# junfeng-chen/position_induced_transformer

Measured on AMD Instinct MI355X. Metric: PiT fwd+bwd samples/sec on Darcy2D, higher is better.
Workload: dtype f32; 1 GPU; darcy2d 43x43 grid->16x16 latent, pit_fixed hid64 H2 blocks4 loc0.02, RelL2 (train_darcy.py:64-111), fwd+loss+bwd, per-GPU batch 8; per_gpu_batch=8, global_batch=8, parallelism=single, launch=hipgraph, head_scale_route=host

## Files before the change

### include/pit_hip.h

```cpp
#ifndef PIT_HIP_H
#define PIT_HIP_H

#ifdef __cplusplus
extern "C" {
#endif

#define PIT_ABI_VERSION 23
#define PIT_DSCALE_SLOTS 1024

#define PIT_METRIC_EUCLID     0
#define PIT_METRIC_PERIODIC1D 1
#define PIT_METRIC_PERIODIC2D 2

#define PIT_ERR_NULL     -1
#define PIT_ERR_SIZE     -2
#define PIT_ERR_METRIC   -3
#define PIT_ERR_UNSUPPORTED -4

int pit_version(void);
const char* pit_error_string(int code);

#define PIT_MATH_FP32 0
#define PIT_MATH_BF16 1
#define PIT_IO_X_BF16    0x100
#define PIT_IO_SAVE_BF16 0x200
#define PIT_IO_DX_BF16   0x400
#define PIT_IO_OUT_BF16  0x800
#define PIT_IO_DOUT_BF16 0x1000
#define PIT_ATT_UNION    0x2000
int pit_mlp_bf16_io_supported(int rows, int n0, int n1, int n2, int out_gelu);

int pit_head_scale(const float* lmda, int n_head, float* scale_out, void* stream);

int pit_select_fwd(const float* mesh_out, const float* mesh_in, int mesh_batch, int n_out, int n_in,
                   int space_dim, int metric, float period, int rank_k, int need_kth,
                   float* stats, void* stream);

int pit_lists_transpose(const int* nbr_idx, const int* nbr_cnt, int mesh_batch, int n_out, int n_in, int cap,
                        int* rev_ptr, int* rev_row, int* workspace, void* stream);

#define PIT_PLAN_WAVE_PER_ROW 1
#define PIT_PLAN_TWO_PASSES   2
int pit_plan_fwd(const float* mesh_out, const float* mesh_in, int mesh_batch, int n_out, int n_in,
                 int space_dim, int metric, float period, int rank_k, float* stats, int cap,
                 int* nbr_idx, int* nbr_cnt, int* rev_ptr, int* rev_row, int* workspace, int flags, void* stream);

int pit_neighbors_fwd(const float* mesh_out, const float* mesh_in, int mesh_batch, int n_out, int n_in,
                      int space_dim, int metric, float period, const float* stats, int cap,
                      int* nbr_idx, int* nbr_cnt, int* rev_ptr, int* rev_row, int* workspace, void* stream);

int pit_posatt_fwd(const float* mesh_out, const float* mesh_in, int mesh_batch, int n_out, int n_in,
                   int space_dim, int metric, float period,
                   const float* values, int batch, int dim, long ld_values, long values_bstride,
                   const float* head, int n_head, int head_is_scale,
                   const float* stats, float rank_w, int masked, int self_attn,
                   float* out, long ld_out, long out_bstride, int out_col0, int copy_inputs,
                   float* rowstat, float* scale_out,
                   const int* nbr_idx, const int* nbr_cnt, int nbr_cap, int coord_dims, int math_mode, void* stream);

struct pit_mlp_params_job;

struct pit_block_weights_job {
    const float* mesh; int n_pts, space_dim, metric; float period;
    int n_layers; const float* const* heads; int head_is_scale, n_head;
    float *e, *q, *inv, *rowstat, *scale_out;
};
int pit_posatt_fwd_job(const float* mesh_out, const float* mesh_in, int mesh_batch, int n_out, int n_in,
                       int space_dim, int metric, float period,
                       const float* values, int batch, int dim, long ld_values, long values_bstride,
                       const float* head, int n_head, int head_is_scale,
                       const float* stats, float rank_w, int masked, int self_attn,
                       float* out, long ld_out, long out_bstride, int out_col0, int copy_inputs,
                       float* rowstat, float* scale_out,
                       const int* nbr_idx, const int* nbr_cnt, int nbr_cap, int coord_dims, int math_mode, void* stream,
                       const struct pit_block_weights_job* job);

typedef struct pit_mlp_params_job {
    const float* x; long ldx; int rows, n0, n1, n2; const float* h; int out_gelu;
    const float* d_y; long ld_dy;
    float *d_w1, *d_b1, *d_w2, *d_b2; int accumulate; const float* scratch; int math_mode;
} pit_mlp_params_job;
#define PIT_HEAD_ACCUMULATE 1
#define PIT_HEAD_DEFER      2
#define PIT_HEAD_IS_SCALE   4
int pit_posatt_bwd(const float* mesh_out, const float* mesh_in, int mesh_batch, int n_out, int n_in,
                   int space_dim, int metric, float period,
                   const float* values, int batch, int dim, long ld_values, long values_bstride,
                   const float* head, int n_head, int head_is_scale, const float* scale,
                   const float* rowstat, int masked,
                   const float* d_out, long ld_dout, long dout_bstride, int out_col0,
                   float* d_values, long ld_dvalues, long dvalues_bstride, int add_residual,
                   float* d_head, int accumulate_head, double* workspace,
                   const int* nbr_idx, const int* nbr_cnt, int nbr_cap, int nbr_complete,
                   const int* rev_ptr, const int* rev_row, const pit_mlp_params_job* rider,
                   int coord_dims, int math_mode, void* stream);

int pit_posatt_dhead_finish(int n_layers, double* const* workspaces, float* const* d_heads,
                            const float* const* heads, const float* const* scales, const int* n_heads,
                            const int* flags, const pit_mlp_params_job* rider, void* stream);

int pit_block_supported(int n_pts, int n_head, int dim, int batch);

int pit_block_weights(const float* mesh, int n_pts, int space_dim, int metric, float period, int n_layers,
                      const float* const* heads, int head_is_scale, int n_head, float* e, float* q,
                      float* inv, float* rowstat, float* scale_out, void* stream);

int pit_block_fwd(const float* e, const float* inv, int n_pts, int n_head, int dim, int batch, float* xcat,
                  const float* w1, const float* b1, const float* w2, const float* b2, int out_gelu,
                  float* z1, float* h, float* z2, float* y, long ldy, int math_mode, void* stream);

int pit_block_bwd(const float* e, const float* inv, const float* qw, int n_pts, int n_head, int dim, int batch,
                  const float* d_xcat, const float* xcat, double* dscale,
                  const float* w1, const float* w2, const float* z1, const float* z2, int out_gelu, int n0_prev,
                  float* d_xprev, long ld_dxprev, float* scratch_prev,
                  float* d_values, long ld_dvalues,
                  const struct pit_mlp_params_job* rider, const struct pit_mlp_params_job* rider2,
                  int math_mode, void* stream);

#define PIT_SLAB_UNION_MAX 64
typedef struct pit_slab_plan {
    int n_out, n_in, cap, n_slabs, umax;
    const float* stats; float rank_w;
    const int* idx; const int* cnt;
    const float* m; const unsigned short* slot; const int* keys; const int* nkeys;
    int rows;
} pit_slab_plan;
int pit_slab_plan_build(const float* mesh_out, const float* mesh_in, int n_out, int n_in, int space_dim, int metric, float period,
                        const int* nbr_idx, const int* nbr_cnt, int cap, int rows_per_slab, float* m, unsigned short* slot,
                        int* keys, int* nkeys, int* report, void* stream);
int pit_edge_supported(int n_head, int dim, int batch, int rows_per_sample);
int pit_decoder_weights(const pit_slab_plan* plan, const float* head, int head_is_scale, int n_head, int max_union, int max_count,
                        float* pw, float* qw, float* scale_out, const float* w1, float* w1f, int dim, void* stream);
typedef struct pit_decoder_weights_job {
    const pit_slab_plan* plan; const float* head; int head_is_scale, n_head, max_union, max_count;
    float *pw, *qw, *scale_out;
    const float* w1; float* w1f; int dim;
} pit_decoder_weights_job;
int pit_decoder_fwd(const pit_slab_plan* plan, const float* values, long ld_values, long values_bstride, int batch,
                    int n_head, int dim, const float* pw,
                    const float* w1, const float* w1f, const float* b1, const float* w2, const float* b2, int n2,
                    float* x, float* z1, float* h, float* y, float* zero_buf, long zero_n,
                    const float* loss_true, const float* loss_scale, const float* loss_shift, int loss_p, double* loss_part,
                    int max_union, void* stream);
int pit_decoder_bwd(const pit_slab_plan* plan, const float* values, long ld_values, long values_bstride, int batch,
                    int n_head, int dim, const float* pw, const float* qw,
                    const float* w1, const float* w2, int n2, const float* z1,
                    const float* d_y, long ld_dy, float* dz1, float* d_values, long dvalues_bstride, double* dscale,
                    const float* loss_pred, const float* loss_true, const float* loss_scale, const float* loss_shift,
                    const float* loss_seed, int loss_p, const double* loss_part, float* d_pred, float* loss_out,
                    float* norms_out, int max_union, void* stream);
int pit_union_att_supported(int n_head, int dim, int batch, int rows_per_sample);
int pit_union_att_fwd(const pit_slab_plan* plan, const float* values, long ld_values, long values_bstride, int batch,
                      int n_head, int dim, const float* pw, void* out, long ld_out, long out_bstride, int out_bf16,
                      int max_union, void* stream);
int pit_union_att_bwd(const pit_slab_plan* plan, const float* values, long ld_values, long values_bstride, int batch,
                      int n_head, int dim, const float* pw, const float* qw,
                      const void* d_out, long ld_dout, long dout_bstride, int dout_bf16,
                      float* d_values, long ld_dvalues, long dvalues_bstride, double* dscale, int max_union, void* stream);
int pit_fold_supported(int n_head, int dim, int batch, int rows_per_sample, int n_in);
int pit_fold_weights(const pit_slab_plan* plan, const float* head, int head_is_scale, int n_head, int max_union, int max_count,
                     float* pw, float* qw, float* scale_out, unsigned short* pw16, unsigned short* qw16, void* stream);
int pit_fold_att_fwd(const pit_slab_plan* plan, const float* vw, long ld_vw, long vw_bstride, int batch, int n_head, int dim,
                     const void* pw, void* z, long ld_z, long z_bstride, int max_union, int math_mode, void* stream);
int pit_fold_att_bwd(const pit_slab_plan* plan, const float* vw, long ld_vw, long vw_bstride, int batch, int n_head, int dim,
                     const void* pw, const void* qw, const void* dz, long ld_dz, long dz_bstride,
                     float* d_vw, long ld_dvw, long dvw_bstride, double* dscale,
                     float* tiles, const int* rev_ptr, const int* rev_ent, int max_union, int math_mode, void* stream);
int pit_thin_tail_scratch_floats(void);
int pit_thin_tail_fwd(const void* z, long ldz, int rows, int n1, int n2, const float* b1, const float* w2, const float* b2,
                      float* y, long ldy, int math_mode, void* stream);
int pit_thin_tail_bwd(const void* z, long ldz, int rows, int n1, int n2, const float* b1, const float* w2,
                      const float* d_y, long ld_dy, void* dz, long ld_dz, float* d_b1, float* d_w2, float* d_b2,
                      float* scratch, int math_mode, void* stream);
int pit_linear_fwd(const float* x, long ldx, int rows, int n_in, int n_out, const float* w, const float* zero_bias,
                   float* y, long ldy, int math_mode, void* stream);
int pit_linear_bwd(const float* x, long ldx, int rows, int n_in, int n_out, const float* w, const float* d_y, long ld_dy,
                   float* d_x, long ld_dx, float* d_w, int accumulate, int math_mode, void* stream);

struct pit_block_weights_job;
int pit_encoder_fwd(const pit_slab_plan* plan, const float* mesh_in, int space_dim, int coord_dims,
                    const float* values, long ld_values, long values_bstride, int value_dim, int batch,
                    int n_head, int dim, const float* head, int head_is_scale,
                    const float* w1, const float* b1, const float* w2, const float* b2,
                    float* x, float* z1, float* h, float* z2, float* y, long ldy, float* rowstat, float* scale_out,
                    float* clear_buf, long clear_n, const struct pit_block_weights_job* weights,
                    const pit_decoder_weights_job* dec_weights, void* stream);
int pit_encoder_bwd(const pit_slab_plan* plan, const float* mesh_in, int space_dim, int coord_dims,
                    const float* values, long ld_values, long values_bstride, int value_dim, int batch,
                    int n_head, int dim, const float* scale, const float* rowstat,
                    const float* w1, const float* w2, const float* z1, const float* z2,
                    const float* d_y, long ld_dy, float* scratch, double* dscale, void* stream);

int pit_posatt_pre_supported(int n_pts, int n_head, int dim, int batch);
int pit_posatt_pre_fwd(const float* e, const float* rowstat, int n_pts, int n_head, int dim, int batch,
                       const float* values, long ld_values, long values_bstride,
                       float* out, long ld_out, long out_bstride, int out_col0, int copy_inputs, int math_mode, void* stream);
int pit_posatt_pre_bwd(const float* e, const float* q, const float* rowstat, int n_pts, int n_head, int dim, int batch,
                       const float* values, long ld_values, long values_bstride,
                       const float* d_out, long ld_dout, long dout_bstride, int out_col0,
                       float* d_values, long ld_dvalues, long dvalues_bstride, int add_residual,
                       double* workspace, int math_mode, void* stream);

int pit_satt_supported(int n_pts, int n_head, int dim, int batch, int mesh_batch);
int pit_satt_fwd(const float* mesh, int mesh_batch, int n_pts, int space_dim, int metric, float period,
                 const float* values, long ld_values, long values_bstride, int batch, int dim,
                 const float* head, int n_head, int head_is_scale, unsigned short* x16,
                 float* out, long ld_out, long out_bstride, int out_col0, int copy_inputs,
                 float* rowstat, float* scale_out, unsigned short* e_tiles, int x16_ready, void* stream);
int pit_satt_bwd(const float* mesh, int mesh_batch, int n_pts, int space_dim, int metric, float period,
                 int batch, int dim, const float* scale, int n_head, const float* rowstat,
                 const unsigned short* x16, unsigned short* g16,
                 const float* d_out, long ld_dout, long dout_bstride, int out_col0,
                 float* d_values, long ld_dvalues, long dvalues_bstride, int add_residual, double* dscale,
                 const unsigned short* e_tiles, int g16_ready, const pit_mlp_params_job* rider, void* stream);
long pit_satt_tiles_elems(int n_pts);

int pit_mlp_fwd(const float* x, long ldx, int rows, int n0, int n1, int n2,
                const float* w1, const float* b1, const float* w2, const float* b2, int out_gelu,
                float* z1, float* h, float* z2, float* y, long ldy, int math_mode, void* stream);

int pit_mlp_chain_supported(int rows, int n0, int n1, int n2);
int pit_mlp_chain_fwd(const float* x, long ldx, int rows, int n0, int n1, const unsigned short* w1_bf16, const float* b1,
                      const unsigned short* w2_bf16, const float* b2, float* z1, float* h, float* z2, float* y, long ldy,
                      unsigned short* y16 , void* stream);
int pit_mlp_chain_bwd(int rows, int n0, int n1, const unsigned short* w1_bf16, const unsigned short* w2_bf16,
                      const float* z1, const float* z2, const float* d_y, long ld_dy, float* d_x, long ld_dx, float* scratch,
                      unsigned short* g16 ,
                      const float* rowstat , int pts, int mesh_batch, void* stream);
int pit_cast_bf16_multi(int n, const float* const* src, unsigned short* const* dst, const long* count, void* stream);

int pit_mlp_bwd(const float* x, long ldx, int rows, int n0, int n1, int n2,
                const float* w1, const float* w2, const float* z1, const float* h, const float* z2,
                int out_gelu, const float* d_y, long ld_dy,
                float* d_x, long ld_dx, float* d_w1, float* d_b1, float* d_w2, float* d_b2,
                int accumulate, float* scratch, int math_mode, void* stream);

int pit_mlp_bwd_data(int rows, int n0, int n1, int n2, const float* w1, const float* w2,
                     const float* z1, const float* z2, int out_gelu, const float* d_y, long ld_dy,
                     float* d_x, long ld_dx, float* scratch, int math_mode, void* stream);
int pit_mlp_bwd_params(const float* x, long ldx, int rows, int n0, int n1, int n2, const float* h,
                       int out_gelu, const float* d_y, long ld_dy,
                       float* d_w1, float* d_b1, float* d_w2, float* d_b2,
                       int accumulate, const float* scratch, int math_mode, void* stream);
int pit_mlp_bwd_params_deferrable(int rows, int n0, int n1, int n2, int out_gelu, long ld_dy);

#define PIT_REL_LP_WS_FLOATS(batch, nch) (4 + 5 * (batch) * (nch))
int pit_rel_lp_loss_fwd(const float* tru, const float* pred, const float* pred_scale,
                        const float* pred_shift, int batch, int npts, int nch, int p,
                        float* norms, float* loss, float* workspace, void* stream);
int pit_rel_lp_loss_bwd(const float* tru, const float* pred, const float* pred_scale,
                        const float* pred_shift, int batch, int npts, int nch, int p,
                        const float* norms, const float* grad_loss, float* d_pred, float* d_true, void* stream);

int pit_rel_lp_loss_fwd_grad(const float* tru, const float* pred, const float* pred_scale,
                             const float* pred_shift, int batch, int npts, int nch, int p,
                             float* norms, float* loss, float* workspace, float* d_pred_unit,
                             float* d_true_unit, float* clear_buf, long clear_n, void* stream);

int pit_rel_max_norm(const float* tru, const float* pred, int batch, int npts, int nch, float* out,
                     double* workspace, void* stream);

int pit_instance_norm_fwd(const float* x, long ldx, long x_bstride, int batch, int npts, int nch, float eps,
                          float* y, float* rstd, void* stream);
int pit_instance_norm_bwd(const float* d_y, const float* y, const float* rstd, int batch, int npts, int nch,
                          float* d_x, void* stream);

int pit_adam_step(float* params, float* grads, float* exp_avg, float* exp_avg_sq, long n,
                  long long* step, float lr0, float eta_min, int cosine_t_max, float beta1, float beta2,
                  float eps, float weight_decay, int zero_grads, float* scalars, void* stream);

int pit_debug_mfma_tile(const float* a, const float* b, float* d, void* stream);

#ifdef __cplusplus
}
#endif
#endif
```

### position_induced_transformer_amd/_lib.py

```python
from __future__ import annotations

import ctypes
import os

import torch

_HERE = os.path.dirname(os.path.abspath(__file__))
LIB_PATH = os.environ.get("PIT_LIB_PATH") or os.path.join(_HERE, "csrc", "libpit_hip.so")

_P = ctypes.c_void_p
_I = ctypes.c_int
_L = ctypes.c_long
_F = ctypes.c_float

class MlpParamsJob(ctypes.Structure):
    _fields_ = [("x", _P), ("ldx", _L), ("rows", _I), ("n0", _I), ("n1", _I), ("n2", _I), ("h", _P), ("out_gelu", _I),
                ("d_y", _P), ("ld_dy", _L), ("d_w1", _P), ("d_b1", _P), ("d_w2", _P), ("d_b2", _P),
                ("accumulate", _I), ("scratch", _P), ("math_mode", _I)]


class BlockWeightsJob(ctypes.Structure):
    _fields_ = [("mesh", _P), ("n_pts", _I), ("space_dim", _I), ("metric", _I), ("period", _F),
                ("n_layers", _I), ("heads", _P), ("head_is_scale", _I), ("n_head", _I),
                ("e", _P), ("q", _P), ("inv", _P), ("rowstat", _P), ("scale_out", _P)]


class SlabPlan(ctypes.Structure):
    _fields_ = [("n_out", _I), ("n_in", _I), ("cap", _I), ("n_slabs", _I), ("umax", _I), ("stats", _P), ("rank_w", _F),
                ("idx", _P), ("cnt", _P), ("m", _P), ("slot", _P), ("keys", _P), ("nkeys", _P), ("rows", _I)]


class DecoderWeightsJob(ctypes.Structure):
    _fields_ = [("plan", _P), ("head", _P), ("head_is_scale", _I), ("n_head", _I), ("max_union", _I), ("max_count", _I),
                ("pw", _P), ("qw", _P), ("scale_out", _P), ("w1", _P), ("w1f", _P), ("dim", _I)]


SIGNATURES = {
    "pit_version": [],
    "pit_error_string": [_I],
    "pit_head_scale": [_P, _I, _P, _P],
    "pit_select_fwd": [_P, _P, _I, _I, _I, _I, _I, _F, _I, _I, _P, _P],
    "pit_plan_fwd": [_P, _P, _I, _I, _I, _I, _I, _F, _I, _P, _I, _P, _P, _P, _P, _P, _I, _P],
    "pit_lists_transpose": [_P, _P, _I, _I, _I, _I, _P, _P, _P, _P],
    "pit_neighbors_fwd": [_P, _P, _I, _I, _I, _I, _I, _F, _P, _I, _P, _P, _P, _P, _P, _P],
    "pit_posatt_fwd": [_P, _P, _I, _I, _I, _I, _I, _F,
                       _P, _I, _I, _L, _L,
                       _P, _I, _I,
                       _P, _F, _I, _I,
                       _P, _L, _L, _I, _I,
                       _P, _P, _P, _P, _I, _I, _I, _P],
    "pit_posatt_fwd_job": [_P, _P, _I, _I, _I, _I, _I, _F,
                           _P, _I, _I, _L, _L,
                           _P, _I, _I,
                           _P, _F, _I, _I,
                           _P, _L, _L, _I, _I,
                           _P, _P, _P, _P, _I, _I, _I, _P, _P],
    "pit_posatt_bwd": [_P, _P, _I, _I, _I, _I, _I, _F,
                       _P, _I, _I, _L, _L,
                       _P, _I, _I, _P,
                       _P, _I,
                       _P, _L, _L, _I,
                       _P, _L, _L, _I,
                       _P, _I, _P, _P, _P, _I, _I, _P, _P, _P, _I, _I, _P],
    "pit_posatt_dhead_finish": [_I, _P, _P, _P, _P, _P, _P, _P, _P],
    "pit_block_supported": [_I, _I, _I, _I],
    "pit_block_weights": [_P, _I, _I, _I, _F, _I, _P, _I, _I, _P, _P, _P, _P, _P, _P],
    "pit_block_fwd": [_P, _P, _I, _I, _I, _I, _P, _P, _P, _P, _P, _I, _P, _P, _P, _P, _L, _I, _P],
    "pit_slab_plan_build": [_P, _P, _I, _I, _I, _I, _F, _P, _P, _I, _I, _P, _P, _P, _P, _P, _P],
    "pit_fold_supported": [_I, _I, _I, _I, _I],
    "pit_fold_weights": [_P, _P, _I, _I, _I, _I, _P, _P, _P, _P, _P, _P],
    "pit_fold_att_fwd": [_P, _P, _L, _L, _I, _I, _I, _P, _P, _L, _L, _I, _I, _P],
    "pit_fold_att_bwd": [_P, _P, _L, _L, _I, _I, _I, _P, _P, _P, _L, _L, _P, _L, _L, _P, _P, _P, _P, _I, _I, _P],
    "pit_thin_tail_scratch_floats": [],
    "pit_thin_tail_fwd": [_P, _L, _I, _I, _I, _P, _P, _P, _P, _L, _I, _P],
    "pit_thin_tail_bwd": [_P, _L, _I, _I, _I, _P, _P, _P, _L, _P, _L, _P, _P, _P, _P, _I, _P],
    "pit_satt_supported": [_I, _I, _I, _I, _I],
    "pit_satt_fwd": [_P, _I, _I, _I, _I, _F, _P, _L, _L, _I, _I, _P, _I, _I, _P, _P, _L, _L, _I, _I, _P, _P, _P, _I, _P],
    "pit_satt_bwd": [_P, _I, _I, _I, _I, _F, _I, _I, _P, _I, _P, _P, _P, _P, _L, _L, _I, _P, _L, _L, _I, _P, _P, _I, _P, _P],
    "pit_satt_tiles_elems": [_I],
    "pit_mlp_chain_supported": [_I, _I, _I, _I],
    "pit_mlp_chain_fwd": [_P, _L, _I, _I, _I, _P, _P, _P, _P, _P, _P, _P, _P, _L, _P, _P],
    "pit_mlp_chain_bwd": [_I, _I, _I, _P, _P, _P, _P, _P, _L, _P, _L, _P, _P, _P, _I, _I, _P],
    "pit_cast_bf16_multi": [_I, _P, _P, _P, _P],
    "pit_linear_fwd": [_P, _L, _I, _I, _I, _P, _P, _P, _L, _I, _P],
    "pit_linear_bwd": [_P, _L, _I, _I, _I, _P, _P, _L, _P, _L, _P, _I, _I, _P],
    "pit_edge_supported": [_I, _I, _I, _I],
    "pit_decoder_weights": [_P, _P, _I, _I, _I, _I, _P, _P, _P, _P, _P, _I, _P],
    "pit_decoder_fwd": [_P, _P, _L, _L, _I, _I, _I, _P, _P, _P, _P, _P, _P, _I, _P, _P, _P, _P, _P, _L,
                        _P, _P, _P, _I, _P, _I, _P],
    "pit_decoder_bwd": [_P, _P, _L, _L, _I, _I, _I, _P, _P, _P, _P, _I, _P, _P, _L, _P, _P, _L, _P,
                        _P, _P, _P, _P, _P, _I, _P, _P, _P, _P, _I, _P],
    "pit_union_att_supported": [_I, _I, _I, _I],
    "pit_union_att_fwd": [_P, _P, _L, _L, _I, _I, _I, _P, _P, _L, _L, _I, _I, _P],
    "pit_union_att_bwd": [_P, _P, _L, _L, _I, _I, _I, _P, _P, _P, _L, _L, _I, _P, _L, _L, _P, _I, _P],
    "pit_encoder_fwd": [_P, _P, _I, _I, _P, _L, _L, _I, _I, _I, _I, _P, _I, _P, _P, _P, _P,
                        _P, _P, _P, _P, _P, _L, _P, _P, _P, _L, _P, _P, _P],
    "pit_encoder_bwd": [_P, _P, _I, _I, _P, _L, _L, _I, _I, _I, _I, _P, _P, _P, _P, _P, _P, _P, _L, _P, _P, _P],
    "pit_posatt_pre_supported": [_I, _I, _I, _I],
    "pit_posatt_pre_fwd": [_P, _P, _I, _I, _I, _I, _P, _L, _L, _P, _L, _L, _I, _I, _I, _P],
    "pit_posatt_pre_bwd": [_P, _P, _P, _I, _I, _I, _I, _P, _L, _L, _P, _L, _L, _I, _P, _L, _L, _I, _P, _I, _P],
    "pit_block_bwd": [_P, _P, _P, _I, _I, _I, _I, _P, _P, _P, _P, _P, _P, _P, _I, _I, _P, _L, _P, _P, _L, _P, _P, _I, _P],
    "pit_mlp_bf16_io_supported": [_I, _I, _I, _I, _I],
    "pit_mlp_fwd": [_P, _L, _I, _I, _I, _I, _P, _P, _P, _P, _I, _P, _P, _P, _P, _L, _I, _P],
    "pit_mlp_bwd": [_P, _L, _I, _I, _I, _I, _P, _P, _P, _P, _P, _I, _P, _L,
                    _P, _L, _P, _P, _P, _P, _I, _P, _I, _P],
    "pit_mlp_bwd_data": [_I, _I, _I, _I, _P, _P, _P, _P, _I, _P, _L, _P, _L, _P, _I, _P],
    "pit_mlp_bwd_params": [_P, _L, _I, _I, _I, _I, _P, _I, _P, _L, _P, _P, _P, _P, _I, _P, _I, _P],
    "pit_mlp_bwd_params_deferrable": [_I, _I, _I, _I, _I, _L],
    "pit_rel_lp_loss_fwd": [_P, _P, _P, _P, _I, _I, _I, _I, _P, _P, _P, _P],
    "pit_rel_lp_loss_fwd_grad": [_P, _P, _P, _P, _I, _I, _I, _I, _P, _P, _P, _P, _P, _P, _L, _P],
    "pit_rel_lp_loss_bwd": [_P, _P, _P, _P, _I, _I, _I, _I, _P, _P, _P, _P, _P],
    "pit_rel_max_norm": [_P, _P, _I, _I, _I, _P, _P, _P],
    "pit_instance_norm_fwd": [_P, _L, _L, _I, _I, _I, _F, _P, _P, _P],
    "pit_instance_norm_bwd": [_P, _P, _P, _I, _I, _I, _P, _P],
    "pit_adam_step": [_P, _P, _P, _P, _L, _P, _F, _F, _I, _F, _F, _F, _F, _I, _P, _P],
    "pit_debug_mfma_tile": [_P, _P, _P, _P],
}

LONG_RETURN = {"pit_satt_tiles_elems"}
ABI_VERSION = 23

_lib = None


def lib() -> ctypes.CDLL:
    global _lib
    if _lib is None:
        if not os.path.exists(LIB_PATH):
            raise RuntimeError(
                f"{LIB_PATH} not found: build it with `python -m position_induced_transformer_amd.build` "
                "(hipcc --offload-arch=gfx950). There is no CPU or PyTorch fallback for the PiT hot path.")
        handle = ctypes.CDLL(LIB_PATH)
        for name, argtypes in SIGNATURES.items():
            fn = getattr(handle, name)
            fn.argtypes = argtypes
            fn.restype = ctypes.c_char_p if name == "pit_error_string" else (_L if name in LONG_RETURN else _I)
        got = handle.pit_version()
        if got != ABI_VERSION:
            raise RuntimeError(f"{LIB_PATH} implements PIT_ABI_VERSION {got}, this package binds version {ABI_VERSION}: "
                               "rebuild it (python -m position_induced_transformer_amd.build)")
        _lib = handle
    return _lib


def check(code: int, what: str) -> None:
    if code != 0:
        msg = lib().pit_error_string(code)
        raise RuntimeError(f"{what} failed ({code}): {msg.decode() if msg else '?'}")


def stream_ptr() -> int:
    return torch.cuda.current_stream().cuda_stream


def ptr(t) -> int:
    return 0 if t is None else t.data_ptr()
```

### position_induced_transformer_amd/csrc/pit_block.hip

```cpp
#include "pit_common.h"
#include "pit_gemm_rd.h"
#include "pit_block_dev.h"
#include <cstdlib>

namespace {

#ifdef PIT_STAMPS
__device__ unsigned long long pit_block_stamps[32];
#define BSTAMP(i_) do { if (blockIdx.x == 5 && threadIdx.x == 0) pit_block_stamps[i_] = __builtin_amdgcn_s_memtime(); } while (0)
#else
#define BSTAMP(i_) do { } while (0)
#endif

#ifdef PIT_WGREC
__device__ unsigned long long pit_block_wgrec[1024 * 4];
#define BREC(slot_) do { if (threadIdx.x == 0 && blockIdx.x < 1024) {                                                       \
        pit_block_wgrec[blockIdx.x * 4 + (slot_)] = __builtin_amdgcn_s_memrealtime();                                       \
        if ((slot_) == 0) { pit_block_wgrec[blockIdx.x * 4 + 2] = __builtin_amdgcn_s_getreg((4 << 0) | (0 << 6) | (31 << 11));   \
                            pit_block_wgrec[blockIdx.x * 4 + 3] = __builtin_amdgcn_s_getreg((20 << 0) | (0 << 6) | (31 << 11)); } } } while (0)
#else
#define BREC(slot_) do { } while (0)
#endif
#ifdef PIT_STAMPS_DBG
__device__ int pit_block_dbg = 0;
#define PIT_BLOCK_DBG pit_block_dbg
#else
#define PIT_BLOCK_DBG 0
#endif
#ifndef PIT_BLOCK_EXP
#define PIT_BLOCK_EXP 0
#endif

__global__ __launch_bounds__(256) void block_weights_kernel(WeightsArgs a) { block_weights_body(a, blockIdx.x); }

template <int NH, bool SHARED>
__device__ __forceinline__ void slab_contract(const float* __restrict__ w, long wstride, int L, const float* __restrict__ v,
                                              long ldv, int vhead, const float* __restrict__ sc, int jb, int je, int l15, int kq,
                                              f32x4_t (&acc)[SHARED ? NH : 1][4]) {
    constexpr int NS = SHARED ? 2 : 1;
    const float* wp = w + (long)l15 * L + 4 * kq;
    const float* vp = v + 4 * l15;
    for (int j0 = jb; j0 < je; j0 += 16 * NS) {
        float4 av[NH][NS], sv[NH][NS], bv[SHARED ? 1 : NH][NS][4];
        const int dbg = PIT_BLOCK_DBG;
#pragma unroll
        for (int h = 0; h < NH; ++h)
#pragma unroll
            for (int s = 0; s < NS; ++s) {
                av[h][s] = (dbg & 4) ? make_float4(1.f, 2.f, 3.f, 4.f) : *reinterpret_cast<const float4*>(wp + h * wstride + j0 + 16 * s);
                if (!SHARED) sv[h][s] = *reinterpret_cast<const float4*>(sc + (long)h * L + j0 + 16 * s + 4 * kq);
            }
#pragma unroll
        for (int h = 0; h < (SHARED ? 1 : NH); ++h)
#pragma unroll
            for (int s = 0; s < NS; ++s)
#pragma unroll
                for (int m = 0; m < 4; ++m)
                    bv[h][s][m] = (dbg & 2) ? make_float4(1.f, 2.f, 3.f, 4.f)
                                            : *reinterpret_cast<const float4*>(vp + h * vhead + (long)(j0 + 16 * s + 4 * kq + m) * ldv);
        __builtin_amdgcn_sched_barrier(0);
#pragma unroll
        for (int s = 0; s < NS; ++s)
#pragma unroll
            for (int m = 0; m < 4; ++m)
#pragma unroll
                for (int h = 0; h < NH; ++h) {
                    if ((PIT_BLOCK_EXP & (SHARED ? 1 : 4)) && (SHARED ? s == 1 : h == 1)) {
                        asm volatile("" :: "v"(av[h][s].x), "v"(av[h][s].y), "v"(av[h][s].z), "v"(av[h][s].w));
                        asm volatile("" :: "v"(bv[SHARED ? 0 : h][s][m].x), "v"(bv[SHARED ? 0 : h][s][m].y), "v"(bv[SHARED ? 0 : h][s][m].z), "v"(bv[SHARED ? 0 : h][s][m].w));
                        if (!SHARED) asm volatile("" :: "v"(sv[h][s].x), "v"(sv[h][s].y), "v"(sv[h][s].z), "v"(sv[h][s].w));
                        continue;
                    }
                    const float* ap = &av[h][s].x;
                    const float* sp = &sv[h][s].x;
                    const float aw = SHARED ? ap[m] : ap[m] * sp[m];
                    const float4 bb = bv[SHARED ? 0 : h][s][m];
                    f32x4_t (&ac)[4] = acc[SHARED ? h : 0];
                    ac[0] = mfma_16x16x4(aw, bb.x, ac[0]);
                    ac[1] = mfma_16x16x4(aw, bb.y, ac[1]);
                    ac[2] = mfma_16x16x4(aw, bb.z, ac[2]);
                    ac[3] = mfma_16x16x4(aw, bb.w, ac[3]);
                }
    }
}

__device__ __forceinline__ bool slab_of(int id, int batch, int slabs, int& sample, int& slab) {
    if (PIT_BLOCK_DBG & 1) return slab_of_linear(id, batch, slabs, sample, slab);
    return slab_of_xcd(id, batch, slabs, sample, slab);
}

struct BlockFwdArgs {
    const float *e, *inv;
    int L, batch;
    float* xcat;
    const float *w1, *b1, *w2, *b2;
    int out_gelu;
    float *z1, *h, *z2, *y; long ldy;
};

template <int H, bool WLDS>
__global__ __launch_bounds__(512, WLDS ? 1 : 2) void block_fwd_kernel(BlockFwdArgs g) {
    constexpr int W = (1 + H) * BD;
    constexpr int XP = W + 4, HP = BD + 4;
    constexpr int KS = W / 16;
    constexpr int NW1 = BD * W / 4 / 512, NW2 = BD * BD / 4 / 512;
    extern __shared__ __attribute__((aligned(16))) float smem[];
    float* pk = smem;
    float* xs = smem + H * PARK_FLOATS;
    float* hs = xs + 16 * XP;
    float* w1s = hs + 16 * HP;
    float* w2s = w1s + BD * XP;
    const int tid = threadIdx.x, lane = tid & 63, wave = tid >> 6;
    const int l15 = lane & 15, kq = lane >> 4;
    const int slabs = g.L / 16;
    int b, slab;
    if (!slab_of(blockIdx.x, g.batch, slabs, b, slab)) return;
    const int n0 = slab * 16;
    const long m0 = ((long)b * slabs + slab) * 16;
    const int klen = g.L / BW;

    float4 xown = make_float4(0.f, 0.f, 0.f, 0.f);
    if (tid < 256) xown = *reinterpret_cast<const float4*>(g.xcat + (m0 + (tid >> 4)) * W + 4 * (tid & 15));
    const float rinv0 = g.inv[(long)((tid >> 8) % H) * g.L + n0 + 4 * ((tid & 63) >> 4) + ((tid >> 6) & 3)];

    BSTAMP(0);
    const bool mlp_wave = wave < 4;
    const int c1 = (wave & 3) * 16 + l15;
    float4 bv[KS], w2v[4];
    float bias = 0.0f, bias2 = 0.0f;
    auto load_weights = [&]() {
        if (!mlp_wave) return;
        if (!WLDS) {
#pragma unroll
            for (int s = 0; s < KS; ++s) bv[s] = *reinterpret_cast<const float4*>(g.w1 + (long)c1 * W + 16 * s + 4 * kq);
#pragma unroll
            for (int s = 0; s < 4; ++s) w2v[s] = *reinterpret_cast<const float4*>(g.w2 + (long)c1 * BD + 16 * s + 4 * kq);
        }
        bias = g.b1[c1];
        bias2 = g.b2[c1];
    };
    f32x4_t wq1[WLDS ? NW1 : 1], wq2[WLDS ? NW2 : 1];
    if (WLDS) {
#pragma unroll
        for (int p = 0; p < NW1; ++p) wq1[p] = reinterpret_cast<const f32x4_t*>(g.w1)[p * 512 + tid];
#pragma unroll
        for (int p = 0; p < NW2; ++p) wq2[p] = reinterpret_cast<const f32x4_t*>(g.w2)[p * 512 + tid];
        load_weights();
    }
    f32x4_t acc[H][4];
#pragma unroll
    for (int hh = 0; hh < H; ++hh)
#pragma unroll
        for (int t = 0; t < 4; ++t) acc[hh][t] = f32x4_t{0.f, 0.f, 0.f, 0.f};
    constexpr int EP = 256 + 4;
    const bool elds = WLDS && g.L == 256 && !(PIT_BLOCK_EXP & 64);
    if (elds) {
        float* es = w1s;
        const float* vp = g.xcat + (long)b * g.L * W + 4 * l15;
        const int j0 = wave * 32;
        f32x4_t eq[H * 2];
#pragma unroll
        for (int p = 0; p < H * 2; ++p) {
            const int q = p * 512 + tid;
            eq[p] = *reinterpret_cast<const f32x4_t*>(g.e + (long)(q >> 10) * g.L * g.L + (long)(n0 + ((q >> 6) & 15)) * g.L + 4 * (q & 63));
        }
        f32x4_t bvv[2][4];
#pragma unroll
        for (int s = 0; s < 2; ++s)
#pragma unroll
            for (int m = 0; m < 4; ++m) bvv[s][m] = *reinterpret_cast<const f32x4_t*>(vp + (long)(j0 + 16 * s + 4 * kq + m) * W);
        __builtin_amdgcn_sched_barrier(0);
#pragma unroll
        for (int p = 0; p < H * 2; ++p) {
            const int q = p * 512 + tid;
            *reinterpret_cast<f32x4_t*>(es + ((q >> 10) * 16 + ((q >> 6) & 15)) * EP + 4 * (q & 63)) = eq[p];
        }
        __syncthreads();
#pragma unroll
        for (int s = 0; s < 2; ++s) {
            f32x4_t av[H];
#pragma unroll
            for (int hh = 0; hh < H; ++hh) av[hh] = *reinterpret_cast<const f32x4_t*>(es + (hh * 16 + l15) * EP + j0 + 16 * s + 4 * kq);
#pragma unroll
            for (int m = 0; m < 4; ++m)
#pragma unroll
                for (int hh = 0; hh < H; ++hh) {
                    acc[hh][0] = mfma_16x16x4(av[hh][m], bvv[s][m][0], acc[hh][0]);
                    acc[hh][1] = mfma_16x16x4(av[hh][m], bvv[s][m][1], acc[hh][1]);
                    acc[hh][2] = mfma_16x16x4(av[hh][m], bvv[s][m][2], acc[hh][2]);
                    acc[hh][3] = mfma_16x16x4(av[hh][m], bvv[s][m][3], acc[hh][3]);
                }
        }
    } else {
        slab_contract<H, true>(g.e + (long)n0 * g.L, (long)g.L * g.L, g.L, g.xcat + (long)b * g.L * W, W, 0, nullptr,
                               wave * klen, (wave + 1) * klen, l15, kq, acc);
    }
    BSTAMP(1);
    if (!WLDS) load_weights();
#pragma unroll
    for (int hh = 0; hh < H; ++hh) park(pk, wave * H + hh, lane, acc[hh]);
    if (tid < 256) *reinterpret_cast<float4*>(xs + (tid >> 4) * XP + 4 * (tid & 15)) = xown;
    __syncthreads();
    BSTAMP(2);
    for (int item = tid; item < H * 256; item += 512) {
        const int hh = item >> 8, i = (item >> 6) & 3, ln = item & 63;
        const int r = 4 * (ln >> 4) + i, col = 4 * (ln & 15);
        float4 s = parked_sum(pk, hh, BW, H, i, ln);
        const float rinv = item == tid ? rinv0 : g.inv[(long)hh * g.L + n0 + r];
        s.x *= rinv; s.y *= rinv; s.z *= rinv; s.w *= rinv;
        *reinterpret_cast<float4*>(xs + r * XP + BD + hh * BD + col) = s;
        *reinterpret_cast<float4*>(g.xcat + (m0 + r) * W + BD + hh * BD + col) = s;
    }
    if (WLDS) {
#pragma unroll
        for (int p = 0; p < NW1; ++p) {
            const int q = p * 512 + tid, row = q / (W / 4), c4 = q % (W / 4);
            *reinterpret_cast<f32x4_t*>(w1s + row * XP + 4 * c4) = wq1[p];
        }
#pragma unroll
        for (int p = 0; p < NW2; ++p) {
            const int q = p * 512 + tid, row = q / (BD / 4), c4 = q % (BD / 4);
            *reinterpret_cast<f32x4_t*>(w2s + row * HP + 4 * c4) = wq2[p];
        }
    }
    BSTAMP(3);
    __syncthreads();
    BSTAMP(4);
    if (mlp_wave) {
        f32x4_t a0 = {0.f, 0.f, 0.f, 0.f}, a1 = {0.f, 0.f, 0.f, 0.f};
#pragma unroll
        for (int s = 0; s < KS; ++s) {
            if ((PIT_BLOCK_EXP & 2) && (s & 1)) { if (!WLDS) asm volatile("" :: "v"(bv[s].x), "v"(bv[s].y), "v"(bv[s].z), "v"(bv[s].w)); continue; }
            const float4 a = *reinterpret_cast<const float4*>(xs + l15 * XP + 16 * s + 4 * kq);
            const float4 bw = WLDS ? *reinterpret_cast<const float4*>(w1s + c1 * XP + 16 * s + 4 * kq) : bv[s];
            a0 = mfma_16x16x4(a.x, bw.x, a0);
            a1 = mfma_16x16x4(a.y, bw.y, a1);
            a0 = mfma_16x16x4(a.z, bw.z, a0);
            a1 = mfma_16x16x4(a.w, bw.w, a1);
        }
        BSTAMP(5);
#pragma unroll
        for (int i = 0; i < 4; ++i) {
            const int r = 4 * kq + i;
            const float z = a0[i] + a1[i] + bias;
            const float hv = gelu_erf(z);
            hs[r * HP + c1] = hv;
            g.z1[(m0 + r) * BD + c1] = z;
            g.h[(m0 + r) * BD + c1] = hv;
        }
    }
    BSTAMP(6);
    __syncthreads();
    BSTAMP(7);
    if (!mlp_wave) return;
    f32x4_t o0 = {0.f, 0.f, 0.f, 0.f}, o1 = {0.f, 0.f, 0.f, 0.f};
#pragma unroll
    for (int s = 0; s < 4; ++s) {
        const float4 a = *reinterpret_cast<const float4*>(hs + l15 * HP + 16 * s + 4 * kq);
        const float4 bw = WLDS ? *reinterpret_cast<const float4*>(w2s + c1 * HP + 16 * s + 4 * kq) : w2v[s];
        o0 = mfma_16x16x4(a.x, bw.x, o0);
        o1 = mfma_16x16x4(a.y, bw.y, o1);
        o0 = mfma_16x16x4(a.z, bw.z, o0);
        o1 = mfma_16x16x4(a.w, bw.w, o1);
    }
    BSTAMP(8);
#pragma unroll
    for (int i = 0; i < 4; ++i) {
        const long r = m0 + 4 * kq + i;
        float v = o0[i] + o1[i] + bias2;
        if (g.out_gelu) { g.z2[r * BD + c1] = v; v = gelu_erf(v); }
        g.y[r * g.ldy + c1] = v;
    }
    BSTAMP(9);
}

struct BlockBwdArgs {
    const float *e, *inv, *qw;
    int L, batch;
    const float* d_xcat;
    const float* xcat;
    double* dscale;
    const float *w1, *w2, *z1, *z2; int out_gelu, n0p;
    float *d_xprev; long ld_dxprev;
    float *dz1, *dz2;
    float* d_values; long ld_dvalues;
    int n_chain, n_ds;
};

template <int H>
__device__ __forceinline__ void block_bwd_chain(const BlockBwdArgs& g, float* smem, int slab) {
    constexpr int W = (1 + H) * BD;
    constexpr int P1 = BD + 4;
    float* pk = smem;
    float* ds2 = smem + PARK_FLOATS;
    float* ds1 = ds2 + 16 * P1;
    const int tid = threadIdx.x, lane = tid & 63, wave = tid >> 6;
    const int l15 = lane & 15, kq = lane >> 4;
    const int slabs = g.L / 16;
    int b, sl;
    if (!slab_of(slab, g.batch, slabs, b, sl)) return;
    const int j0 = sl * 16;
    const long m0 = ((long)b * slabs + sl) * 16;
    const int klen = g.L / BW;

    const int oi = (tid >> 6) & 3, oln = tid & 63, oh = tid >> 8;
    const int orow = 4 * (oln >> 4) + oi, ocol = 4 * (oln & 15) + 2 * oh;
    const bool has_mlp = g.w1 != nullptr;
    const float2 res = *reinterpret_cast<const float2*>(g.d_xcat + (m0 + orow) * W + ocol);
    float2 z2v = make_float2(0.f, 0.f);
    if (has_mlp && g.out_gelu) z2v = *reinterpret_cast<const float2*>(g.z2 + (m0 + orow) * BD + ocol);
    const int c1 = (wave & 3) * 16 + l15;
    BSTAMP(10);
    f32x4_t acc[1][4];
#pragma unroll
    for (int t = 0; t < 4; ++t) acc[0][t] = f32x4_t{0.f, 0.f, 0.f, 0.f};
    slab_contract<H, false>(g.e + (long)j0 * g.L, (long)g.L * g.L, g.L, g.d_xcat + (long)b * g.L * W + BD, W, BD, g.inv,
                            wave * klen, (wave + 1) * klen, l15, kq, acc);
    BSTAMP(11);
    float w2v[4][4], z1v[4], w1v[2][4][4];
    if (has_mlp) {
        if (wave < 4) {
#pragma unroll
            for (int s = 0; s < 4; ++s)
#pragma unroll
                for (int ee = 0; ee < 4; ++ee) w2v[s][ee] = g.w2[(long)(16 * s + 4 * kq + ee) * BD + c1];
#pragma unroll
            for (int i = 0; i < 4; ++i) z1v[i] = g.z1[(m0 + 4 * kq + i) * BD + c1];
        }
#pragma unroll
        for (int t = 0; t < 2; ++t) {
            const int col = (wave + t * BW) * 16 + l15;
#pragma unroll
            for (int s = 0; s < 4; ++s)
#pragma unroll
                for (int ee = 0; ee < 4; ++ee)
                    w1v[t][s][ee] = (col < g.n0p) ? g.w1[(long)(16 * s + 4 * kq + ee) * g.n0p + col] : 0.0f;
        }
    }
    park(pk, wave, lane, acc[0]);
    __syncthreads();
    BSTAMP(12);
    {
        float2 s = res;
#pragma unroll
        for (int w = 0; w < BW; ++w) {
            s.x += pk[((w * 4 + 2 * oh) * 4 + oi) * 64 + oln];
            s.y += pk[((w * 4 + 2 * oh + 1) * 4 + oi) * 64 + oln];
        }
        if (!has_mlp) {
            *reinterpret_cast<float2*>(g.d_values + (m0 + orow) * g.ld_dvalues + ocol) = s;
        } else {
            if (g.out_gelu) { s.x *= gelu_erf_grad(z2v.x); s.y *= gelu_erf_grad(z2v.y); }
            *reinterpret_cast<float2*>(g.dz2 + (m0 + orow) * BD + ocol) = s;
            *reinterpret_cast<float2*>(ds2 + orow * P1 + ocol) = s;
        }
    }
    if (!has_mlp) return;
    BSTAMP(13);
    __syncthreads();
    BSTAMP(14);
    if (wave < 4) {
        f32x4_t a0 = {0.f, 0.f, 0.f, 0.f}, a1 = {0.f, 0.f, 0.f, 0.f};
#pragma unroll
        for (int s = 0; s < 4; ++s) {
            const float4 a = *reinterpret_cast<const float4*>(ds2 + l15 * P1 + 16 * s + 4 * kq);
            a0 = mfma_16x16x4(a.x, w2v[s][0], a0);
            a1 = mfma_16x16x4(a.y, w2v[s][1], a1);
            a0 = mfma_16x16x4(a.z, w2v[s][2], a0);
            a1 = mfma_16x16x4(a.w, w2v[s][3], a1);
        }
#pragma unroll
        for (int i = 0; i < 4; ++i) {
            const int r = 4 * kq + i;
            const float v = (a0[i] + a1[i]) * gelu_erf_grad(z1v[i]);
            ds1[r * P1 + c1] = v;
            g.dz1[(m0 + r) * BD + c1] = v;
        }
    }
    BSTAMP(15);
    __syncthreads();
    BSTAMP(16);
    if (!g.d_xprev) return;
#pragma unroll
    for (int t = 0; t < 2; ++t) {
        const int tile = wave + t * BW;
        if (tile * 16 >= g.n0p) break;
        if ((PIT_BLOCK_EXP & 8) && t == 1) {
#pragma unroll
            for (int s = 0; s < 4; ++s) asm volatile("" :: "v"(w1v[t][s][0]), "v"(w1v[t][s][1]), "v"(w1v[t][s][2]), "v"(w1v[t][s][3]));
            break;
        }
        f32x4_t o0 = {0.f, 0.f, 0.f, 0.f}, o1 = {0.f, 0.f, 0.f, 0.f};
#pragma unroll
        for (int s = 0; s < 4; ++s) {
            const float4 a = *reinterpret_cast<const float4*>(ds1 + l15 * P1 + 16 * s + 4 * kq);
            o0 = mfma_16x16x4(a.x, w1v[t][s][0], o0);
            o1 = mfma_16x16x4(a.y, w1v[t][s][1], o1);
            o0 = mfma_16x16x4(a.z, w1v[t][s][2], o0);
            o1 = mfma_16x16x4(a.w, w1v[t][s][3], o1);
        }
        const int col = tile * 16 + l15;
        if (col < g.n0p) {
#pragma unroll
            for (int i = 0; i < 4; ++i) g.d_xprev[(m0 + 4 * kq + i) * g.ld_dxprev + col] = o0[i] + o1[i];
        }
    }
    BSTAMP(17);
}

template <int H>
__device__ __forceinline__ void block_bwd_dscale(const BlockBwdArgs& g, float* smem, int slab) {
    constexpr int W = (1 + H) * BD;
    float* pk = smem;
    double* wred = reinterpret_cast<double*>(smem + H * PARK_FLOATS);
    const int tid = threadIdx.x, lane = tid & 63, wave = tid >> 6;
    const int l15 = lane & 15, kq = lane >> 4;
    const int slabs = g.L / 16;
    int b, sl;
    if (!slab_of(slab, g.batch, slabs, b, sl)) return;
    const int n0 = sl * 16;
    const long m0 = ((long)b * slabs + sl) * 16;
    const int klen = g.L / BW;
    const bool own = tid < H * 256;
    const int hh = tid >> 8, i = (tid >> 6) & 3, ln = tid & 63;
    const int r = 4 * (ln >> 4) + i, col = 4 * (ln & 15);
    float4 dov = make_float4(0.f, 0.f, 0.f, 0.f);
    if (own) dov = *reinterpret_cast<const float4*>(g.d_xcat + (m0 + r) * W + BD + hh * BD + col);
    f32x4_t acc[H][4];
#pragma unroll
    for (int h2 = 0; h2 < H; ++h2)
#pragma unroll
        for (int t = 0; t < 4; ++t) acc[h2][t] = f32x4_t{0.f, 0.f, 0.f, 0.f};
    slab_contract<H, true>(g.qw + (long)n0 * g.L, (long)g.L * g.L, g.L, g.xcat + (long)b * g.L * W, W, 0, nullptr,
                           wave * klen, (wave + 1) * klen, l15, kq, acc);
#pragma unroll
    for (int h2 = 0; h2 < H; ++h2) park(pk, wave * H + h2, lane, acc[h2]);
    __syncthreads();
    double part = 0.0;
    if (own) {
        const float4 s = parked_sum(pk, hh, BW, H, i, ln);
        part = (double)s.x * (double)dov.x + (double)s.y * (double)dov.y + (double)s.z * (double)dov.z + (double)s.w * (double)dov.w;
    }
    part = wave_sum_d(part);
    if (lane == 0) wred[wave] = part;
    __syncthreads();
    if (tid < H) {
        double tot = 0.0;
        for (int w = 4 * tid; w < 4 * tid + 4; ++w) tot += wred[w];
        atomicAdd(g.dscale + (long)tid * PIT_DSCALE_SLOTS + ((int)(m0 >> 4) & (PIT_DSCALE_SLOTS - 1)), -tot);
    }
}

template <int H, int NDW>
__global__ __launch_bounds__(512) void block_bwd_kernel(BlockBwdArgs g, pit_detail::DwPair w, pit_detail::DwPair w2) {
    extern __shared__ __attribute__((aligned(16))) float smem[];
    int id = blockIdx.x;
    BREC(0);
    if (id < g.n_chain) { block_bwd_chain<H>(g, smem, id); BREC(1); return; }
    id -= g.n_chain;
    if (id < g.n_ds) { block_bwd_dscale<H>(g, smem, id); BREC(1); return; }
    id -= g.n_ds;
    if (PIT_BLOCK_EXP & 32) return;
    if (NDW >= 1 && id < w.n1 + w.n2) { dw_pair_body(w, id, smem); BREC(1); return; }
    if (NDW >= 2) dw_pair_body(w2, id - (w.n1 + w.n2), smem);
    BREC(1);
}

constexpr size_t fwd_smem(int H, bool wlds) {
    return ((size_t)H * PARK_FLOATS + 16 * ((1 + H) * BD + 4) + 16 * (BD + 4) + (wlds ? BD * ((1 + H) * BD + 4) + BD * (BD + 4) : 0)) * sizeof(float);
}
constexpr size_t bwd_smem(int H, bool dscale) {
    return std::max((size_t)(PARK_FLOATS + 2 * 16 * (BD + 4)) * sizeof(float),
                    dscale ? ((size_t)H * PARK_FLOATS) * sizeof(float) + BW * sizeof(double) : (size_t)0);
}

}

extern "C" int pit_block_supported(int n_pts, int n_head, int dim, int batch) {
    if (dim != BD || (n_head != 1 && n_head != 2)) return 0;
    if (n_pts <= 0 || batch <= 0 || n_pts % (32 * BW) != 0) return 0;
    if (n_pts > 2048) return 0;
    const long rows = (long)batch * n_pts;
    return rows >= 256 && rows <= 16384;
}

extern "C" int pit_block_weights(const float* mesh, int n_pts, int space_dim, int metric, float period, int n_layers,
                                 const float* const* heads, int head_is_scale, int n_head, float* e, float* q,
                                 float* inv, float* rowstat, float* scale_out, void* stream) {
    WeightsArgs a;
    if (int rc = fill_weights_args(a, mesh, n_pts, space_dim, metric, period, n_layers, heads, head_is_scale, n_head, e, q, inv,
                                   rowstat, scale_out)) return rc;
    const long rows = (long)n_layers * n_head * n_pts;
    hipLaunchKernelGGL(block_weights_kernel, dim3((unsigned)((rows + 3) / 4)), dim3(256), 0, (hipStream_t)stream, a);
    PIT_CHECK_LAUNCH();
    return 0;
}

extern "C" int pit_block_fwd(const float* e, const float* inv, int n_pts, int n_head, int dim, int batch, float* xcat,
                             const float* w1, const float* b1, const float* w2, const float* b2, int out_gelu,
                             float* z1, float* h, float* z2, float* y, long ldy, int math_mode, void* stream) {
    if (!e || !inv || !xcat || !w1 || !b1 || !w2 || !b2 || !z1 || !h || !y || (out_gelu && !z2)) return PIT_ERR_NULL;
    if (math_mode != PIT_MATH_FP32 || !pit_block_supported(n_pts, n_head, dim, batch)) return PIT_ERR_UNSUPPORTED;
    if (ldy < dim || !aligned16(e) || !aligned16(xcat) || !aligned16(w1) || !aligned16(w2)) return PIT_ERR_SIZE;
    BlockFwdArgs g;
    g.e = e; g.inv = inv; g.L = n_pts; g.batch = batch; g.xcat = xcat;
    g.w1 = w1; g.b1 = b1; g.w2 = w2; g.b2 = b2; g.out_gelu = out_gelu;
    g.z1 = z1; g.h = h; g.z2 = z2; g.y = y; g.ldy = ldy;
    const dim3 grid((unsigned)slab_grid(batch, n_pts / 16)), block(64 * BW);
    static const bool no_wlds = getenv("PIT_NO_BLOCK_WLDS") != nullptr;
    static const int n_cus = [] {
        int dev = 0, cus = 0;
        if (hipGetDevice(&dev) != hipSuccess || hipDeviceGetAttribute(&cus, hipDeviceAttributeMultiprocessorCount, dev) != hipSuccess) cus = 0;
        return cus;
    }();
    const bool earlyw = !no_wlds && (int)grid.x <= n_cus;
    const size_t FWD_SMEM = fwd_smem(n_head, earlyw);
#define PIT_BLOCK_FWD(H_, E_)                                                                                              \
    do {                                                                                                                   \
        static bool once = ((void)hipFuncSetAttribute((const void*)block_fwd_kernel<H_, E_>,                              \
                                                hipFuncAttributeMaxDynamicSharedMemorySize, 160 * 1024), true);            \
        (void)once;                                                                                                        \
        hipLaunchKernelGGL((block_fwd_kernel<H_, E_>), grid, block, FWD_SMEM, (hipStream_t)stream, g);                     \
    } while (0)
    if (n_head == 1) { if (earlyw) PIT_BLOCK_FWD(1, true); else PIT_BLOCK_FWD(1, false); }
    else { if (earlyw) PIT_BLOCK_FWD(2, true); else PIT_BLOCK_FWD(2, false); }
#undef PIT_BLOCK_FWD
    PIT_CHECK_LAUNCH();
    return 0;
}

#ifdef PIT_WGREC
extern "C" int pit_block_read_wgrec(unsigned long long* out, int n) {
    return (int)hipMemcpyFromSymbol(out, HIP_SYMBOL(pit_block_wgrec), (size_t)n * 4 * sizeof(unsigned long long));
}
#endif
#ifdef PIT_STAMPS_DBG
extern "C" int pit_block_set_dbg(int v) { return (int)hipMemcpyToSymbol(HIP_SYMBOL(pit_block_dbg), &v, sizeof(int)); }
#endif
#ifdef PIT_STAMPS
extern "C" int pit_block_read_stamps(unsigned long long* out) {
    return (int)hipMemcpyFromSymbol(out, HIP_SYMBOL(pit_block_stamps), sizeof(unsigned long long) * 32);
}
#endif

extern "C" int pit_block_bwd(const float* e, const float* inv, const float* qw, int n_pts, int n_head, int dim, int batch,
                             const float* d_xcat, const float* xcat, double* dscale,
                             const float* w1, const float* w2, const float* z1, const float* z2, int out_gelu, int n0_prev,
                             float* d_xprev, long ld_dxprev, float* scratch_prev,
                             float* d_values, long ld_dvalues,
                             const pit_mlp_params_job* rider, const pit_mlp_params_job* rider2, int math_mode, void* stream) {
    if (!e || !inv || !d_xcat) return PIT_ERR_NULL;
    if (dscale && (!qw || !xcat)) return PIT_ERR_NULL;
    if (math_mode != PIT_MATH_FP32 || !pit_block_supported(n_pts, n_head, dim, batch)) return PIT_ERR_UNSUPPORTED;
    const bool has_mlp = w1 != nullptr;
    if (has_mlp) {
        if (!w2 || !z1 || !scratch_prev || (out_gelu && !z2)) return PIT_ERR_NULL;
        if (n0_prev <= 0 || n0_prev > 16 * 16 || (d_xprev && ld_dxprev < n0_prev)) return PIT_ERR_SIZE;
    } else if (!d_values || ld_dvalues < dim || ld_dvalues % 4 != 0 || !aligned16(d_values)) {
        return d_values ? PIT_ERR_SIZE : PIT_ERR_NULL;
    }
    if (!aligned16(e) || !aligned16(d_xcat) || (qw && !aligned16(qw)) || (xcat && !aligned16(xcat)) ||
        (has_mlp && (!aligned16(scratch_prev) || (z2 && !aligned16(z2))))) return PIT_ERR_SIZE;
    hipStream_t s = (hipStream_t)stream;
    const long rows = (long)batch * n_pts;
    BlockBwdArgs g;
    g.e = e; g.inv = inv; g.qw = qw; g.L = n_pts; g.batch = batch; g.d_xcat = d_xcat; g.xcat = xcat; g.dscale = dscale;
    g.w1 = w1; g.w2 = w2; g.z1 = z1; g.z2 = z2; g.out_gelu = out_gelu; g.n0p = n0_prev;
    g.d_xprev = d_xprev; g.ld_dxprev = ld_dxprev;
    g.dz1 = scratch_prev; g.dz2 = has_mlp ? scratch_prev + rows * dim : nullptr;
    g.d_values = d_values; g.ld_dvalues = ld_dvalues;
    g.n_chain = slab_grid(batch, n_pts / 16);
    g.n_ds = dscale ? g.n_chain : 0;
    pit_detail::DwPair dw = pit_detail::DwPair(), dw2 = pit_detail::DwPair();
    const pit_mlp_params_job* jobs[2] = {rider, rider2};
    pit_detail::DwPair* plans[2] = {&dw, &dw2};
    int ndw = 0;
    bool carried[2] = {false, false};
    for (int r = 0; r < 2; ++r)
        if (jobs[r] && pit_detail::plan_dw_pair(*jobs[r], BW, plans[ndw], 768, true)) { carried[r] = true; ++ndw; }
    const int n_dw = (ndw >= 1 ? dw.n1 + dw.n2 : 0) + (ndw >= 2 ? dw2.n1 + dw2.n2 : 0);
    const bool any_rr = (ndw >= 1 && (dw.rr1 || dw.rr2)) || (ndw >= 2 && (dw2.rr1 || dw2.rr2));
    const size_t sm = std::max(std::max(bwd_smem(n_head, dscale != nullptr), ndw ? (size_t)BW * 16 * 64 * sizeof(float) : (size_t)0),
                               any_rr ? (size_t)4 * pit_detail::RR_BK * 64 * sizeof(float) : (size_t)0);
    const dim3 grid((unsigned)(g.n_chain + g.n_ds + n_dw)), block(64 * BW);
#define PIT_BLOCK_BWD(H_, DW_)                                                                                             \
    do {                                                                                                                   \
        static bool once = ((void)hipFuncSetAttribute((const void*)block_bwd_kernel<H_, DW_>,                             \
                                                hipFuncAttributeMaxDynamicSharedMemorySize, 98304), true);                 \
        (void)once;                                                                                                        \
        hipLaunchKernelGGL((block_bwd_kernel<H_, DW_>), grid, block, sm, s, g, dw, dw2);                                   \
    } while (0)
#define PIT_BLOCK_BWD_H(H_) do { if (ndw == 2) PIT_BLOCK_BWD(H_, 2); else if (ndw == 1) PIT_BLOCK_BWD(H_, 1); else PIT_BLOCK_BWD(H_, 0); } while (0)
    if (n_head == 1) PIT_BLOCK_BWD_H(1); else PIT_BLOCK_BWD_H(2);
#undef PIT_BLOCK_BWD_H
#undef PIT_BLOCK_BWD
    PIT_CHECK_LAUNCH();
    for (int r = 0; r < 2; ++r)
        if (jobs[r] && !carried[r]) {
            const pit_mlp_params_job* j = jobs[r];
            const int rc = pit_mlp_bwd_params(j->x, j->ldx, j->rows, j->n0, j->n1, j->n2, j->h, j->out_gelu, j->d_y, j->ld_dy,
                                              j->d_w1, j->d_b1, j->d_w2, j->d_b2, j->accumulate, j->scratch, j->math_mode, stream);
            if (rc) return rc;
        }
    return 0;
}
```

### position_induced_transformer_amd/ops.py

```python
from __future__ import annotations

import ctypes
import math
import os
import threading
from collections import OrderedDict
from typing import Optional

import numpy as np
import torch

from . import _lib

METRIC_ID = {"euclid": 0, "periodic1d": 1, "periodic2d": 2}

FUSED_GRAD_ACCUMULATION = True

SPARSE_MASKED = True

_DSCALE_WS = {}
_LOSS_WS = {}
_PINNED = []


def _capturing() -> bool:
    return torch.cuda.is_available() and torch.cuda.is_current_stream_capturing()


_PINNED_IDS = set()


def _pin(*objs) -> None:
    for o in objs:
        if id(o) not in _PINNED_IDS:
            _PINNED_IDS.add(id(o))
            _PINNED.append(o)


def _ws_key(device):
    return (device.index, torch.cuda.current_stream(device).cuda_stream)


def _graph_task() -> int:
    return torch._C._current_graph_task_id()


def _dscale_workspace(device, n_head: int) -> torch.Tensor:
    key = _ws_key(device)
    ws = _DSCALE_WS.get(key)
    if ws is None or ws.numel() < n_head * 1024 + 8:
        ws = torch.zeros(max(8, n_head) * 1024 + 8, device=device, dtype=torch.float64)
        _DSCALE_WS[key] = ws
    if _capturing():
        _pin(ws)
    return ws


DEFER_HEAD_FINISH = os.environ.get("PIT_DEFER_HEAD_FINISH", "1") != "0"
_PENDING_HEADS = {}
_LAYER_WS = {}
_MAX_PENDING_TASKS = 64


def _layer_workspace(slot: torch.Tensor, n_head: int) -> torch.Tensor:
    key = (slot.device.index, slot.data_ptr(), n_head)
    ws = _LAYER_WS.get(key)
    if ws is None:
        while len(_LAYER_WS) >= 1024:
            _LAYER_WS.pop(next(iter(_LAYER_WS)))
        ws = _LAYER_WS[key] = torch.zeros(n_head * 1024, device=slot.device, dtype=torch.float64)
    if _capturing():
        _pin(ws)
    return ws


def _flush_head_finishes(task: int) -> None:
    seen, pend = set(), []
    for entry in _PENDING_HEADS.pop(task, ()):
        key = (entry[0].data_ptr(), entry[1].data_ptr())
        if key not in seen:
            seen.add(key)
            pend.append(entry)
    job = _PENDING_DW.get(task)
    for dev in sorted({p[0].device.index for p in pend}):
        grp = [p for p in pend if p[0].device.index == dev]
        for i in range(0, len(grp), 32):
            part = grp[i:i + 32]
            n = len(part)
            rider = None
            if job is not None and job[2].device.index == dev and job[2] == torch.cuda.current_stream(job[2].device):
                rider, job = job, None
                _PENDING_DW[task] = None
            ws = (ctypes.c_void_p * n)(*[p[0].data_ptr() for p in part])
            dh = (ctypes.c_void_p * n)(*[p[1].data_ptr() for p in part])
            hd = (ctypes.c_void_p * n)(*[p[2].data_ptr() for p in part])
            sc = (ctypes.c_void_p * n)(*[p[3].data_ptr() for p in part])
            nh = (ctypes.c_int * n)(*[p[4] for p in part])
            fl = (ctypes.c_int * n)(*[p[5] for p in part])
            with torch.cuda.device(dev):
                rc = _lib.lib().pit_posatt_dhead_finish(n, ws, dh, hd, sc, nh, fl,
                                                        ctypes.cast(ctypes.pointer(rider[0]), ctypes.c_void_p) if rider is not None else None,
                                                        _lib.stream_ptr())
            _lib.check(rc, "pit_posatt_dhead_finish")


def _defer_head_begin(work: torch.Tensor) -> None:
    task = _graph_task()
    ptr = work.data_ptr()
    for other in [t for t in _PENDING_HEADS if t != task]:
        stale = [e for e in _PENDING_HEADS[other] if e[0].data_ptr() == ptr]
        if stale:
            stale[0][0].zero_()
            _PENDING_HEADS[other] = [e for e in _PENDING_HEADS[other] if e[0].data_ptr() != ptr]
            if not _PENDING_HEADS[other]:
                del _PENDING_HEADS[other]
    if task not in _PENDING_HEADS:
        while len(_PENDING_HEADS) >= _MAX_PENDING_TASKS:
            for e in _PENDING_HEADS.pop(next(iter(_PENDING_HEADS))):
                e[0].zero_()
        _PENDING_HEADS[task] = []
        torch.autograd.Variable._execution_engine.queue_callback(lambda: _flush_head_finishes(task))


def _defer_head_finish(work, d_head, head, scale, n_head: int, flags: int) -> None:
    _defer_head_begin(work)
    _PENDING_HEADS[_graph_task()].append((work, d_head, head, scale, n_head, flags))


MLP_PARAMS_RIDER = os.environ.get("PIT_DW_RIDER", "1") != "0"
_STEP = threading.local()


def _processor_hook():
    return getattr(_STEP, "processor_hook", None)


class step_state:

    def __init__(self, processor_hook=None, loss=None, clear=None):
        self.new = (processor_hook, loss, clear)

    def __enter__(self):
        self.old = (getattr(_STEP, "processor_hook", None), getattr(_STEP, "loss", None), getattr(_STEP, "clear", None),
                    getattr(_STEP, "loss_issued", None))
        _STEP.processor_hook, _STEP.loss, _STEP.clear = self.new
        _STEP.loss_issued = None
        return self

    def __exit__(self, *exc):
        _STEP.processor_hook, _STEP.loss, _STEP.clear, _STEP.loss_issued = self.old
        return False


def take_pending_clear():
    t = getattr(_STEP, "clear", None)
    _STEP.clear = None
    return t


_PENDING_DW = {}
_DEFERRABLE = {}


def _dw_run(job) -> None:
    st, keep, stream = job
    cur = torch.cuda.current_stream(stream.device)
    with torch.cuda.stream(stream):
        rc = _lib.lib().pit_mlp_bwd_params(st.x, st.ldx, st.rows, st.n0, st.n1, st.n2, st.h, st.out_gelu, st.d_y,
                                           st.ld_dy, st.d_w1, st.d_b1, st.d_w2, st.d_b2, st.accumulate, st.scratch,
                                           st.math_mode, stream.cuda_stream)
    _lib.check(rc, "pit_mlp_bwd_params")
    if cur != stream:
        cur.wait_stream(stream)


def _dw_flush(task: int) -> None:
    job = _PENDING_DW.get(task)
    if job is not None:
        _PENDING_DW[task] = None
        _dw_run(job)


def _dw_end_of_pass(task: int) -> None:
    _dw_flush(task)
    _PENDING_DW.pop(task, None)


def _dw_defer(st, keep, device) -> None:
    task = _graph_task()
    for other in [t for t, j in _PENDING_DW.items() if t != task and j is not None and j[0].d_w1 == st.d_w1]:
        del _PENDING_DW[other]
    if task not in _PENDING_DW:
        while len(_PENDING_DW) >= _MAX_PENDING_TASKS:
            del _PENDING_DW[next(iter(_PENDING_DW))]
        _PENDING_DW[task] = None
        torch.autograd.Variable._execution_engine.queue_callback(lambda: _dw_end_of_pass(task))
    else:
        _dw_flush(task)
    _PENDING_DW[task] = (st, keep, torch.cuda.current_stream(device))


def _dw_take(device):
    task = _graph_task()
    job = _PENDING_DW.get(task)
    if job is None:
        return None
    if job[2] != torch.cuda.current_stream(device):
        _dw_flush(task)
        return None
    _PENDING_DW[task] = None
    return job


BIG_RIDER_ROWS = 8192


def _dw_pending_rows(device) -> int:
    job = _PENDING_DW.get(_graph_task())
    return int(job[0].rows) if job is not None else 0


def _dw_slices(job, parts: int):
    st = job[0]
    out, per = [], -(-st.rows // parts // 16) * 16
    for r0 in range(0, st.rows, per):
        n = min(per, st.rows - r0)
        out.append(_lib.MlpParamsJob(st.x + 4 * r0 * st.ldx, st.ldx, n, st.n0, st.n1, st.n2, st.h + 4 * r0 * st.n1, 0,
                                     st.d_y + 4 * r0 * st.ld_dy, st.ld_dy, st.d_w1, st.d_b1, st.d_w2, st.d_b2, 1,
                                     st.scratch + 4 * r0 * st.n1, st.math_mode))
    return out


def _dw_deferrable(rows: int, n0: int, n1: int, n2: int, out_gelu: int, ld_dy: int) -> bool:
    key = (rows, n0, n1, n2, out_gelu, ld_dy)
    v = _DEFERRABLE.get(key)
    if v is None:
        if len(_DEFERRABLE) > 4096:
            _DEFERRABLE.clear()
        v = _DEFERRABLE[key] = bool(_lib.lib().pit_mlp_bwd_params_deferrable(*key))
    return v


def mark_inplace_grad(param, grad_view) -> None:
    param._pit_grad_ptr = grad_view.data_ptr()


def _grad_slot(param) -> Optional[torch.Tensor]:
    if not FUSED_GRAD_ACCUMULATION or param is None:
        return None
    want = getattr(param, "_pit_grad_ptr", None)
    g = getattr(param, "grad", None)
    if want is None or g is None or g.data_ptr() != want:
        return None
    if not g.is_cuda or g.dtype != torch.float32 or not g.is_contiguous():
        return None
    if param._backward_hooks or getattr(param, "_post_accumulate_grad_hooks", None):
        return None
    return g


IO_X_BF16, IO_SAVE_BF16, IO_DX_BF16, IO_OUT_BF16, IO_DOUT_BF16 = 0x100, 0x200, 0x400, 0x800, 0x1000
BF16_STORAGE = os.environ.get("PIT_BF16_STORAGE", "1") != "0"


def mlp_bf16_io_supported(rows: int, n0: int, n1: int, n2: int) -> bool:
    return BF16_STORAGE and get_math_mode() == "bf16" and bool(_lib.lib().pit_mlp_bf16_io_supported(rows, n0, n1, n2, 0))


def _need_gpu_bf16_ok(t) -> None:
    if t is not None and not t.is_cuda:
        raise RuntimeError("position_induced_transformer_amd: the PiT hot path runs on the HIP device only; "
                           "got a CPU tensor (move the model and its inputs to 'cuda')")
    if t is not None and t.dtype not in (torch.float32, torch.bfloat16):
        raise RuntimeError(f"position_induced_transformer_amd: fp32 (or bf16-stored) tensor expected, got {t.dtype}")


def _need_gpu(*tensors) -> None:
    for t in tensors:
        if t is not None and not t.is_cuda:
            raise RuntimeError("position_induced_transformer_amd: the PiT hot path runs on the HIP device only; "
                               "got a CPU tensor (move the model and its inputs to 'cuda')")
        if t is not None and t.dtype != torch.float32:
            raise RuntimeError(f"position_induced_transformer_amd: fp32 tensors expected, got {t.dtype}")


def quantile_rank(locality: float, n_in: int):
    rank = np.float32(locality) * np.float32(n_in - 1)
    k = int(np.floor(rank))
    w = np.float32(rank - np.float32(k))
    return k, float(w)


def mesh_period(metric: str, mesh_in: torch.Tensor) -> float:
    if metric == "periodic1d":
        return float(torch.abs(mesh_in[1, 0] - mesh_in[0, 0]) * mesh_in.shape[0])
    if metric == "periodic2d":
        res = int(mesh_in.shape[0] ** 0.5)
        dx = (torch.max(mesh_in[:, 0]) - torch.min(mesh_in[:, 0])) / (res - 1)
        return float(dx * res)
    return 0.0


SLAB_UNION_MAX = 64
FOLD_SLAB_ROWS = (256, 128, 64)
PLAN_FLAGS = 0
UNION_TILES = os.environ.get("PIT_UNION_TILES", "auto")
UNION_DV = os.environ.get("PIT_UNION_DV", "auto")
_UNION_DECISIONS = {}
ATT_UNION = 0x2000


class MeshPlan:

    __slots__ = ("mesh_out", "mesh_in", "mesh_batch", "n_out", "n_in", "sdim", "metric", "metric_id", "period",
                 "rank_k", "rank_w", "masked", "self_attn", "stats", "nbr_idx", "nbr_cnt", "nbr_cap", "rev_ptr",
                 "rev_row", "_complete", "_union", "_slab", "_fold")

    def __init__(self, metric: str, mesh_out: torch.Tensor, mesh_in: torch.Tensor, locality: float,
                 self_attn: bool, period: Optional[float] = None):
        _need_gpu(mesh_out, mesh_in)
        if metric not in METRIC_ID:
            raise ValueError(f"unknown metric {metric!r}")
        if mesh_out.dim() != mesh_in.dim() or mesh_out.dim() not in (2, 3):
            raise RuntimeError(f"mesh shapes {tuple(mesh_out.shape)} / {tuple(mesh_in.shape)} not supported")
        if mesh_out.shape[-1] != mesh_in.shape[-1]:
            raise RuntimeError("mesh_out and mesh_in must have the same number of coordinates")
        batched = mesh_out.dim() == 3
        if batched and metric != "euclid":
            raise RuntimeError("periodic metrics are defined for batch-free meshes only (pit.py:186-258)")
        if batched and mesh_out.shape[0] != mesh_in.shape[0]:
            raise RuntimeError("batched meshes must share the batch size")
        self.metric = metric
        self.metric_id = METRIC_ID[metric]
        self.mesh_out = mesh_out.detach().contiguous()
        self.mesh_in = self.mesh_out if (self_attn and mesh_in is mesh_out) else mesh_in.detach().contiguous()
        self.mesh_batch = mesh_out.shape[0] if batched else 1
        self.n_out, self.n_in, self.sdim = mesh_out.shape[-2], mesh_in.shape[-2], mesh_out.shape[-1]
        if not 1 <= self.sdim <= 3:
            raise RuntimeError("space_dim must be 1, 2 or 3")
        self.period = mesh_period(metric, self.mesh_in) if period is None else float(period)
        self.rank_k, self.rank_w = quantile_rank(locality, self.n_in)
        self.masked = bool(locality < 1.0)
        self.self_attn = bool(self_attn)
        self.stats = None
        self.nbr_idx = self.nbr_cnt = self.rev_ptr = self.rev_row = None
        self.nbr_cap = 0
        self._complete = None
        self._union = None
        self._slab = None
        self._fold = None
        cap = 0
        if self.masked and SPARSE_MASKED:
            want = self.rank_k + 2
            cap = ((want + max(16, want // 4) + 15) // 16) * 16
            if cap * 3 > self.n_in:
                cap = 0
        if self.masked or not self.self_attn:
            self.stats = torch.empty((3, self.mesh_batch, self.n_out), device=mesh_out.device, dtype=torch.float32)
        if cap:
            self._build_lists(cap, self._wants_reverse_lists(cap))
        elif self.stats is not None:
            rc = _lib.lib().pit_select_fwd(self.mesh_out.data_ptr(), self.mesh_in.data_ptr(), self.mesh_batch,
                                           self.n_out, self.n_in, self.sdim, self.metric_id, self.period,
                                           self.rank_k, 1 if self.masked else 0, self.stats.data_ptr(),
                                           _lib.stream_ptr())
            _lib.check(rc, "pit_select_fwd")

    def _union_key(self, cap):
        return (self.metric, self.n_out, self.n_in, cap, self.mesh_batch > 1, self.sdim)

    def _wants_reverse_lists(self, cap: int) -> bool:
        return self.mesh_batch == 1

    def ensure_reverse_lists(self) -> None:
        if self.nbr_idx is None or self.rev_ptr is not None:
            return
        dev = self.mesh_out.device
        rev_ptr = torch.empty((self.mesh_batch, self.n_in + 1), device=dev, dtype=torch.int32)
        rev_row = torch.empty((self.mesh_batch, self.n_out * self.nbr_cap), device=dev, dtype=torch.int32)
        work = torch.empty((2 * self.mesh_batch * self.n_in,), device=dev, dtype=torch.int32)
        rc = _lib.lib().pit_lists_transpose(self.nbr_idx.data_ptr(), self.nbr_cnt.data_ptr(), self.mesh_batch, self.n_out,
                                            self.n_in, self.nbr_cap, rev_ptr.data_ptr(), rev_row.data_ptr(), work.data_ptr(),
                                            _lib.stream_ptr())
        if rc == -4:
            self._build_lists(self.nbr_cap, True)
            return
        _lib.check(rc, "pit_lists_transpose")
        self.rev_ptr, self.rev_row = rev_ptr, rev_row

    def union_tiles(self) -> bool:
        if self._union is not None:
            return self._union
        if self.nbr_idx is None or UNION_TILES == "0" or self.n_in > 4096 or self.n_out < 16 or self.nbr_cap > 64 \
                or (self.mesh_batch == 1 and UNION_TILES != "1"):
            self._union = False
            return False
        if UNION_TILES == "1":
            self._union = True
            return True
        key = self._union_key(self.nbr_cap)
        hit = _UNION_DECISIONS.get(key)
        if hit is None:
            if torch.cuda.is_current_stream_capturing():
                return False
            cap, tiles = self.nbr_cap, min(32, self.n_out // 16)
            first = (torch.linspace(0, self.n_out // 16 - 1, tiles).long() * 16).to(self.nbr_idx.device)
            rows = (first[:, None] + torch.arange(16, device=first.device)[None, :]).reshape(-1)
            idx = self.nbr_idx.view(-1, cap)[rows].long()
            cnt = self.nbr_cnt[rows].long()
            keys = torch.where(torch.arange(cap, device=first.device)[None, :] < cnt[:, None], idx, -1).view(tiles, 16 * cap)
            srt = torch.sort(keys, dim=1).values
            union = (srt[:, 1:] != srt[:, :-1]).sum(1) + 1 - (srt[:, 0] < 0).long()
            mean_u, mean_k, over = (float(v) for v in torch.stack(
                [union.float().mean(), cnt.float().mean(), (cnt > cap).float().max()]).tolist())
            hit = over == 0.0 and mean_u <= min(64.0, 4.0 * mean_k)
            _UNION_DECISIONS[key] = hit
        self._union = hit
        return hit

    def slab_plan(self):
        if self._slab is not None:
            return self._slab or None
        if self.nbr_idx is None or self.mesh_batch != 1 or not self.masked or self.n_in > 16384 or self.nbr_cap > 64:
            self._slab = False
            return None
        if torch.cuda.is_current_stream_capturing():
            return None
        dev = self.mesh_out.device
        built = self._build_slab_plan(16)
        if built is None:
            self._slab = False
            return None
        self._slab = built
        return self._slab

    def _build_slab_plan(self, rows: int):
        dev = self.mesh_out.device
        n_slabs = (self.n_out + rows - 1) // rows
        m = torch.empty((n_slabs * rows, self.nbr_cap), device=dev, dtype=torch.float32)
        slot = torch.empty((n_slabs * rows, self.nbr_cap), device=dev, dtype=torch.int16)
        keys = torch.empty((n_slabs, SLAB_UNION_MAX), device=dev, dtype=torch.int32)
        nkeys = torch.empty((n_slabs,), device=dev, dtype=torch.int32)
        report = torch.zeros((3,), device=dev, dtype=torch.int32)
        rc = _lib.lib().pit_slab_plan_build(self.mesh_out.data_ptr(), self.mesh_in.data_ptr(), self.n_out, self.n_in, self.sdim,
                                            self.metric_id, self.period, self.nbr_idx.data_ptr(), self.nbr_cnt.data_ptr(),
                                            self.nbr_cap, rows, m.data_ptr(), slot.data_ptr(), keys.data_ptr(), nkeys.data_ptr(),
                                            report.data_ptr(), _lib.stream_ptr())
        _lib.check(rc, "pit_slab_plan_build")
        max_union, overflowed, max_count = report.tolist()
        if overflowed:
            return None
        sp = _lib.SlabPlan(self.n_out, self.n_in, self.nbr_cap, n_slabs, SLAB_UNION_MAX, self.stats.data_ptr(), self.rank_w,
                           self.nbr_idx.data_ptr(), self.nbr_cnt.data_ptr(), m.data_ptr(), slot.data_ptr(), keys.data_ptr(),
                           nkeys.data_ptr(), rows)
        return (sp, int(max_union), (m, slot, keys, nkeys), max(1, int(max_count)))

    def fold_plan(self):
        if self._fold is not None:
            return self._fold or None
        if self.nbr_idx is None or self.mesh_batch != 1 or not self.masked or self.n_in > 16384 or self.nbr_cap > 64 \
                or self.n_out < 64:
            self._fold = False
            return None
        if torch.cuda.is_current_stream_capturing():
            return None
        for rows in FOLD_SLAB_ROWS:
            built = self._build_slab_plan(rows)
            if built is None:
                break
            if built[1] <= SLAB_UNION_MAX:
                sp, mu, keep, mc = built
                keys, nkeys = keep[2], keep[3]
                n_slabs = keys.shape[0]
                slot = torch.arange(SLAB_UNION_MAX, device=keys.device, dtype=torch.int64)[None, :].expand(n_slabs, -1)
                valid = slot < nkeys[:, None].long()
                ent = (torch.arange(n_slabs, device=keys.device, dtype=torch.int64)[:, None] * SLAB_UNION_MAX + slot)[valid]
                key = keys.long()[valid]
                order = torch.sort(key, stable=True).indices
                rev_ent = ent[order].to(torch.int32).contiguous()
                rev_ptr = torch.zeros((self.n_in + 1,), device=keys.device, dtype=torch.int64)
                rev_ptr[1:] = torch.cumsum(torch.bincount(key, minlength=self.n_in), 0)
                rev_ptr = rev_ptr.to(torch.int32).contiguous()
                self._fold = (sp, mu, keep + (rev_ptr, rev_ent), mc)
                return self._fold
        self._fold = False
        return None

    def lists_complete(self) -> int:
        if self.nbr_cnt is None or self.mesh_batch != 1:
            return 0
        if self._complete is None:
            if torch.cuda.is_current_stream_capturing():
                return 0
            self._complete = int(bool((self.nbr_cnt <= self.nbr_cap).all().item()))
        return self._complete

    def _build_lists(self, cap: int, reverse: bool = True) -> None:
        dev = self.mesh_out.device
        rows = self.mesh_batch * self.n_out
        L = _lib.lib()
        self.nbr_cap = cap
        self.nbr_idx = torch.empty((rows, cap), device=dev, dtype=torch.int32)
        self.nbr_cnt = torch.empty((rows,), device=dev, dtype=torch.int32)
        work = None
        if reverse:
            self.rev_ptr = torch.empty((self.mesh_batch, self.n_in + 1), device=dev, dtype=torch.int32)
            self.rev_row = torch.empty((self.mesh_batch, self.n_out * cap), device=dev, dtype=torch.int32)
            work = torch.empty((2 * self.mesh_batch * self.n_in,), device=dev, dtype=torch.int32)
        rc = L.pit_plan_fwd(self.mesh_out.data_ptr(), self.mesh_in.data_ptr(), self.mesh_batch, self.n_out,
                            self.n_in, self.sdim, self.metric_id, self.period, self.rank_k, self.stats.data_ptr(), cap,
                            self.nbr_idx.data_ptr(), self.nbr_cnt.data_ptr(), _lib.ptr(self.rev_ptr),
                            _lib.ptr(self.rev_row), _lib.ptr(work), int(PLAN_FLAGS), _lib.stream_ptr())
        _lib.check(rc, "pit_plan_fwd")


def _row_view(t: torch.Tensor) -> torch.Tensor:
    if t.dim() != 3:
        raise RuntimeError(f"expected a (batch, points, channels) tensor, got {tuple(t.shape)}")
    if t.stride(2) != 1 or t.stride(1) < t.shape[2]:
        t = t.contiguous()
    return t


UNION_ATT = os.environ.get("PIT_UNION_ATT", "1") != "0"
SATT = os.environ.get("PIT_SATT", "auto")
SATT_TILES = os.environ.get("PIT_SATT_TILES", "1") != "0"
SATT_FUSE_PREP = os.environ.get("PIT_SATT_FUSE_PREP", "1") != "0"
SATT_DW_RIDER = os.environ.get("PIT_SATT_DW_RIDER", "1") != "0"
WIDE_DW_RIDER = os.environ.get("PIT_WIDE_DW_RIDER", "1") != "0"


def _satt_pays(n_pts: int, n_head: int, d: int) -> bool:
    if SATT == "auto":
        return n_pts >= 256
    return SATT not in ("0", "", False)


def _handoff_x16(values: torch.Tensor):
    x16 = getattr(values, "_pit_x16", None)
    if x16 is None or getattr(values, "_pit_x16_version", None) != values._version:
        return None
    return x16


def _handoff_g16_ready(link, d_out: torch.Tensor, shape) -> bool:
    g16 = link.get("g16") if link is not None else None
    return (g16 is not None and link.get("dx_ptr") == d_out.data_ptr() and link.get("dx_version") == d_out._version
            and tuple(g16.shape) == tuple(shape))


def _union_att_ok(plan: "MeshPlan", n_head: int, d: int, b: int, values: torch.Tensor) -> bool:
    if torch.are_deterministic_algorithms_enabled():
        return False
    if not (plan.mesh_batch == 1 and plan.masked and plan.nbr_idx is not None and not plan.self_attn and n_head in (1, 2)
            and d % 64 == 0 and d >= UNION_ATT_MIN_DIM):
        return False
    if values.stride(1) % 4 or values.stride(0) % 4 or values.data_ptr() % 16:
        return False
    if not _lib.lib().pit_union_att_supported(int(n_head), int(d), int(b), int(plan.n_out)):
        return False
    sp = plan.slab_plan()
    return sp is not None and sp[1] <= SLAB_UNION_MAX


UNION_ATT_MIN_DIM = 128


class _PosAtt(torch.autograd.Function):

    @staticmethod
    def forward(ctx, values, head, plan: MeshPlan, n_head: int, concat: bool, head_is_scale: bool,
                head_param=None, out_slot=None, coord_dims: int = 0, scale_in=None, out_bf16: bool = False, link=None):
        _need_gpu(values, head)
        ctx.math = _math_code()
        out_bf16 = bool(out_bf16 and not concat and plan.nbr_idx is not None and ctx.math == MATH_MODES["bf16"])
        ctx.coord_dims = int(coord_dims)
        ctx.union = ATT_UNION if (plan.masked and plan.nbr_idx is not None and not coord_dims and n_head <= 2
                                  and values.shape[-1] % 8 == 0 and plan.union_tiles()) else 0
        out_buf = out_slot[0].detach() if out_slot else None
        values = _row_view(values)
        b, j, d = values.shape
        d += int(coord_dims)
        if j != plan.n_in:
            raise RuntimeError(f"inputs have {j} points but mesh_in has {plan.n_in}")
        if plan.mesh_batch not in (1, b):
            raise RuntimeError("mesh batch and input batch differ")
        head = head.detach().reshape(-1).contiguous()
        if head.numel() != n_head:
            raise RuntimeError("lmda must hold one value per head")
        ctx.uatt = None
        if UNION_ATT and not concat and not coord_dims and out_buf is None and _union_att_ok(plan, n_head, d, b, values):
            w = _new_decoder_weights(plan, head, scale_in, n_head, head_is_scale, True)
            _launch_decoder_weights(w)
            out = torch.empty((b, plan.n_out, n_head * d), device=values.device, dtype=torch.bfloat16 if out_bf16 else torch.float32)
            sp, max_union = plan.slab_plan()[0], plan.slab_plan()[1]
            rc = _lib.lib().pit_union_att_fwd(ctypes.byref(sp), values.data_ptr(), values.stride(1), values.stride(0), b, n_head, d,
                                              w.pw.data_ptr(), out.data_ptr(), out.stride(1), out.stride(0), 1 if out_bf16 else 0,
                                              max_union, _lib.stream_ptr())
            _lib.check(rc, "pit_union_att_fwd")
            ctx.uatt = w
            ctx.plan, ctx.n_head, ctx.concat, ctx.head_is_scale = plan, n_head, concat, head_is_scale
            ctx.head_param = head_param
            ctx.union = 0
            ctx.save_for_backward(values, head, w.scale, w.scale)
            return out
        ctx.satt = None
        if _satt_pays(int(plan.n_in), int(n_head), int(d)) and concat and not coord_dims and plan.self_attn and not plan.masked and ctx.math == MATH_MODES["bf16"] \
                and values.dtype == torch.float32 and values.stride(1) % 4 == 0 and values.stride(0) % 4 == 0 and values.data_ptr() % 16 == 0 \
                and _lib.lib().pit_satt_supported(int(plan.n_in), int(n_head), int(d), int(b), int(plan.mesh_batch)):
            k_head, k_is_scale = (scale_in, True) if scale_in is not None else (head, head_is_scale)
            out = out_buf if out_buf is not None else torch.empty((b, plan.n_out, (n_head + 1) * d), device=values.device, dtype=torch.float32)
            x16 = link.get("x16") if (link is not None and out_buf is not None) else None
            x16_ready = x16 is not None and tuple(x16.shape) == (b * j, d) and x16.dtype == torch.bfloat16 and x16.is_contiguous()
            if not x16_ready:
                x16 = torch.empty((b, j, d), device=values.device, dtype=torch.bfloat16)
            rowstat = torch.empty((plan.mesh_batch, n_head, plan.n_out, 4), device=values.device, dtype=torch.float32)
            scale = torch.empty((n_head,), device=values.device, dtype=torch.float32)
            et = torch.empty((plan.mesh_batch, n_head, int(_lib.lib().pit_satt_tiles_elems(int(plan.n_in)))), device=values.device,
                             dtype=torch.bfloat16) if SATT_TILES else None
            rc = _lib.lib().pit_satt_fwd(plan.mesh_in.data_ptr(), plan.mesh_batch, plan.n_in, plan.sdim, plan.metric_id, plan.period,
                                         values.data_ptr(), values.stride(1), values.stride(0), b, d, k_head.data_ptr(), n_head,
                                         1 if k_is_scale else 0, x16.data_ptr(), out.data_ptr(), out.stride(1), out.stride(0), d,
                                         1 if out_buf is None else 0, rowstat.data_ptr(), scale.data_ptr(), _lib.ptr(et),
                                         1 if x16_ready else 0, _lib.stream_ptr())
            _lib.check(rc, "pit_satt_fwd")
            ctx.satt = x16
            ctx.satt_tiles = et
            ctx.satt_link = link
            if link is not None:
                link.update(rowstat=rowstat, n_head=n_head, pts=int(j), mesh_batch=int(plan.mesh_batch), dim=int(d), batch=int(b), g16=None,
                            dx_ptr=None, dx_version=None)
            ctx.union = 0
            ctx.plan, ctx.n_head, ctx.concat, ctx.head_is_scale = plan, n_head, concat, head_is_scale
            ctx.head_param = head_param
            ctx.save_for_backward(values, head, rowstat, scale)
            return out
        width = (n_head + (1 if concat else 0)) * d
        copy_inputs = 1 if concat else 0
        if out_buf is not None:
            out, copy_inputs = out_buf, 0
        else:
            out = torch.empty((b, plan.n_out, width), device=values.device,
                              dtype=torch.bfloat16 if out_bf16 else torch.float32)
        rowstat = torch.empty((plan.mesh_batch, n_head, plan.n_out, 4), device=values.device, dtype=torch.float32)
        scale = torch.empty((n_head,), device=values.device, dtype=torch.float32)
        k_head, k_is_scale = (scale_in, True) if scale_in is not None else (head, head_is_scale)
        wjob = getattr(_STEP, "fwd_job", None)
        if wjob is not None:
            _STEP.fwd_job = None
        rc = _lib.lib().pit_posatt_fwd_job(
            plan.mesh_out.data_ptr(), plan.mesh_in.data_ptr(), plan.mesh_batch, plan.n_out, plan.n_in, plan.sdim,
            plan.metric_id, plan.period,
            values.data_ptr(), b, d, values.stride(1), values.stride(0),
# ... 163 lines not shown
    _PARAM_EPOCH[0] += 1


def host_head_scale(lmda: torch.Tensor) -> torch.Tensor:
    key = (lmda._version, lmda.data_ptr(), _PARAM_EPOCH[0], lmda.device.index)
    ent = getattr(lmda, "_pit_host_c", None)
    if ent is None or ent[0] != key:
        if _capturing():
            raise RuntimeError("head-scale route 'host' cannot be captured into a hipGraph for an lmda whose current "
                               "value has no host-evaluated scale yet (that needs a device->host copy): it is exact "
                               "for a FROZEN lmda only - run the step once eagerly with this route first; if an "
                               "optimizer updates lmda every step, capture with the 'device' route")
        HOST_SCALE_EVALUATIONS[0] += 1
        host = lmda.detach().reshape(-1).cpu()
        c = torch.tan(0.25 * math.pi * (1 - 1e-7) * (1.0 + torch.sin(host)))
        ent = (key, c.to(lmda.device))
        lmda._pit_host_c = ent
    if _capturing():
        _HOSTC_CAPTURE["used"] = True
        _HOSTC_CAPTURE["log"].append((lmda, lmda._version))
        _pin(ent[1])
    else:
        _HOSTC_CAPTURE["used"] = False
        _HOSTC_CAPTURE["log"].clear()
    return ent[1]


def assert_frozen_since_capture() -> None:
    log, _HOSTC_CAPTURE["log"] = _HOSTC_CAPTURE["log"], []
    _HOSTC_CAPTURE["used"] = False
    for lmda, version in log:
        if lmda._version != version:
            raise RuntimeError("head-scale route 'host' is exact for a FROZEN lmda only, but the captured step "
                               "modified lmda (an optimizer inside the graph): capture it with the 'device' route")


def _concat_buffer_of(values: torch.Tensor, n_out: int, n_head: int):
    buf = getattr(values, "_pit_concat", None)
    if buf is None:
        return None
    values._pit_concat = None
    b, j, d = values.shape
    w = (1 + n_head) * d
    ok = (buf.dim() == 3 and tuple(buf.shape) == (b, n_out, w) and j == n_out and buf.is_contiguous()
          and values.data_ptr() == buf.data_ptr() and tuple(values.stride()) == (n_out * w, w, 1))
    return buf if ok else None


def tag_coords(func: torch.Tensor, mesh_in: torch.Tensor) -> torch.Tensor:
    out = func.view_as(func)
    out._pit_coords = mesh_in
    return out


def materialize_coords(func: torch.Tensor) -> torch.Tensor:
    mesh = getattr(func, "_pit_coords", None)
    if mesh is None:
        return func
    return torch.cat((mesh.reshape(1, -1, mesh.shape[-1]).expand(func.shape[0], -1, -1), func), -1)


@torch.compiler.disable
def posatt_apply(values: torch.Tensor, lmda: torch.Tensor, plan: MeshPlan, n_head: int, concat: bool,
                 head_is_scale: bool = False, coord_dims: int = 0, out_bf16: bool = False) -> torch.Tensor:
    out_buf = _concat_buffer_of(values, plan.n_out, n_head) if concat else None
    slot = [out_buf] if out_buf is not None else None
    param = lmda if isinstance(lmda, torch.nn.Parameter) else None
    c = host_head_scale(lmda) if (not head_is_scale and get_head_scale_route() == "host") else None
    link = {"x16": _handoff_x16(values)} if concat else None
    out = _PosAtt.apply(values, lmda.reshape(-1), plan, n_head, concat, head_is_scale, param, slot, coord_dims, c,
                        out_bf16, link)
    if link is not None and link.get("rowstat") is not None:
        out._pit_satt = link
    elif concat and plan.self_attn and not plan.masked and plan.nbr_idx is None and not coord_dims:
        out._pit_dense_att = True
    return out


CHAIN_MLP = os.environ.get("PIT_CHAIN_MLP", "1") != "0"


def chain_mlp_supported(rows: int, n0: int, n1: int, n2: int, out_gelu: bool) -> bool:
    return bool(CHAIN_MLP and out_gelu and get_math_mode() == "bf16"
                and _lib.lib().pit_mlp_chain_supported(int(rows), int(n0), int(n1), int(n2)))


def bf16_weights(tensors, new_pass: bool = False):
    cap = _capturing()
    if new_pass:
        _STEP.cap_fresh = set()
    fresh = getattr(_STEP, "cap_fresh", None) if cap else None
    out, need = [], []
    for t in tensors:
        ent = getattr(t, "_pit_bf16", None)
        if ent is None or ent[0].shape != t.shape or ent[0].device != t.device:
            ent = [torch.empty(t.shape, device=t.device, dtype=torch.bfloat16), -1, -1, 0]
            t._pit_bf16 = ent
        if cap:
            _pin(ent[0], t)
            stale = fresh is None or id(t) not in fresh
        else:
            stale = ent[1] != t._version or ent[2] != _PARAM_EPOCH[0] or ent[3] != t.data_ptr()
        if stale:
            need.append((t, ent))
        out.append(ent[0])
    if need:
        n = len(need)
        src = (ctypes.c_void_p * n)(*[t.data_ptr() for t, _e in need])
        dst = (ctypes.c_void_p * n)(*[e[0].data_ptr() for _t, e in need])
        cnt = (ctypes.c_long * n)(*[t.numel() for t, _e in need])
        rc = _lib.lib().pit_cast_bf16_multi(n, src, dst, cnt, _lib.stream_ptr())
        _lib.check(rc, "pit_cast_bf16_multi")
        for t, ent in need:
            if cap:
                ent[1] = ent[2] = -1
                if fresh is None:
                    fresh = _STEP.cap_fresh = set()
                fresh.add(id(t))
            else:
                ent[1], ent[2], ent[3] = t._version, _PARAM_EPOCH[0], t.data_ptr()
    return out


def _chain_weight_ok(w) -> bool:
    return torch.is_tensor(w) and w.is_cuda and w.dtype == torch.float32 and w.is_contiguous() and w.data_ptr() % 16 == 0 \
        and w.numel() % 4 == 0


def prepare_chain_weights(mlps, rows: int) -> None:
    ws = []
    for w1, w2 in mlps:
        n1, n0 = w1.shape
        if w2.shape == (n1, n1) and chain_mlp_supported(rows, n0, n1, n1, True) and _chain_weight_ok(w1) and _chain_weight_ok(w2):
            ws += [w1, w2]
    if ws:
        bf16_weights(ws[:32], new_pass=True)


class _Mlp(torch.autograd.Function):

    @staticmethod
    def forward(ctx, x, w1, b1, w2, b2, out_gelu: bool, concat_heads: int = 0, satt_link=None, y16_slot=None, after_dense_att: bool = False):
        _need_gpu(w1, b1, w2, b2)
        _need_gpu_bf16_ok(x)
        shape = x.shape
        n0 = shape[-1]
        n1, n2 = w1.shape[0], w2.shape[0]
        x16 = x.dtype == torch.bfloat16
        if x16 and (out_gelu or concat_heads > 0 or not mlp_bf16_io_supported(x.numel() // n0, n0, n1, n2)):
            x, x16 = x.float(), False
        x2 = x.reshape(-1, n0)
        if x2.stride(1) != 1 or x2.stride(0) < n0:
            x2 = x2.contiguous()
        rows = x2.shape[0]
        if w1.shape[1] != n0 or w2.shape[1] != n1:
            raise RuntimeError(f"mlp shapes do not chain: x[...,{n0}], w1{tuple(w1.shape)}, w2{tuple(w2.shape)}")
        w1c, b1c, w2c, b2c = (t.detach().contiguous() for t in (w1, b1, w2, b2))
        dev = x.device
        save_dt = torch.bfloat16 if x16 else torch.float32
        z1 = torch.empty((rows, n1), device=dev, dtype=save_dt)
        h = torch.empty((rows, n1), device=dev, dtype=save_dt)
        z2 = torch.empty((rows, n2), device=dev, dtype=torch.float32) if out_gelu else None
        buf = None
        if concat_heads > 0:
            buf = torch.empty((rows, (1 + concat_heads) * n2), device=dev, dtype=torch.float32)
            y = buf[:, :n2]
        else:
            y = torch.empty((rows, n2), device=dev, dtype=torch.float32)
        ctx.math = _math_code() | ((IO_X_BF16 | IO_SAVE_BF16 | IO_DX_BF16) if x16 else 0)
        ctx.x16 = x16
        ctx.chain = None
        if not x16 and chain_mlp_supported(rows, n0, n1, n2, out_gelu) and x2.stride(0) % 4 == 0 and x2.data_ptr() % 16 == 0 \
                and _chain_weight_ok(w1) and _chain_weight_ok(w2):
            w1b, w2b = bf16_weights([w1, w2])
            y16 = torch.empty((rows, n2), device=dev, dtype=torch.bfloat16) if (y16_slot is not None and buf is not None and SATT_FUSE_PREP) else None
            rc = _lib.lib().pit_mlp_chain_fwd(x2.data_ptr(), x2.stride(0), rows, n0, n1, w1b.data_ptr(), b1c.data_ptr(),
                                              w2b.data_ptr(), b2c.data_ptr(), z1.data_ptr(), h.data_ptr(), z2.data_ptr(),
                                              y.data_ptr(), y.stride(0), _lib.ptr(y16), _lib.stream_ptr())
            _lib.check(rc, "pit_mlp_chain_fwd")
            ctx.chain = (w1b, w2b)
            if y16 is not None:
                y16_slot.append(y16)
        else:
            rc = _lib.lib().pit_mlp_fwd(x2.data_ptr(), x2.stride(0), rows, n0, n1, n2, w1c.data_ptr(), b1c.data_ptr(),
                                        w2c.data_ptr(), b2c.data_ptr(), 1 if out_gelu else 0, z1.data_ptr(),
                                        h.data_ptr(), _lib.ptr(z2), y.data_ptr(), y.stride(0), ctx.math & ~IO_DX_BF16,
                                        _lib.stream_ptr())
            _lib.check(rc, "pit_mlp_fwd")
        ctx.out_gelu, ctx.dims, ctx.in_shape = out_gelu, (rows, n0, n1, n2), shape
        ctx.satt_link = satt_link if ctx.chain is not None else None
        ctx.after_dense_att = bool(after_dense_att)
        ctx.params = (w1, b1, w2, b2)
        ctx.save_for_backward(x2, w1c, w2c, z1, h, z2 if out_gelu else z1)
        out = y.reshape(*shape[:-1], n2)
        if buf is None:
            return out
        buf = buf.reshape(*shape[:-1], (1 + concat_heads) * n2)
        ctx.mark_non_differentiable(buf)
        ctx.set_materialize_grads(False)
        return out, buf

    @staticmethod
    def backward(ctx, d_y, _d_buf=None):
        x2, w1, w2, z1, h, z2 = ctx.saved_tensors
        rows, n0, n1, n2 = ctx.dims
        if d_y is None:
            d_y = torch.zeros((rows, n2), device=x2.device, dtype=torch.float32)
        dev = x2.device
        d_y2 = d_y.reshape(rows, n2)
        if d_y2.stride(1) != 1 or d_y2.stride(0) < n2:
            d_y2 = d_y2.contiguous()
        need_x = ctx.needs_input_grad[0]
        d_x = torch.empty((rows, n0), device=dev, dtype=torch.bfloat16 if ctx.x16 else torch.float32) if need_x else None
        slots = [_grad_slot(p) if isinstance(p, torch.nn.Parameter) else None for p in ctx.params]
        inplace = all(s is not None for s in slots) and all(ctx.needs_input_grad[1:5])
        if inplace:
            d_w1, d_b1, d_w2, d_b2 = slots
        else:
            d_w1 = torch.empty((n1, n0), device=dev, dtype=torch.float32)
            d_b1 = torch.empty((n1,), device=dev, dtype=torch.float32)
            d_w2 = torch.empty((n2, n1), device=dev, dtype=torch.float32)
            d_b2 = torch.empty((n2,), device=dev, dtype=torch.float32)
        scratch = torch.empty((rows * (n1 + n2),), device=dev, dtype=torch.float32)
        L = _lib.lib()
        z2p = z2.data_ptr() if ctx.out_gelu else 0
        og = 1 if ctx.out_gelu else 0
        if ctx.chain is not None and d_y2.stride(0) % 4 == 0 and d_y2.data_ptr() % 16 == 0:
            w1b, w2b = ctx.chain
            lk, g16 = ctx.satt_link, None
            if (lk is not None and SATT_FUSE_PREP and d_x is not None and lk.get("rowstat") is not None and lk["dim"] == n1
                    and (1 + lk["n_head"]) * n1 == n0 and lk["batch"] * lk["pts"] == rows):
                g16 = torch.empty((lk["batch"], lk["n_head"], lk["pts"], n1), device=dev, dtype=torch.bfloat16)
            rc = L.pit_mlp_chain_bwd(rows, n0, n1, w1b.data_ptr(), w2b.data_ptr(), z1.data_ptr(), z2p, d_y2.data_ptr(),
                                     d_y2.stride(0), _lib.ptr(d_x), n0, scratch.data_ptr(), _lib.ptr(g16),
                                     lk["rowstat"].data_ptr() if g16 is not None else None, lk["pts"] if g16 is not None else 0,
                                     lk["mesh_batch"] if g16 is not None else 0, _lib.stream_ptr())
            _lib.check(rc, "pit_mlp_chain_bwd")
            if g16 is not None:
                lk["g16"], lk["dx_ptr"], lk["dx_version"] = g16, d_x.data_ptr(), d_x._version
            if lk is not None and inplace and SATT_DW_RIDER and lk.get("rowstat") is not None:
                st = _lib.MlpParamsJob(x2.data_ptr(), x2.stride(0), rows, n0, n1, n2, h.data_ptr(), og, d_y2.data_ptr(),
                                       d_y2.stride(0), d_w1.data_ptr(), d_b1.data_ptr(), d_w2.data_ptr(), d_b2.data_ptr(),
                                       1, scratch.data_ptr(), ctx.math)
                _dw_defer(st, (x2, h, d_y2, scratch, d_w1, d_b1, d_w2, d_b2), dev)
            else:
                rc = L.pit_mlp_bwd_params(x2.data_ptr(), x2.stride(0), rows, n0, n1, n2, h.data_ptr(), og, d_y2.data_ptr(),
                                          d_y2.stride(0), d_w1.data_ptr(), d_b1.data_ptr(), d_w2.data_ptr(), d_b2.data_ptr(),
                                          1 if inplace else 0, scratch.data_ptr(), ctx.math, _lib.stream_ptr())
                _lib.check(rc, "pit_mlp_bwd_params")
        elif MLP_PARAMS_RIDER and inplace and _dw_deferrable(rows, n0, n1, n2, og, d_y2.stride(0)):
            rc = L.pit_mlp_bwd_data(rows, n0, n1, n2, w1.data_ptr(), w2.data_ptr(), z1.data_ptr(), z2p, og,
                                    d_y2.data_ptr(), d_y2.stride(0), _lib.ptr(d_x), n0, scratch.data_ptr(),
                                    ctx.math, _lib.stream_ptr())
            _lib.check(rc, "pit_mlp_bwd_data")
            st = _lib.MlpParamsJob(x2.data_ptr(), x2.stride(0), rows, n0, n1, n2, h.data_ptr(), og, d_y2.data_ptr(),
                                   d_y2.stride(0), d_w1.data_ptr(), d_b1.data_ptr(), d_w2.data_ptr(), d_b2.data_ptr(),
                                   1, scratch.data_ptr(), 0)
            _dw_defer(st, (x2, h, d_y2, scratch, d_w1, d_b1, d_w2, d_b2), dev)
        elif (WIDE_DW_RIDER and inplace and ctx.after_dense_att and not ctx.x16 and rows >= 1024 and n1 >= 128 and n1 % 64 == 0
              and n2 % 64 == 0 and n0 % 64 == 0 and (not og or d_y2.stride(0) == n2)):
            rc = L.pit_mlp_bwd_data(rows, n0, n1, n2, w1.data_ptr(), w2.data_ptr(), z1.data_ptr(), z2p, og,
                                    d_y2.data_ptr(), d_y2.stride(0), _lib.ptr(d_x), n0, scratch.data_ptr(),
                                    ctx.math, _lib.stream_ptr())
            _lib.check(rc, "pit_mlp_bwd_data")
            st = _lib.MlpParamsJob(x2.data_ptr(), x2.stride(0), rows, n0, n1, n2, h.data_ptr(), og, d_y2.data_ptr(),
                                   d_y2.stride(0), d_w1.data_ptr(), d_b1.data_ptr(), d_w2.data_ptr(), d_b2.data_ptr(),
                                   1, scratch.data_ptr(), ctx.math)
            _dw_defer(st, (x2, h, d_y2, scratch, d_w1, d_b1, d_w2, d_b2), dev)
        else:
            small = not ctx.x16 and _dw_deferrable(rows, n0, n1, n2, og, d_y2.stride(0))
            rc = L.pit_mlp_bwd(x2.data_ptr(), x2.stride(0), rows, n0, n1, n2, w1.data_ptr(), w2.data_ptr(),
                               z1.data_ptr(), h.data_ptr(), z2p, og, d_y2.data_ptr(), d_y2.stride(0),
                               _lib.ptr(d_x), n0, d_w1.data_ptr(), d_b1.data_ptr(), d_w2.data_ptr(), d_b2.data_ptr(),
                               1 if inplace else 0, scratch.data_ptr(), 0 if small else ctx.math, _lib.stream_ptr())
            _lib.check(rc, "pit_mlp_bwd")
        dx = d_x.reshape(ctx.in_shape) if need_x else None
        if inplace:
            return dx, None, None, None, None, None, None, None, None, None
        return dx, d_w1, d_b1, d_w2, d_b2, None, None, None, None, None


@torch.compiler.disable
def mlp_apply(x, w1, b1, w2, b2, out_gelu: bool = False, concat_heads: int = 0) -> torch.Tensor:
    link = getattr(x, "_pit_satt", None)
    dense = bool(getattr(x, "_pit_dense_att", False))
    if concat_heads <= 0 or x.dim() != 3:
        return _Mlp.apply(x, w1, b1, w2, b2, out_gelu, 0, link, None, dense)
    y16_slot = []
    y, buf = _Mlp.apply(x, w1, b1, w2, b2, out_gelu, int(concat_heads), link, y16_slot, dense)
    y._pit_concat = buf
    if y16_slot:
        y._pit_x16, y._pit_x16_version = y16_slot[0], y._version
    return y


BLOCK_FUSION = os.environ.get("PIT_BLOCK_FUSION", "1") != "0"
BLOCK_MAX_LAYERS = 16


def block_fusion_supported(n_pts: int, n_head: int, dim: int, batch: int) -> bool:
    return BLOCK_FUSION and bool(_lib.lib().pit_block_supported(int(n_pts), int(n_head), int(dim), int(batch)))


PRE_WEIGHTS = os.environ.get("PIT_PRE_WEIGHTS", "1") != "0"


def pre_weights_supported(n_pts: int, n_head: int, dim: int, batch: int) -> bool:
    return PRE_WEIGHTS and bool(_lib.lib().pit_posatt_pre_supported(int(n_pts), int(n_head), int(dim), int(batch)))


def block_weights(plan: "MeshPlan", lmdas, n_head: int, need_q: bool = True):
    n, L, dev = len(lmdas), plan.n_in, plan.mesh_in.device
    scales = [host_head_scale(p) for p in lmdas] if get_head_scale_route() == "host" else None
    heads = [t.detach().reshape(-1).contiguous() for t in lmdas]
    kheads = scales if scales is not None else heads
    E = torch.empty((n, n_head, L, L), device=dev, dtype=torch.float32)
    Q = torch.empty((n, n_head, L, L), device=dev, dtype=torch.float32) if need_q else None
    inv = torch.empty((n, n_head, L), device=dev, dtype=torch.float32)
    rowstat = torch.empty((n, n_head, L, 4), device=dev, dtype=torch.float32)
    scale = torch.empty((n, n_head), device=dev, dtype=torch.float32)
    for l0 in range(0, n, BLOCK_MAX_LAYERS):
        m = min(BLOCK_MAX_LAYERS, n - l0)
        hp = (ctypes.c_void_p * m)(*[t.data_ptr() for t in kheads[l0:l0 + m]])
        rc = _lib.lib().pit_block_weights(plan.mesh_in.data_ptr(), L, plan.sdim, plan.metric_id, plan.period, m, hp,
                                          1 if scales is not None else 0, n_head, E[l0].data_ptr(),
                                          Q[l0].data_ptr() if Q is not None else None, inv[l0].data_ptr(),
                                          rowstat[l0].data_ptr(), scale[l0].data_ptr(), _lib.stream_ptr())
        _lib.check(rc, "pit_block_weights")
    return E, Q, inv, rowstat, scale, heads


class _PosAttPre(torch.autograd.Function):

    @staticmethod
    def forward(ctx, values, head, e, q, rowstat, scale, n_head: int, head_param, out_slot):
        _need_gpu(values, head)
        b, L, D = values.shape
        W = (1 + n_head) * D
        if values.stride(2) != 1:
            values = values.contiguous()
        given = out_slot[0] if out_slot else None
        out = given if given is not None else torch.empty((b, L, W), device=values.device, dtype=torch.float32)
        ctx.math = _math_code()
        rc = _lib.lib().pit_posatt_pre_fwd(e.data_ptr(), rowstat.data_ptr(), L, n_head, D, b, values.data_ptr(), values.stride(1),
                                           values.stride(0), out.data_ptr(), W, L * W, D, 0 if given is not None else 1,
                                           ctx.math, _lib.stream_ptr())
        _lib.check(rc, "pit_posatt_pre_fwd")
        ctx.n_head, ctx.head_param = n_head, head_param
        ctx.save_for_backward(values, head, e, q, rowstat, scale)
        return out

    @staticmethod
    def backward(ctx, d_out):
        values, head, e, q, rowstat, scale = ctx.saved_tensors
        n_head = ctx.n_head
        b, L, D = values.shape
        d_out = _row_view(d_out)
        if d_out.dtype != torch.float32:
            d_out = d_out.float()
        need_v, need_h = ctx.needs_input_grad[0], ctx.needs_input_grad[1]
        dev = values.device
        d_values = torch.empty((b, L, D), device=dev, dtype=torch.float32)
        slot = _grad_slot(ctx.head_param) if need_h else None
        defer = DEFER_HEAD_FINISH and slot is not None
        work = None
        if need_h:
            if q is None:
                raise RuntimeError("d(lmda) needs the d(scale) weights: block_weights(..., need_q=True)")
            if defer:
                work = _layer_workspace(slot, n_head)
                _defer_head_begin(work)
            else:
                work = torch.zeros(n_head * 1024, device=dev, dtype=torch.float64)
        rider = _dw_take(dev)
        if rider is not None:
            _dw_run(rider)
        rc = _lib.lib().pit_posatt_pre_bwd(e.data_ptr(), _lib.ptr(q), rowstat.data_ptr(), L, n_head, D, b, values.data_ptr(),
                                           values.stride(1), values.stride(0), d_out.data_ptr(), d_out.stride(1), d_out.stride(0),
                                           D, d_values.data_ptr(), D, L * D, 1, _lib.ptr(work), ctx.math, _lib.stream_ptr())
        _lib.check(rc, "pit_posatt_pre_bwd")
        d_head = None
        if need_h:
            if defer:
                _defer_head_finish(work, slot, head, scale, n_head, 1)
            else:
                d_head = slot if slot is not None else torch.empty((n_head,), device=dev, dtype=torch.float32)
                one = lambda t: (ctypes.c_void_p * 1)(t.data_ptr())
                _lib.check(_lib.lib().pit_posatt_dhead_finish(1, one(work), one(d_head), one(head), one(scale), (ctypes.c_int * 1)(n_head),
                                                              (ctypes.c_int * 1)(1 if slot is not None else 0), None, _lib.stream_ptr()),
                           "pit_posatt_dhead_finish")
                if slot is not None:
                    d_head = None
        return (d_values if need_v else None), d_head, None, None, None, None, None, None, None


@torch.compiler.disable
def posatt_pre_apply(values: torch.Tensor, lmda: torch.Tensor, weights, layer: int, n_head: int) -> torch.Tensor:
    E, Q, _inv, rowstat, scale, _heads = weights
    out_buf = _concat_buffer_of(values, values.shape[1], n_head)
    slot = [out_buf] if out_buf is not None else None
    param = lmda if isinstance(lmda, torch.nn.Parameter) else None
    return _PosAttPre.apply(values, lmda.reshape(-1), E[layer], Q[layer] if Q is not None else None, rowstat[layer], scale[layer],
                            n_head, param, slot)


EARLY_WEIGHTS = os.environ.get("PIT_EARLY_WEIGHTS", "rider")


class EarlyWeights:
    __slots__ = ("key", "E", "Q", "inv", "rowstat", "scale", "job", "keep")

    def join(self) -> None:
        if getattr(_STEP, "fwd_job", None) is self:
            _STEP.fwd_job = None
            j = self.job
            rc = _lib.lib().pit_block_weights(j.mesh, j.n_pts, j.space_dim, j.metric, j.period, j.n_layers, j.heads,
                                              j.head_is_scale, j.n_head, j.e, j.q, j.inv, j.rowstat, j.scale_out,
                                              _lib.stream_ptr())
            _lib.check(rc, "pit_block_weights")


def drop_forward_job(early) -> None:
    if early is not None and getattr(_STEP, "fwd_job", None) is early:
        _STEP.fwd_job = None
    _STEP.dec_job = None


def _weights_key(plan: MeshPlan, lmdas, scales, n_head: int):
    return (id(plan), n_head, _PARAM_EPOCH[0], scales is not None,
            tuple((p._version, p.data_ptr()) for p in lmdas), tuple(t.data_ptr() for t in scales) if scales is not None else None)


def _weights_buffers(plan: MeshPlan, n: int, n_head: int, need_q: bool):
    L, dev = plan.n_in, plan.mesh_in.device
    E = torch.empty((n, n_head, L, L), device=dev, dtype=torch.float32)
    Q = torch.empty((n, n_head, L, L), device=dev, dtype=torch.float32) if need_q else None
    inv = torch.empty((n, n_head, L), device=dev, dtype=torch.float32)
    rowstat = torch.empty((n, n_head, L, 4), device=dev, dtype=torch.float32)
    scale = torch.empty((n, n_head), device=dev, dtype=torch.float32)
    return E, Q, inv, rowstat, scale


def _launch_block_weights(plan: MeshPlan, kheads, is_scale: bool, n_head: int, need_q: bool, stream_ptr):
    n = len(kheads)
    E, Q, inv, rowstat, scale = _weights_buffers(plan, n, n_head, need_q)
    hp = (ctypes.c_void_p * n)(*[t.data_ptr() for t in kheads])
    rc = _lib.lib().pit_block_weights(plan.mesh_in.data_ptr(), plan.n_in, plan.sdim, plan.metric_id, plan.period, n, hp,
                                      1 if is_scale else 0, n_head, E.data_ptr(), _lib.ptr(Q), inv.data_ptr(),
                                      rowstat.data_ptr(), scale.data_ptr(), stream_ptr)
    _lib.check(rc, "pit_block_weights")
    return E, Q, inv, rowstat, scale


def early_block_weights(plan: MeshPlan, lmdas, n_head: int, need_q: bool):
    if EARLY_WEIGHTS != "rider" or not plan.mesh_in.is_cuda:
        return None
    scales = [host_head_scale(p) for p in lmdas] if get_head_scale_route() == "host" else None
    heads = [t.detach().reshape(-1).contiguous() for t in lmdas]
    kheads = scales if scales is not None else heads
    ew = EarlyWeights()
    ew.key = _weights_key(plan, lmdas, scales, n_head)
    ew.job = ew.keep = None
    n = len(kheads)
    ew.E, ew.Q, ew.inv, ew.rowstat, ew.scale = _weights_buffers(plan, n, n_head, need_q)
    hp = (ctypes.c_void_p * n)(*[t.data_ptr() for t in kheads])
    ew.keep = (hp, kheads, plan)
    ew.job = _lib.BlockWeightsJob(plan.mesh_in.data_ptr(), plan.n_in, plan.sdim, plan.metric_id, plan.period, n,
                                  ctypes.cast(hp, ctypes.c_void_p), 1 if scales is not None else 0, n_head,
                                  ew.E.data_ptr(), _lib.ptr(ew.Q), ew.inv.data_ptr(), ew.rowstat.data_ptr(), ew.scale.data_ptr())
    _STEP.fwd_job = ew
    return ew


class _Processor(torch.autograd.Function):

    @staticmethod
    def forward(ctx, x, plan: MeshPlan, n_head: int, scales, params, early, *tensors):
        n = len(tensors) // 5
        lmdas, mlps = tensors[:n], [tensors[n + 4 * i:n + 4 * i + 4] for i in range(n)]
        _need_gpu(x, *tensors)
        b, L, D = x.shape
        H, W, rows = n_head, (1 + n_head) * D, b * L
        dev = x.device
        L_ = _lib.lib()
        ctx.math = 0
        heads = [t.detach().reshape(-1).contiguous() for t in lmdas]
        kheads = list(scales) if scales is not None else heads
        need_q = any(ctx.needs_input_grad)
        if early is not None and early.key == _weights_key(plan, params[0], scales, H) and (early.Q is not None or not need_q):
            E, Q, inv, rowstat, scale = early.E, early.Q, early.inv, early.rowstat, early.scale
        else:
            E, Q, inv, rowstat, scale = _launch_block_weights(plan, kheads, scales is not None, H, need_q, _lib.stream_ptr())
        buf0 = _concat_buffer_of(x, L, H)
        if buf0 is None:
            buf0 = torch.empty((b, L, W), device=dev, dtype=torch.float32)
            buf0[:, :, :D].copy_(x.detach())
        else:
            buf0 = buf0.detach()
        bufs = [buf0] + [torch.empty((b, L, W), device=dev, dtype=torch.float32) for _ in range(n - 1)]
        out = torch.empty((b, L, D), device=dev, dtype=torch.float32)
        z1 = torch.empty((n, rows, D), device=dev, dtype=torch.float32)
        hh = torch.empty((n, rows, D), device=dev, dtype=torch.float32)
        z2 = torch.empty((n, rows, D), device=dev, dtype=torch.float32)
        wts = [tuple(t.detach().contiguous() for t in m) for m in mlps]
        for i in range(n):
            w1, b1, w2, b2 = wts[i]
            if tuple(w1.shape) != (D, W) or tuple(w2.shape) != (D, D):
                raise RuntimeError(f"fused processor: block {i} MLP is {tuple(w1.shape)} / {tuple(w2.shape)}, expected "
                                   f"({D}, {W}) / ({D}, {D})")
        for i in range(n):
            y, ldy = (bufs[i + 1], W) if i + 1 < n else (out, D)
            w1, b1, w2, b2 = wts[i]
            rc = L_.pit_block_fwd(E[i].data_ptr(), inv[i].data_ptr(), L, H, D, b, bufs[i].data_ptr(), w1.data_ptr(),
                                  b1.data_ptr(), w2.data_ptr(), b2.data_ptr(), 1, z1[i].data_ptr(), hh[i].data_ptr(),
                                  z2[i].data_ptr(), y.data_ptr(), ldy, ctx.math, _lib.stream_ptr())
            _lib.check(rc, "pit_block_fwd")
        ctx.n, ctx.H, ctx.dims, ctx.plan = n, H, (b, L, D), plan
        ctx.params = params
        ctx.hook = _processor_hook()
        ctx.keep = (bufs, wts, heads, E, Q, inv, scale, z1, hh, z2)
        return out

    @staticmethod
    def backward(ctx, d_out):
        n, H = ctx.n, ctx.H
        b, L, D = ctx.dims
        W, rows = (1 + H) * D, b * L
        bufs, wts, heads, E, Q, inv, scale, z1, hh, z2 = ctx.keep
        lm_params, mlp_params = ctx.params
        dev = d_out.device
        L_ = _lib.lib()
        d_out = d_out.contiguous()
        dxc = [torch.empty((b, L, W), device=dev, dtype=torch.float32) for _ in range(n)]
        scratch = [torch.empty((rows * 2 * D,), device=dev, dtype=torch.float32) for _ in range(n)]
        dx = torch.empty((b, L, D), device=dev, dtype=torch.float32)
        lm_slots = [_grad_slot(p) if isinstance(p, torch.nn.Parameter) else None for p in lm_params]
        w_slots, w_grads = [], []
        for i in range(n):
            sl = [_grad_slot(p) if isinstance(p, torch.nn.Parameter) else None for p in mlp_params[i]]
            if all(s is not None for s in sl):
                w_slots.append(sl)
                w_grads.append(None)
            else:
                g = [torch.zeros_like(t) for t in wts[i]]
                w_slots.append(g)
                w_grads.append(g)
        defer = [DEFER_HEAD_FINISH and s is not None for s in lm_slots]
        work = []
        for i in range(n):
            if defer[i]:
                ws = _layer_workspace(lm_slots[i], H)
                _defer_head_begin(ws)
            else:
                ws = torch.zeros(H * 1024, device=dev, dtype=torch.float64)
            work.append(ws)
        extra = _dw_take(dev)
        slices = []
        if extra is not None:
            st = extra[0]
            if not st.out_gelu and st.accumulate and (st.math_mode & 0xff) == 0:
                slices = _dw_slices(extra, n if ctx.hook is None else max(1, n - ctx.hook[1]))
            else:
                _dw_run(extra)
        w1, _, w2, _ = wts[n - 1]
        rc = L_.pit_mlp_bwd_data(rows, W, D, D, w1.data_ptr(), w2.data_ptr(), z1[n - 1].data_ptr(), z2[n - 1].data_ptr(), 1,
                                 d_out.data_ptr(), D, dxc[n - 1].data_ptr(), W, scratch[n - 1].data_ptr(), ctx.math,
                                 _lib.stream_ptr())
        _lib.check(rc, "pit_mlp_bwd_data")
        for i in range(n - 1, -1, -1):
            dw1, db1, dw2, db2 = w_slots[i]
            job = _lib.MlpParamsJob(bufs[i].data_ptr(), W, rows, W, D, D, hh[i].data_ptr(), 1, scratch[i].data_ptr(), D,
                                    dw1.data_ptr(), db1.data_ptr(), dw2.data_ptr(), db2.data_ptr(), 1,
                                    scratch[i].data_ptr(), ctx.math)
            if i > 0:
                pw1, _, pw2, _ = wts[i - 1]
                prev = (pw1.data_ptr(), pw2.data_ptr(), z1[i - 1].data_ptr(), z2[i - 1].data_ptr(), 1, W,
                        dxc[i - 1].data_ptr(), W, scratch[i - 1].data_ptr(), None, 0)
            else:
                prev = (None, None, None, None, 0, 0, None, 0, None, dx.data_ptr(), D)
            k = n - 1 - i
            job2 = ctypes.cast(ctypes.pointer(slices[k]), ctypes.c_void_p) if k < len(slices) else None
            rc = L_.pit_block_bwd(E[i].data_ptr(), inv[i].data_ptr(), Q[i].data_ptr(), L, H, D, b, dxc[i].data_ptr(),
                                  bufs[i].data_ptr(), work[i].data_ptr(), *prev,
                                  ctypes.cast(ctypes.pointer(job), ctypes.c_void_p), job2, ctx.math,
                                  _lib.stream_ptr())
            _lib.check(rc, "pit_block_bwd")
            if ctx.hook is not None:
                ctx.hook[0](i)
        d_heads = [None] * n
        now = [i for i in range(n) if not defer[i]]
        for i in range(n):
            if defer[i]:
                _defer_head_finish(work[i], lm_slots[i], heads[i], scale[i], H, 1)
        if now:
            m = len(now)
            for i in now:
                d_heads[i] = lm_slots[i] if lm_slots[i] is not None else torch.empty((H,), device=dev, dtype=torch.float32)
            ws = (ctypes.c_void_p * m)(*[work[i].data_ptr() for i in now])
            dh = (ctypes.c_void_p * m)(*[d_heads[i].data_ptr() for i in now])
            hd = (ctypes.c_void_p * m)(*[heads[i].data_ptr() for i in now])
            sc = (ctypes.c_void_p * m)(*[scale[i].data_ptr() for i in now])
            nh = (ctypes.c_int * m)(*[H] * m)
            fl = (ctypes.c_int * m)(*[1 if lm_slots[i] is not None else 0 for i in now])
            _lib.check(L_.pit_posatt_dhead_finish(m, ws, dh, hd, sc, nh, fl, None, _lib.stream_ptr()), "pit_posatt_dhead_finish")
        grads = [dx, None, None, None, None, None]
        for i in range(n):
            g = None if lm_slots[i] is not None else d_heads[i]
            grads.append(g)
        for i in range(n):
            grads.extend(w_grads[i] if w_grads[i] is not None else [None, None, None, None])
        return tuple(grads)




@torch.compiler.disable
def processor_apply(x: torch.Tensor, plan: MeshPlan, n_head: int, lmdas, mlps, early=None) -> torch.Tensor:
    scales = None
    if get_head_scale_route() == "host":
        scales = [host_head_scale(p) for p in lmdas]
    flat = [p.reshape(-1) for p in lmdas] + [t for m in mlps for t in m]
    return _Processor.apply(x, plan, n_head, scales, (tuple(lmdas), tuple(tuple(m) for m in mlps)), early, *flat)


EDGE_FUSION = os.environ.get("PIT_EDGE_FUSION", "1") != "0"


def edge_fusion_supported(plan: MeshPlan, n_head: int, dim: int, batch: int, needs_union: bool) -> bool:
    if not EDGE_FUSION or plan.mesh_batch != 1 or plan.self_attn or not plan.masked or plan.nbr_idx is None:
        return False
    if needs_union and torch.are_deterministic_algorithms_enabled():
        return False
    if not _lib.lib().pit_edge_supported(int(n_head), int(dim), int(batch), int(plan.n_out)):
        return False
    sp = plan.slab_plan()
    return sp is not None and (not needs_union or sp[1] <= SLAB_UNION_MAX)


def _finish_heads_now(work, d_head, head, scale, n_head: int, flags: int) -> None:
    one = lambda t: (ctypes.c_void_p * 1)(_lib.ptr(t))
    rc = _lib.lib().pit_posatt_dhead_finish(1, one(work), one(d_head), one(head), one(scale), (ctypes.c_int * 1)(n_head),
                                            (ctypes.c_int * 1)(flags), None, _lib.stream_ptr())
    _lib.check(rc, "pit_posatt_dhead_finish")


def _mlp_grad_slots(params, shapes, needs, device):
    slots = [_grad_slot(p) if isinstance(p, torch.nn.Parameter) else None for p in params]
    if all(s is not None for s in slots) and all(needs):
        return slots, True
    return [torch.zeros(tuple(sh), device=device, dtype=torch.float32) for sh in shapes], False


class LossSpec:
    __slots__ = ("true", "scale", "shift", "p", "out_dim", "seed", "partials", "pred", "token", "value")

    def __init__(self, true, scale, shift, out_dim: int, p: int, seed=None):
        b = true.size(0)
        self.true = true.reshape(b, -1, out_dim).contiguous()
        npts = self.true.shape[1]
        self.scale = scale.reshape(npts, out_dim).contiguous() if scale is not None else None
        self.shift = shift.reshape(npts, out_dim).contiguous() if shift is not None else None
        self.p, self.out_dim, self.seed = int(p), int(out_dim), seed
        self.partials = self.pred = self.token = self.value = None

    def fits(self, batch: int, npts: int, n2: int) -> bool:
        return self.p in (1, 2) and n2 == self.out_dim and tuple(self.true.shape) == (batch, npts, n2) and not self.true.requires_grad


class DecoderWeights:
    __slots__ = ("key", "pw", "qw", "scale", "job", "keep", "w1f")


def _dec_weights_key(plan: MeshPlan, lmda, scale_in, n_head: int, head_is_scale: bool, w1=None):
    return (id(plan), n_head, _PARAM_EPOCH[0], lmda._version, lmda.data_ptr(), bool(head_is_scale),
            scale_in.data_ptr() if scale_in is not None else None,
            (w1.data_ptr(), w1._version, tuple(w1.shape)) if w1 is not None else None)


def _new_decoder_weights(plan: MeshPlan, lmda, scale_in, n_head: int, head_is_scale: bool, need_q: bool, w1=None) -> DecoderWeights:
    sp, max_union, _t, max_count = plan.slab_plan()
    um = 32 if max_union <= 32 else (48 if max_union <= 48 else 64)
    dev = plan.mesh_out.device
    w = DecoderWeights()
    w.key = _dec_weights_key(plan, lmda, scale_in, n_head, head_is_scale, w1)
    w1c = w1.detach() if (w1 is not None and w1.is_contiguous() and w1.dtype == torch.float32 and w1.dim() == 2
                          and w1.shape[0] % 16 == 0 and w1.shape[1] == n_head * w1.shape[0] and w1.data_ptr() % 16 == 0) else None
    w.w1f = torch.empty_like(w1c) if w1c is not None else None
    w.pw = torch.empty((sp.n_slabs, n_head, 16, um), device=dev, dtype=torch.float32)
    w.qw = torch.empty((sp.n_slabs, n_head, 16, um), device=dev, dtype=torch.float32) if need_q else None
    w.scale = torch.empty((n_head,), device=dev, dtype=torch.float32)
    head = scale_in if scale_in is not None else lmda.detach().reshape(-1).contiguous()
    w.keep = (head, plan, sp, w1c)
    w.job = _lib.DecoderWeightsJob(ctypes.cast(ctypes.pointer(sp), ctypes.c_void_p), head.data_ptr(),
                                   1 if (scale_in is not None or head_is_scale) else 0, n_head, max_union, max_count,
                                   w.pw.data_ptr(), _lib.ptr(w.qw), w.scale.data_ptr(),
                                   _lib.ptr(w1c), _lib.ptr(w.w1f), w1c.shape[0] if w1c is not None else 0)
    return w


def _launch_decoder_weights(w: DecoderWeights) -> None:
    j = w.job
    rc = _lib.lib().pit_decoder_weights(j.plan, j.head, j.head_is_scale, j.n_head, j.max_union, j.max_count, j.pw, j.qw,
                                        j.scale_out, j.w1, j.w1f, j.dim, _lib.stream_ptr())
    _lib.check(rc, "pit_decoder_weights")


def early_decoder_weights(plan: MeshPlan, lmda, n_head: int, need_q: bool, w1=None) -> None:
    scale_in = host_head_scale(lmda) if get_head_scale_route() == "host" else None
    _STEP.dec_job = _new_decoder_weights(plan, lmda, scale_in, n_head, False, need_q, w1)
    _STEP.dec_ready = None


class _Decoder(torch.autograd.Function):

    @staticmethod
    def forward(ctx, values, head, plan: MeshPlan, n_head: int, head_is_scale: bool, head_param, weights, params, loss, w1, b1, w2, b2):
        _need_gpu(values, head, w1, b1, w2, b2)
        values = _row_view(values)
        if values.stride(1) % 4 or values.stride(0) % 4 or values.data_ptr() % 16:
            values = values.contiguous()
        b, j, d = values.shape
        n2 = w2.shape[0]
        dev = values.device
        sp = plan.slab_plan()[0]
        head = head.detach().reshape(-1).contiguous()
        w1c, b1c, w2c, b2c = (t.detach().contiguous() for t in (w1, b1, w2, b2))
        rows = b * plan.n_out
        need = weights.qw is not None
        y = torch.empty((b, plan.n_out, n2), device=dev, dtype=torch.float32)
        x = z1 = h = dvals = None
        if need:
            x = torch.empty((rows, n_head * d), device=dev, dtype=torch.float32)
            z1 = torch.empty((rows, d), device=dev, dtype=torch.float32)
            h = torch.empty((rows, d), device=dev, dtype=torch.float32)
            dvals = torch.empty((b, j, d), device=dev, dtype=torch.float32)
        lt = ls = lh = lpart = None
        lp = 0
        if loss is not None and need:
            lt, ls, lh, lp = loss.true, loss.scale, loss.shift, loss.p
            lpart = loss.partials = torch.empty((b, n2, sp.n_slabs, 2), device=dev, dtype=torch.float64)
            loss.value = torch.empty((), device=dev, dtype=torch.float32)
        w1f = weights.w1f if (weights.w1f is not None and weights.keep[3].data_ptr() == w1c.data_ptr()) else None
        rc = _lib.lib().pit_decoder_fwd(ctypes.byref(sp), values.data_ptr(), values.stride(1), values.stride(0), b, n_head, d,
                                        weights.pw.data_ptr(), w1c.data_ptr(), _lib.ptr(w1f), b1c.data_ptr(), w2c.data_ptr(),
                                        b2c.data_ptr(), n2, _lib.ptr(x), _lib.ptr(z1), _lib.ptr(h), y.data_ptr(),
                                        _lib.ptr(dvals), dvals.numel() if dvals is not None else 0,
                                        _lib.ptr(lt), _lib.ptr(ls), _lib.ptr(lh), lp, _lib.ptr(lpart), plan.slab_plan()[1],
                                        _lib.stream_ptr())
        _lib.check(rc, "pit_decoder_fwd")
        ctx.plan, ctx.n_head, ctx.head_is_scale, ctx.head_param, ctx.params = plan, n_head, head_is_scale, head_param, params
        ctx.loss = loss if lpart is not None else None
        if ctx.loss is not None:
            loss.pred = y
        ctx.dvals_clean = True
        ctx.keep = (values, head, w1c, w2c, x, z1, h, weights, dvals)
        return y

    @staticmethod
    def backward(ctx, d_y):
        values, head, w1, w2, x, z1, h, weights, dvals = ctx.keep
        scale = weights.scale
        plan, n_head = ctx.plan, ctx.n_head
        b, j, d = values.shape
        n2, rows = w2.shape[0], b * plan.n_out
        dev = values.device
        sp = plan.slab_plan()[0]
        loss = ctx.loss
        inside = loss is not None and loss.token is not None and d_y.data_ptr() == loss.token.data_ptr()
        if loss is not None and loss.token is not None and not inside:
            raise RuntimeError("the fused loss's gradient token reached pit.decoder's backward as a copy: the prediction must reach "
                               "the loss through views only (engine.TrainStep)")
        if not ctx.dvals_clean:
            dvals.zero_()
        ctx.dvals_clean = False
        dz1 = torch.empty((rows, d), device=dev, dtype=torch.float32)
        if inside:
            d_pred = torch.empty((rows, n2), device=dev, dtype=torch.float32)
            dyp, ld = None, n2
        else:
            d_pred = d_y.reshape(rows, n2)
            if d_pred.stride(1) != 1 or d_pred.stride(0) < n2:
                d_pred = d_pred.contiguous()
            dyp, ld = d_pred, d_pred.stride(0)
        need_h = ctx.needs_input_grad[1]
        slot = _grad_slot(ctx.head_param) if need_h else None
        defer = DEFER_HEAD_FINISH and slot is not None
        work = None
        if need_h:
            work = _layer_workspace(slot, n_head) if defer else torch.zeros(n_head * 1024, device=dev, dtype=torch.float64)
            if defer:
                _defer_head_begin(work)
        L = _lib.lib()
        rc = L.pit_decoder_bwd(ctypes.byref(sp), values.data_ptr(), values.stride(1), values.stride(0), b, n_head, d,
                               weights.pw.data_ptr(), weights.qw.data_ptr(), w1.data_ptr(), w2.data_ptr(), n2, z1.data_ptr(),
                               _lib.ptr(dyp), ld, dz1.data_ptr(), dvals.data_ptr(), dvals.stride(0), _lib.ptr(work),
                               loss.pred.data_ptr() if inside else None, _lib.ptr(loss.true) if inside else None,
                               _lib.ptr(loss.scale) if inside else None, _lib.ptr(loss.shift) if inside else None,
                               _lib.ptr(loss.seed) if inside else None, loss.p if inside else 0,
                               _lib.ptr(loss.partials) if inside else None, d_pred.data_ptr() if inside else None,
                               loss.value.data_ptr() if inside else None, None, plan.slab_plan()[1], _lib.stream_ptr())
        _lib.check(rc, "pit_decoder_bwd")
        d_head = None
        if need_h:
            flags = 1 | (4 if ctx.head_is_scale else 0)
            if defer:
                _defer_head_finish(work, slot, head, scale, n_head, flags)
            else:
                d_head = slot if slot is not None else torch.empty((n_head,), device=dev, dtype=torch.float32)
                _finish_heads_now(work, d_head, head, scale, n_head, flags if slot is not None else flags & ~1)
                if slot is not None:
                    d_head = None
        grads, inplace = _mlp_grad_slots(ctx.params, (w1.shape, (d,), w2.shape, (n2,)), ctx.needs_input_grad[9:13], dev)
        d_w1, d_b1, d_w2, d_b2 = grads
        st = _lib.MlpParamsJob(x.data_ptr(), x.stride(0), rows, n_head * d, d, n2, h.data_ptr(), 0, d_pred.data_ptr(),
                               d_pred.stride(0), d_w1.data_ptr(), d_b1.data_ptr(), d_w2.data_ptr(), d_b2.data_ptr(), 1,
                               dz1.data_ptr(), 0)
        keep = (x, h, d_pred, dz1, d_w1, d_b1, d_w2, d_b2)
        if inplace and MLP_PARAMS_RIDER and _dw_deferrable(rows, n_head * d, d, n2, 0, d_pred.stride(0)):
            _dw_defer(st, keep, dev)
        else:
            _dw_run((st, keep, torch.cuda.current_stream(dev)))
        dv = dvals if ctx.needs_input_grad[0] else None
        w = (None, None, None, None) if inplace else (d_w1, d_b1, d_w2, d_b2)
        return (dv, d_head, None, None, None, None, None, None, None) + w


@torch.compiler.disable
def decoder_apply(values: torch.Tensor, lmda: torch.Tensor, plan: MeshPlan, n_head: int, mlp, head_is_scale: bool = False) -> torch.Tensor:
    param = lmda if isinstance(lmda, torch.nn.Parameter) else None
    c = host_head_scale(lmda) if (not head_is_scale and get_head_scale_route() == "host") else None
    need_q = torch.is_grad_enabled() and (values.requires_grad or lmda.requires_grad or any(t.requires_grad for t in mlp))
    weights = getattr(_STEP, "dec_ready", None)
    _STEP.dec_ready = None
    if weights is None or weights.key != _dec_weights_key(plan, lmda, c, n_head, head_is_scale, mlp[0]) or (need_q and weights.qw is None):
        weights = _new_decoder_weights(plan, lmda, c, n_head, head_is_scale, need_q, mlp[0])
        _launch_decoder_weights(weights)
    loss = getattr(_STEP, "loss", None)
    if loss is not None:
        _STEP.loss = None
        if not loss.fits(values.shape[0], plan.n_out, mlp[2].shape[0]):
            loss = None
        else:
            _STEP.loss_issued = loss
    return _Decoder.apply(values, lmda.reshape(-1), plan, n_head, head_is_scale, param, weights, tuple(mlp), loss, *mlp)


FOLD_DECODER = os.environ.get("PIT_FOLD_DECODER", "1") != "0"
FOLD_TILES = os.environ.get("PIT_FOLD_TILES", "auto")
FOLD_TILES_MAX_BYTES = 64 << 20


def _fold_tiles(nbytes: int) -> bool:
    if FOLD_TILES in ("0", False):
        return False
    return FOLD_TILES in ("1", True) or nbytes <= FOLD_TILES_MAX_BYTES or torch.are_deterministic_algorithms_enabled()
FOLD_EDGE_ROWS = int(os.environ.get("PIT_FOLD_EDGE_ROWS", "300000"))
_ZERO_BIAS = {}


def _zero_bias(n: int, device) -> torch.Tensor:
    key = (device.index, n)
    z = _ZERO_BIAS.get(key)
    if z is None:
        z = _ZERO_BIAS[key] = torch.zeros((n,), device=device, dtype=torch.float32)
        _pin(z)
    return z


def _rows2d(t: torch.Tensor) -> torch.Tensor:
    t = _row_view(t)
    if t.stride(0) != t.shape[1] * t.stride(1) or t.stride(1) % 4 or t.data_ptr() % 16:
        t = t.contiguous()
    return t


class _Linear(torch.autograd.Function):

    @staticmethod
    def forward(ctx, x, w, w_param):
        _need_gpu(x, w)
        x = _rows2d(x)
        b, j, d = x.shape
        wc = w.detach()
        if not wc.is_contiguous() or wc.data_ptr() % 16:
            wc = wc.contiguous()
        n_out = wc.numel() // d
        y = torch.empty((b, j, n_out), device=x.device, dtype=torch.float32)
        ctx.math = _math_code()
        rc = _lib.lib().pit_linear_fwd(x.data_ptr(), x.stride(1), b * j, d, n_out, wc.data_ptr(), _zero_bias(n_out, x.device).data_ptr(),
# ... 554 lines not shown
```

Baseline: 55150 samples/s.

## Use separable tensor-grid attention for processor blocks on structured latent meshes

```diff
diff --git a/include/pit_hip.h b/include/pit_hip.h
--- a/include/pit_hip.h
+++ b/include/pit_hip.h
@@ -5,7 +5,7 @@
 extern "C" {
 #endif
 
-#define PIT_ABI_VERSION 23
+#define PIT_ABI_VERSION 24
 #define PIT_DSCALE_SLOTS 1024
 
 #define PIT_METRIC_EUCLID     0
@@ -116,6 +116,20 @@
                   float* d_values, long ld_dvalues,
                   const struct pit_mlp_params_job* rider, const struct pit_mlp_params_job* rider2,
                   int math_mode, void* stream);
+
+int pit_block_sep_supported(int nx, int ny, int n_head, int dim, int batch);
+int pit_block_sep_fwd(const float* xs, const float* ys, int nx, int ny, int metric, float period, const float* head,
+                      int head_is_scale, int n_head, int dim, int batch, float* xcat,
+                      const float* w1, const float* b1, const float* w2, const float* b2, int out_gelu,
+                      float* z1, float* h, float* z2, float* y, long ldy, float* scale_out, float* tables,
+                      int math_mode, void* stream);
+int pit_block_sep_bwd(const float* tables, int nx, int ny, int n_head, int dim, int batch,
+                      const float* d_xcat, const float* xcat, double* dscale,
+                      const float* w1, const float* w2, const float* z1, const float* z2, int out_gelu, int n0_prev,
+                      float* d_xprev, long ld_dxprev, float* scratch_prev,
+                      float* d_values, long ld_dvalues,
+                      const struct pit_mlp_params_job* rider, const struct pit_mlp_params_job* rider2,
+                      int math_mode, void* stream);
 
 #define PIT_SLAB_UNION_MAX 64
 typedef struct pit_slab_plan {
diff --git a/position_induced_transformer_amd/_lib.py b/position_induced_transformer_amd/_lib.py
--- a/position_induced_transformer_amd/_lib.py
+++ b/position_induced_transformer_amd/_lib.py
@@ -100,6 +100,10 @@
     "pit_posatt_pre_fwd": [_P, _P, _I, _I, _I, _I, _P, _L, _L, _P, _L, _L, _I, _I, _I, _P],
     "pit_posatt_pre_bwd": [_P, _P, _P, _I, _I, _I, _I, _P, _L, _L, _P, _L, _L, _I, _P, _L, _L, _I, _P, _I, _P],
     "pit_block_bwd": [_P, _P, _P, _I, _I, _I, _I, _P, _P, _P, _P, _P, _P, _P, _I, _I, _P, _L, _P, _P, _L, _P, _P, _I, _P],
+    "pit_block_sep_supported": [_I, _I, _I, _I, _I],
+    "pit_block_sep_fwd": [_P, _P, _I, _I, _I, _F, _P, _I, _I, _I, _I, _P, _P, _P, _P, _P, _I, _P, _P, _P, _P, _L, _P, _P, _I,
+                          _P],
+    "pit_block_sep_bwd": [_P, _I, _I, _I, _I, _I, _P, _P, _P, _P, _P, _P, _P, _I, _I, _P, _L, _P, _P, _L, _P, _P, _I, _P],
     "pit_mlp_bf16_io_supported": [_I, _I, _I, _I, _I],
     "pit_mlp_fwd": [_P, _L, _I, _I, _I, _I, _P, _P, _P, _P, _I, _P, _P, _P, _P, _L, _I, _P],
     "pit_mlp_bwd": [_P, _L, _I, _I, _I, _I, _P, _P, _P, _P, _P, _I, _P, _L,
@@ -118,7 +122,7 @@
 }
 
 LONG_RETURN = {"pit_satt_tiles_elems"}
-ABI_VERSION = 23
+ABI_VERSION = 24
 
 _lib = None
 
diff --git a/position_induced_transformer_amd/csrc/pit_block.hip b/position_induced_transformer_amd/csrc/pit_block.hip
--- a/position_induced_transformer_amd/csrc/pit_block.hip
+++ b/position_induced_transformer_amd/csrc/pit_block.hip
@@ -89,6 +89,325 @@
     return slab_of_xcd(id, batch, slabs, sample, slab);
 }
 
+struct SepGrid {
+    const float *xs, *ys;
+    int nx, ny, periodic; float period;
+    const float* head; int head_is_scale;
+    float* scale_out;
+    float* tab;
+    int tab_wg;
+};
+constexpr int SEP_MAX = 32;
+constexpr int SEP_SP = BD + 4;
+
+template <int H>
+__device__ __forceinline__ void sep_scales(const SepGrid& sg, float (&c)[H]) {
+#pragma unroll
+    for (int h = 0; h < H; ++h) c[h] = sg.head_is_scale ? sg.head[h] : head_scale_from_lmda(sg.head[h]);
+}
+
+__device__ __forceinline__ int sep_lnx(int nx) { return nx == 32 ? 5 : 4; }
+
+template <int H, bool FULL>
+struct SepEntry {
+    bool isx, valid; int h, row, col;
+    __device__ __forceinline__ SepEntry(int e, int nx, int ny) {
+        const int lnxr = FULL ? sep_lnx(nx) : 4, nxr = 1 << lnxr, nex = H * nxr * 32;
+        isx = e < nex;
+        const int r = isx ? e : e - nex, hr = r >> 5;
+        col = r & 31;
+        if (isx) { h = hr >> lnxr; row = hr & (nxr - 1); }
+        else if (FULL) { h = hr / ny; row = hr - h * ny; }
+        else { h = hr; row = 0; }
+        valid = col < (isx ? nx : ny) && h < H;
+    }
+};
+template <bool FULL>
+__host__ __device__ inline int sep_entries(int H, int nx, int ny) { return H * 32 * (FULL ? nx + ny : 16 + 1); }
+
+template <int H, int TQ, bool FULL>
+__device__ __forceinline__ void sep_coords(const SepGrid& sg, int xr0, int yr0, float (&ca)[TQ], float (&cb)[TQ]) {
+    const int nx = sg.nx, ny = sg.ny, ne = sep_entries<FULL>(H, nx, ny);
+#pragma unroll
+    for (int i = 0; i < TQ; ++i) {
+        const SepEntry<H, FULL> t(min((int)threadIdx.x + 64 * BW * i, ne - 1), nx, ny);
+        const float* co = t.isx ? sg.xs : sg.ys;
+        ca[i] = co[(t.isx ? xr0 : yr0) + t.row];
+        cb[i] = co[min(t.col, (t.isx ? nx : ny) - 1)];
+    }
+}
+
+template <int H, int TQ, bool FULL>
+__device__ __forceinline__ void sep_tables(const SepGrid& sg, const float (&c)[H], const float (&ca)[TQ], const float (&cb)[TQ],
+                                           float* ex, float* ey, float* mx, float* my, float* st) {
+    const int nx = sg.nx, ny = sg.ny, EPX = nx + 1, EPY = ny + 1, ne = sep_entries<FULL>(H, nx, ny);
+    const int nxr = FULL ? nx : 16, nyr = FULL ? ny : 1;
+    const bool want_m = mx != nullptr;
+#pragma unroll
+    for (int i = 0; i < TQ; ++i) {
+        const int e = threadIdx.x + 64 * BW * i;
+        const SepEntry<H, FULL> t(min(e, ne - 1), nx, ny);
+        if (e >= ne || !t.valid) continue;
+        float d = __fsub_rn(ca[i], cb[i]);
+        if (sg.periodic) { d = fabsf(d); d = fminf(d, __fsub_rn(sg.period, d)); }
+        const float m = __fmul_rn(d, d);
+        const float ev = __expf(-__fmul_rn(m, t.h == 0 ? c[0] : c[H - 1]));
+        const int off = t.isx ? (t.h * nxr + t.row) * EPX + t.col : (t.h * nyr + t.row) * EPY + t.col;
+        (t.isx ? ex : ey)[off] = ev;
+        if (want_m) (t.isx ? mx : my)[off] = m;
+    }
+    __syncthreads();
+    float *invx = st, *invy = invx + H * nxr, *mbx = invy + H * nyr, *mby = mbx + H * nxr;
+    for (int q = threadIdx.x; q < H * (nxr + nyr); q += 64 * BW) {
+        const int h = q / (nxr + nyr);
+        int row = q - h * (nxr + nyr);
+        const bool isx = row < nxr;
+        if (!isx) row -= nxr;
+        const int n = isx ? nx : ny;
+        const int off = isx ? (h * nxr + row) * EPX : (h * nyr + row) * EPY;
+        const float* e = (isx ? ex : ey) + off;
+        const float* mm = want_m ? (isx ? mx : my) + off : nullptr;
+        float s = 0.0f, sm = 0.0f;
+#pragma unroll 16
+        for (int k = 0; k < n; ++k) {
+            s += e[k];
+            if (want_m) sm += e[k] * mm[k];
+        }
+        const float inv = s > 0.0f ? 1.0f / s : 0.0f;
+        (isx ? invx : invy)[isx ? h * nxr + row : h * nyr + row] = inv;
+        if (want_m) (isx ? mbx : mby)[isx ? h * nxr + row : h * nyr + row] = sm * inv;
+    }
+    __syncthreads();
+}
+
+__host__ __device__ inline int sep_table_floats(int H, int nx, int ny, int nxr, int nyr, bool m) {
+    return (m ? 2 : 1) * H * (nxr * (nx + 1) + nyr * (ny + 1)) + 2 * H * (nxr + nyr);
+}
+__host__ __device__ inline int up4(int n) { return (n + 3) & ~3; }
+__host__ __device__ inline int sep_parts(int groups) { return groups >= 64 * BW ? 1 : (64 * BW) / groups; }
+__host__ __device__ inline int sep_fwd_floats(int H, int nx, int ny) {
+    return up4(sep_parts(nx * 16) * H * nx * SEP_SP) + sep_table_floats(H, nx, ny, 16, 1, false);
+}
+__host__ __device__ inline int sep_bwd_floats(int H, int nx, int ny) {
+    return up4(sep_parts(H * nx * 16) * 2 * H * nx * SEP_SP) + 2 * 16 * SEP_SP + 2 * BW * 2 + 2 * H * (16 * (nx + 1) + ny);
+}
+__host__ __device__ inline int sep_tab_floats(int H, int nx, int ny) { return H * 2 * (nx * nx + ny * ny); }
+
+template <int H>
+__device__ __forceinline__ void sep_write_tables(const SepGrid& sg, float* sm) {
+    const int nx = sg.nx, ny = sg.ny, EPX = nx + 1, EPY = ny + 1;
+    float* ex = sm;
+    float* ey = ex + H * nx * EPX;
+    float* mx = ey + H * ny * EPY;
+    float* my = mx + H * nx * EPX;
+    float* st = my + H * ny * EPY;
+    const float *invx = st, *invy = invx + H * nx, *mbx = invy + H * ny, *mby = mbx + H * nx;
+    constexpr int TQ = (H * 32 * 2 * SEP_MAX + 64 * BW - 1) / (64 * BW);
+    float ca[TQ], cb[TQ];
+    sep_coords<H, TQ, true>(sg, 0, 0, ca, cb);
+    float c[H];
+    sep_scales<H>(sg, c);
+    sep_tables<H, TQ, true>(sg, c, ca, cb, ex, ey, mx, my, st);
+    const int per_h = 2 * (nx * nx + ny * ny);
+    for (int q = threadIdx.x; q < H * per_h; q += 64 * BW) {
+        const int h = q / per_h;
+        int r = q - h * per_h;
+        const bool isx = r < 2 * nx * nx;
+        if (!isx) r -= 2 * nx * nx;
+        const int n = isx ? nx : ny, which = r / (n * n), a = (r / n) % n, k = r % n;
+        const int off = isx ? (h * nx + a) * EPX + k : (h * ny + a) * EPY + k;
+        const float w = (isx ? ex : ey)[off] * (isx ? invx[h * nx + k] : invy[h * ny + k]);
+        sg.tab[q] = which == 0 ? w : w * ((isx ? mx : my)[off] - (isx ? mbx[h * nx + k] : mby[h * ny + k]));
+    }
+}
+
+template <int H, int XP>
+__device__ __forceinline__ void sep_fwd_attention(const SepGrid& sg, const float* xcat, float* xcat_out,
+                                                  int L, int b, int n0, long m0, float* sm, float* xs) {
+    constexpr int W = (1 + H) * BD;
+    const int tid = threadIdx.x, lane = tid & 63, wave = tid >> 6, l15 = lane & 15, kq = lane >> 4;
+    const int nx = sg.nx, ny = sg.ny, lnx = sep_lnx(nx), iy = n0 >> lnx, ix0 = n0 & (nx - 1);
+    const int NG = nx * 16, P = sep_parts(NG), lpp = P == 1 ? ny : (ny + 1) >> 1;
+    float* sp = sm;
+    float* ex = sm + up4(P * H * nx * SEP_SP);
+    float* ey = ex + H * 16 * (nx + 1);
+    float* st = ey + H * (ny + 1);
+    const float *invx = st, *invy = invx + H * 16;
+    const int grp = tid & (NG - 1), part = tid >> (lnx + 4), jx = grp >> 4, d4 = grp & 15;
+    const int lb = part * lpp, le = min(ny, lb + lpp);
+    const float* xp = xcat + ((long)b * L + jx) * W + 4 * d4;
+    const long lstep = (long)nx * W;
+    constexpr int TQ = (H * 32 * 17 + 64 * BW - 1) / (64 * BW);
+    float ca[TQ], cb[TQ];
+    sep_coords<H, TQ, false>(sg, ix0, iy, ca, cb);
+    float4 xv[8];
+#pragma unroll
+    for (int u = 0; u < 8; ++u) xv[u] = *reinterpret_cast<const float4*>(xp + min(lb + u, ny - 1) * lstep);
+    float c[H];
+    sep_scales<H>(sg, c);
+    if (sg.scale_out && blockIdx.x == 0 && tid < H) sg.scale_out[tid] = tid == 0 ? c[0] : c[H - 1];
+    sep_tables<H, TQ, false>(sg, c, ca, cb, ex, ey, nullptr, nullptr, st);
+    float4 s[H];
+#pragma unroll
+    for (int h = 0; h < H; ++h) s[h] = make_float4(0.f, 0.f, 0.f, 0.f);
+    for (int j0 = lb; j0 < le; j0 += 8) {
+        if (j0 != lb) {
+#pragma unroll
+            for (int u = 0; u < 8; ++u) xv[u] = *reinterpret_cast<const float4*>(xp + min(j0 + u, ny - 1) * lstep);
+        }
+#pragma unroll
+        for (int u = 0; u < 8; ++u) {
+            if (j0 + u >= le) break;
+#pragma unroll
+            for (int h = 0; h < H; ++h) {
+                const float w = ey[h * (ny + 1) + j0 + u] * invy[h];
+                s[h].x += w * xv[u].x; s[h].y += w * xv[u].y; s[h].z += w * xv[u].z; s[h].w += w * xv[u].w;
+            }
+        }
+    }
+#pragma unroll
+    for (int h = 0; h < H; ++h) *reinterpret_cast<float4*>(sp + ((part * H + h) * nx + jx) * SEP_SP + 4 * d4) = s[h];
+    __syncthreads();
+    if (wave < 4 * H) {
+        const int h = wave >> 2, t = wave & 3;
+        const float ai = invx[h * 16 + l15];
+        f32x4_t acc = {0.f, 0.f, 0.f, 0.f};
+#pragma unroll 4
+        for (int k = kq; k < nx; k += 4) {
+            float bsum = 0.0f;
+            for (int p = 0; p < P; ++p) bsum += sp[((p * H + h) * nx + k) * SEP_SP + 16 * t + l15];
+            acc = mfma_16x16x4(ex[(h * 16 + l15) * (nx + 1) + k] * ai, bsum, acc);
+        }
+        const int col = BD + h * BD + 16 * t + l15;
+#pragma unroll
+        for (int i = 0; i < 4; ++i) {
+            const int r = 4 * kq + i;
+            xs[r * XP + col] = acc[i];
+            xcat_out[(m0 + r) * W + col] = acc[i];
+        }
+    }
+}
+
+template <int H, typename Mid>
+__device__ __forceinline__ void sep_bwd_attention(const SepGrid& sg, const float* __restrict__ d_xcat, const float* __restrict__ xcat,
+                                                  bool dscale, int L, int b, int j0, long m0, float* sm, float*& dvs, double*& wred,
+                                                  Mid&& mid) {
+    constexpr int W = (1 + H) * BD;
+    const int tid = threadIdx.x, lane = tid & 63, wave = tid >> 6, l15 = lane & 15, kq = lane >> 4;
+    const int nx = sg.nx, ny = sg.ny, lnx = sep_lnx(nx), jy = j0 >> lnx, jx0 = j0 & (nx - 1), EPX = nx + 1;
+    const int lng = (H == 2 ? 1 : 0) + lnx + 4, NG = 1 << lng, P = sep_parts(NG), lpp = P == 1 ? ny : (ny + 1) >> 1;
+    float* tp = sm;
+    dvs = tp + up4(P * 2 * H * nx * SEP_SP);
+    wred = reinterpret_cast<double*>(dvs + 2 * 16 * SEP_SP);
+    float* ad = dvs + 2 * 16 * SEP_SP + 2 * BW * 2;
+    float* wv = ad + 2 * H * 16 * EPX;
+    const long lstep = (long)nx * W;
+    const int nq = NG * P;
+    auto group_of = [nx, lnx, lng, lpp, ny](int q, int& h, int& ix, int& d4, int& lb, int& le) {
+        const int grp = q & ((1 << lng) - 1), part = q >> lng;
+        h = grp >> (lnx + 4); ix = (grp >> 4) & (nx - 1); d4 = grp & 15;
+        lb = part * lpp; le = min(ny, lb + lpp);
+    };
+    const int per_h = 2 * (nx * nx + ny * ny), nm = dscale ? 2 : 1, n_ad = nm * H * 16 * 32, n_all = n_ad + nm * H * 32;
+    constexpr int TQ = (2 * H * 17 * 32 + 64 * BW - 1) / (64 * BW);
+    float tv[TQ];
+    int tdst[TQ];
+#pragma unroll
+    for (int i = 0; i < TQ; ++i) {
+        const int e = min(tid + 64 * BW * i, n_all - 1);
+        const bool isx = e < n_ad;
+        const int r = isx ? e : e - n_ad, k = r & 31, row = r >> 5;
+        const int mh = isx ? row >> 4 : row, m = H == 2 ? mh >> 1 : mh, h = H == 2 ? (mh & 1) : 0;
+        const int src = isx ? h * per_h + m * nx * nx + (jx0 + (row & 15)) * nx + min(k, nx - 1)
+                            : h * per_h + 2 * nx * nx + m * ny * ny + jy * ny + min(k, ny - 1);
+        tdst[i] = (tid + 64 * BW * i >= n_all || k >= (isx ? nx : ny)) ? -1 : (isx ? row * EPX + k : 2 * H * 16 * EPX + mh * ny + k);
+        tv[i] = sg.tab[src];
+    }
+    constexpr int LC = 16;
+    float4 v[LC];
+    {
+        int h, ix, d4, lb, le;
+        group_of(tid, h, ix, d4, lb, le);
+        const float* gp = d_xcat + ((long)b * L + ix) * W + BD + h * BD + 4 * d4;
+#pragma unroll
+        for (int u = 0; u < LC; ++u) v[u] = *reinterpret_cast<const float4*>(gp + min(lb + u, ny - 1) * lstep);
+    }
+#pragma unroll
+    for (int i = 0; i < TQ; ++i)
+        if (tdst[i] >= 0) ad[tdst[i]] = tv[i];
+    float xq[4];
+    const float* xsrc = xcat ? xcat : d_xcat;
+#pragma unroll
+    for (int i = 0; i < 4; ++i) xq[i] = xsrc[(m0 + 4 * kq + i) * W + 16 * (wave & 3) + l15];
+    __syncthreads();
+    for (int q = tid; q < nq; q += 64 * BW) {
+        int h, ix, d4, lb, le;
+        group_of(q, h, ix, d4, lb, le);
+        const float* gp = d_xcat + ((long)b * L + ix) * W + BD + h * BD + 4 * d4;
+        const float* w = wv + h * ny;
+        const float* w2 = wv + (H + h) * ny;
+        float4 t = make_float4(0.f, 0.f, 0.f, 0.f), t2 = t;
+        for (int i0 = lb; i0 < le; i0 += LC) {
+            if (q != tid || i0 != lb) {
+#pragma unroll
+                for (int u = 0; u < LC; ++u) v[u] = *reinterpret_cast<const float4*>(gp + min(i0 + u, ny - 1) * lstep);
+            }
+#pragma unroll
+            for (int u = 0; u < LC; ++u) {
+                if (i0 + u >= le) break;
+                const float wu = w[i0 + u];
+                t.x += wu * v[u].x; t.y += wu * v[u].y; t.z += wu * v[u].z; t.w += wu * v[u].w;
+                if (dscale) {
+                    const float wq = w2[i0 + u];
+                    t2.x += wq * v[u].x; t2.y += wq * v[u].y; t2.z += wq * v[u].z; t2.w += wq * v[u].w;
+                }
+            }
+        }
+        const int part = q / NG;
+        *reinterpret_cast<float4*>(tp + (((part * 2 + 0) * H + h) * nx + ix) * SEP_SP + 4 * d4) = t;
+        if (dscale) *reinterpret_cast<float4*>(tp + (((part * 2 + 1) * H + h) * nx + ix) * SEP_SP + 4 * d4) = t2;
+    }
+    mid();
+    __syncthreads();
+    auto tsum = [&](int which, int h, int k, int col) {
+        float v = 0.0f;
+        for (int p = 0; p < P; ++p) v += tp[(((p * 2 + which) * H + h) * nx + k) * SEP_SP + col];
+        return v;
+    };
+    double part[2] = {0.0, 0.0};
+    if (wave < 4 * H) {
+        f32x4_t acc = {0.f, 0.f, 0.f, 0.f};
+        const int tile = (dscale ? 4 : 0) + wave;
+        if (!dscale) {
+            const int h = wave >> 2, col = 16 * (wave & 3) + l15;
+#pragma unroll 4
+            for (int k = kq; k < nx; k += 4)
+                acc = mfma_16x16x4(ad[(h * 16 + l15) * EPX + k], tsum(0, h, k, col), acc);
+#pragma unroll
+            for (int i = 0; i < 4; ++i) dvs[(h * 16 + 4 * kq + i) * SEP_SP + col] = acc[i];
+        } else {
+            const int h = (tile - 4) >> 2, col = 16 * ((tile - 4) & 3) + l15;
+#pragma unroll 4
+            for (int k = kq; k < nx; k += 4) {
+                const int a = (h * 16 + l15) * EPX + k;
+                acc = mfma_16x16x4(ad[H * 16 * EPX + a], tsum(0, h, k, col), acc);
+                acc = mfma_16x16x4(ad[a], tsum(1, h, k, col), acc);
+            }
+            double d = 0.0;
+#pragma unroll
+            for (int i = 0; i < 4; ++i) d += (double)acc[i] * (double)xq[i];
+            if (h == 0) part[0] -= d; else part[1] -= d;
+        }
+    }
+    if (dscale) {
+#pragma unroll
+        for (int h = 0; h < H; ++h) {
+            const double v = wave_sum_d(part[h]);
+            if (lane == 0) wred[wave * 2 + h] = v;
+        }
+    }
+}
+
 struct BlockFwdArgs {
     const float *e, *inv;
     int L, batch;
@@ -96,9 +415,10 @@
     const float *w1, *b1, *w2, *b2;
     int out_gelu;
     float *z1, *h, *z2, *y; long ldy;
+    SepGrid sg;
 };
 
-template <int H, bool WLDS>
+template <int H, bool WLDS, bool SEP>
 __global__ __launch_bounds__(512, WLDS ? 1 : 2) void block_fwd_kernel(BlockFwdArgs g) {
     constexpr int W = (1 + H) * BD;
     constexpr int XP = W + 4, HP = BD + 4;
@@ -113,6 +433,9 @@
     const int tid = threadIdx.x, lane = tid & 63, wave = tid >> 6;
     const int l15 = lane & 15, kq = lane >> 4;
     const int slabs = g.L / 16;
+    if constexpr (SEP) {
+        if ((int)blockIdx.x == g.sg.tab_wg) { sep_write_tables<H>(g.sg, pk); return; }
+    }
     int b, slab;
     if (!slab_of(blockIdx.x, g.batch, slabs, b, slab)) return;
     const int n0 = slab * 16;
@@ -121,7 +444,7 @@
 
     float4 xown = make_float4(0.f, 0.f, 0.f, 0.f);
     if (tid < 256) xown = *reinterpret_cast<const float4*>(g.xcat + (m0 + (tid >> 4)) * W + 4 * (tid & 15));
-    const float rinv0 = g.inv[(long)((tid >> 8) % H) * g.L + n0 + 4 * ((tid & 63) >> 4) + ((tid >> 6) & 3)];
+    const float rinv0 = SEP ? 0.0f : g.inv[(long)((tid >> 8) % H) * g.L + n0 + 4 * ((tid & 63) >> 4) + ((tid >> 6) & 3)];
 
     BSTAMP(0);
     const bool mlp_wave = wave < 4;
@@ -147,6 +470,11 @@
         for (int p = 0; p < NW2; ++p) wq2[p] = reinterpret_cast<const f32x4_t*>(g.w2)[p * 512 + tid];
         load_weights();
     }
+    if constexpr (SEP) {
+        sep_fwd_attention<H, XP>(g.sg, g.xcat, g.xcat, g.L, b, n0, m0, pk, xs);
+        if (!WLDS) load_weights();
+        if (tid < 256) *reinterpret_cast<float4*>(xs + (tid >> 4) * XP + 4 * (tid & 15)) = xown;
+    } else {
     f32x4_t acc[H][4];
 #pragma unroll
     for (int hh = 0; hh < H; ++hh)
@@ -210,6 +538,7 @@
         s.x *= rinv; s.y *= rinv; s.z *= rinv; s.w *= rinv;
         *reinterpret_cast<float4*>(xs + r * XP + BD + hh * BD + col) = s;
         *reinterpret_cast<float4*>(g.xcat + (m0 + r) * W + BD + hh * BD + col) = s;
+    }
     }
     if (WLDS) {
 #pragma unroll
@@ -285,14 +614,36 @@
     float *dz1, *dz2;
     float* d_values; long ld_dvalues;
     int n_chain, n_ds;
+    SepGrid sg;
 };
 
-template <int H>
+__device__ __forceinline__ void load_mlp_operands(const BlockBwdArgs& g, int wave, int kq, int l15, int c1, long m0, float (&w2v)[4][4],
+                                                  float (&z1v)[4], float (&w1v)[2][4][4]) {
+    if (wave < 4) {
+#pragma unroll
+        for (int s = 0; s < 4; ++s)
+#pragma unroll
+            for (int ee = 0; ee < 4; ++ee) w2v[s][ee] = g.w2[(long)(16 * s + 4 * kq + ee) * BD + c1];
+#pragma unroll
+        for (int i = 0; i < 4; ++i) z1v[i] = g.z1[(m0 + 4 * kq + i) * BD + c1];
+    }
+#pragma unroll
+    for (int t = 0; t < 2; ++t) {
+        const int col = (wave + t * BW) * 16 + l15;
+#pragma unroll
+        for (int s = 0; s < 4; ++s)
+#pragma unroll
+            for (int ee = 0; ee < 4; ++ee)
+                w1v[t][s][ee] = (col < g.n0p) ? g.w1[(long)(16 * s + 4 * kq + ee) * g.n0p + col] : 0.0f;
+    }
+}
+
+template <int H, bool SEP>
 __device__ __forceinline__ void block_bwd_chain(const BlockBwdArgs& g, float* smem, int slab) {
     constexpr int W = (1 + H) * BD;
     constexpr int P1 = BD + 4;
     float* pk = smem;
-    float* ds2 = smem + PARK_FLOATS;
+    float* ds2 = smem + (SEP ? sep_bwd_floats(H, g.sg.nx, g.sg.ny) : PARK_FLOATS);
     float* ds1 = ds2 + 16 * P1;
     const int tid = threadIdx.x, lane = tid & 63, wave = tid >> 6;
     const int l15 = lane & 15, kq = lane >> 4;
@@ -311,14 +662,21 @@
     if (has_mlp && g.out_gelu) z2v = *reinterpret_cast<const float2*>(g.z2 + (m0 + orow) * BD + ocol);
     const int c1 = (wave & 3) * 16 + l15;
     BSTAMP(10);
+    float w2v[4][4], z1v[4], w1v[2][4][4];
     f32x4_t acc[1][4];
+    float* dvs = nullptr;
+    double* wred = nullptr;
+    if constexpr (SEP) {
+        sep_bwd_attention<H>(g.sg, g.d_xcat, g.xcat, false, g.L, b, j0, m0, smem, dvs, wred,
+                             [&] { if (has_mlp) load_mlp_operands(g, wave, kq, l15, c1, m0, w2v, z1v, w1v); });
+    } else {
 #pragma unroll
     for (int t = 0; t < 4; ++t) acc[0][t] = f32x4_t{0.f, 0.f, 0.f, 0.f};
     slab_contract<H, false>(g.e + (long)j0 * g.L, (long)g.L * g.L, g.L, g.d_xcat + (long)b * g.L * W + BD, W, BD, g.inv,
                             wave * klen, (wave + 1) * klen, l15, kq, acc);
+    }
     BSTAMP(11);
-    float w2v[4][4], z1v[4], w1v[2][4][4];
-    if (has_mlp) {
+    if (!SEP && has_mlp) {
         if (wave < 4) {
 #pragma unroll
             for (int s = 0; s < 4; ++s)
@@ -337,15 +695,23 @@
                     w1v[t][s][ee] = (col < g.n0p) ? g.w1[(long)(16 * s + 4 * kq + ee) * g.n0p + col] : 0.0f;
         }
     }
-    park(pk, wave, lane, acc[0]);
+    if constexpr (!SEP) park(pk, wave, lane, acc[0]);
     __syncthreads();
     BSTAMP(12);
     {
         float2 s = res;
+        if constexpr (SEP) {
+#pragma unroll
+            for (int h = 0; h < H; ++h) {
+                s.x += dvs[(h * 16 + orow) * SEP_SP + ocol];
+                s.y += dvs[(h * 16 + orow) * SEP_SP + ocol + 1];
+            }
+        } else {
 #pragma unroll
         for (int w = 0; w < BW; ++w) {
             s.x += pk[((w * 4 + 2 * oh) * 4 + oi) * 64 + oln];
             s.y += pk[((w * 4 + 2 * oh + 1) * 4 + oi) * 64 + oln];
+        }
         }
         if (!has_mlp) {
             *reinterpret_cast<float2*>(g.d_values + (m0 + orow) * g.ld_dvalues + ocol) = s;
@@ -451,14 +817,35 @@
     }
 }
 
-template <int H, int NDW>
+template <int H>
+__device__ __forceinline__ void block_bwd_sep_dscale(const BlockBwdArgs& g, float* smem, int slab) {
+    const int slabs = g.L / 16;
+    int b, sl;
+    if (!slab_of(slab, g.batch, slabs, b, sl)) return;
+    const long m0 = ((long)b * slabs + sl) * 16;
+    float* dvs;
+    double* wred;
+    sep_bwd_attention<H>(g.sg, g.d_xcat, g.xcat, true, g.L, b, sl * 16, m0, smem, dvs, wred, [] {});
+    __syncthreads();
+    if (threadIdx.x < H) {
+        double tot = 0.0;
+        for (int w = 0; w < BW; ++w) tot += wred[w * 2 + threadIdx.x];
+        atomicAdd(g.dscale + (long)threadIdx.x * PIT_DSCALE_SLOTS + ((int)(m0 >> 4) & (PIT_DSCALE_SLOTS - 1)), tot);
+    }
+}
+
+template <int H, int NDW, bool SEP>
 __global__ __launch_bounds__(512) void block_bwd_kernel(BlockBwdArgs g, pit_detail::DwPair w, pit_detail::DwPair w2) {
     extern __shared__ __attribute__((aligned(16))) float smem[];
     int id = blockIdx.x;
     BREC(0);
-    if (id < g.n_chain) { block_bwd_chain<H>(g, smem, id); BREC(1); return; }
+    if (id < g.n_chain) { block_bwd_chain<H, SEP>(g, smem, id); BREC(1); return; }
     id -= g.n_chain;
-    if (id < g.n_ds) { block_bwd_dscale<H>(g, smem, id); BREC(1); return; }
+    if (id < g.n_ds) {
+        if constexpr (SEP) block_bwd_sep_dscale<H>(g, smem, id); else block_bwd_dscale<H>(g, smem, id);
+        BREC(1);
+        return;
+    }
     id -= g.n_ds;
     if (PIT_BLOCK_EXP & 32) return;
     if (NDW >= 1 && id < w.n1 + w.n2) { dw_pair_body(w, id, smem); BREC(1); return; }
@@ -496,37 +883,86 @@
     return 0;
 }
 
-extern "C" int pit_block_fwd(const float* e, const float* inv, int n_pts, int n_head, int dim, int batch, float* xcat,
-                             const float* w1, const float* b1, const float* w2, const float* b2, int out_gelu,
-                             float* z1, float* h, float* z2, float* y, long ldy, int math_mode, void* stream) {
-    if (!e || !inv || !xcat || !w1 || !b1 || !w2 || !b2 || !z1 || !h || !y || (out_gelu && !z2)) return PIT_ERR_NULL;
+namespace {
+int fill_fwd_args(BlockFwdArgs& g, int n_pts, int n_head, int dim, int batch, float* xcat, const float* w1, const float* b1,
+                  const float* w2, const float* b2, int out_gelu, float* z1, float* h, float* z2, float* y, long ldy, int math_mode) {
+    if (!xcat || !w1 || !b1 || !w2 || !b2 || !z1 || !h || !y || (out_gelu && !z2)) return PIT_ERR_NULL;
     if (math_mode != PIT_MATH_FP32 || !pit_block_supported(n_pts, n_head, dim, batch)) return PIT_ERR_UNSUPPORTED;
-    if (ldy < dim || !aligned16(e) || !aligned16(xcat) || !aligned16(w1) || !aligned16(w2)) return PIT_ERR_SIZE;
-    BlockFwdArgs g;
-    g.e = e; g.inv = inv; g.L = n_pts; g.batch = batch; g.xcat = xcat;
+    if (ldy < dim || !aligned16(xcat) || !aligned16(w1) || !aligned16(w2)) return PIT_ERR_SIZE;
+    g = BlockFwdArgs();
+    g.L = n_pts; g.batch = batch; g.xcat = xcat;
     g.w1 = w1; g.b1 = b1; g.w2 = w2; g.b2 = b2; g.out_gelu = out_gelu;
     g.z1 = z1; g.h = h; g.z2 = z2; g.y = y; g.ldy = ldy;
-    const dim3 grid((unsigned)slab_grid(batch, n_pts / 16)), block(64 * BW);
+    return 0;
+}
+
+template <bool SEP>
+int launch_block_fwd(const BlockFwdArgs& g, int n_head, int batch, int n_pts, void* stream) {
+    const int n_slab_wgs = slab_grid(batch, n_pts / 16);
+    const dim3 grid((unsigned)(n_slab_wgs + (SEP && g.sg.tab_wg >= 0 ? 1 : 0))), block(64 * BW);
     static const bool no_wlds = getenv("PIT_NO_BLOCK_WLDS") != nullptr;
     static const int n_cus = [] {
         int dev = 0, cus = 0;
         if (hipGetDevice(&dev) != hipSuccess || hipDeviceGetAttribute(&cus, hipDeviceAttributeMultiprocessorCount, dev) != hipSuccess) cus = 0;
         return cus;
     }();
-    const bool earlyw = !no_wlds && (int)grid.x <= n_cus;
+    const bool earlyw = !no_wlds && n_slab_wgs <= n_cus;
     const size_t FWD_SMEM = fwd_smem(n_head, earlyw);
 #define PIT_BLOCK_FWD(H_, E_)                                                                                              \
     do {                                                                                                                   \
-        static bool once = ((void)hipFuncSetAttribute((const void*)block_fwd_kernel<H_, E_>,                              \
+        static bool once = ((void)hipFuncSetAttribute((const void*)block_fwd_kernel<H_, E_, SEP>,                         \
                                                 hipFuncAttributeMaxDynamicSharedMemorySize, 160 * 1024), true);            \
         (void)once;                                                                                                        \
-        hipLaunchKernelGGL((block_fwd_kernel<H_, E_>), grid, block, FWD_SMEM, (hipStream_t)stream, g);                     \
+        hipLaunchKernelGGL((block_fwd_kernel<H_, E_, SEP>), grid, block, FWD_SMEM, (hipStream_t)stream, g);                \
     } while (0)
     if (n_head == 1) { if (earlyw) PIT_BLOCK_FWD(1, true); else PIT_BLOCK_FWD(1, false); }
     else { if (earlyw) PIT_BLOCK_FWD(2, true); else PIT_BLOCK_FWD(2, false); }
 #undef PIT_BLOCK_FWD
     PIT_CHECK_LAUNCH();
     return 0;
+}
+
+int fill_sep_grid(SepGrid& sg, const float* xs, const float* ys, int nx, int ny, int metric, float period, const float* head,
+                  int head_is_scale, int n_head, int dim, int batch) {
+    if (!xs || !ys || !head) return PIT_ERR_NULL;
+    if (metric != PIT_METRIC_EUCLID && metric != PIT_METRIC_PERIODIC2D) return PIT_ERR_METRIC;
+    if (!pit_block_sep_supported(nx, ny, n_head, dim, batch)) return PIT_ERR_UNSUPPORTED;
+    sg.xs = xs; sg.ys = ys; sg.nx = nx; sg.ny = ny; sg.periodic = metric == PIT_METRIC_PERIODIC2D; sg.period = period;
+    sg.head = head; sg.head_is_scale = head_is_scale; sg.scale_out = nullptr; sg.tab = nullptr; sg.tab_wg = -1;
+    return 0;
+}
+}
+
+extern "C" int pit_block_fwd(const float* e, const float* inv, int n_pts, int n_head, int dim, int batch, float* xcat,
+                             const float* w1, const float* b1, const float* w2, const float* b2, int out_gelu,
+                             float* z1, float* h, float* z2, float* y, long ldy, int math_mode, void* stream) {
+    if (!e || !inv) return PIT_ERR_NULL;
+    BlockFwdArgs g;
+    if (int rc = fill_fwd_args(g, n_pts, n_head, dim, batch, xcat, w1, b1, w2, b2, out_gelu, z1, h, z2, y, ldy, math_mode)) return rc;
+    if (!aligned16(e)) return PIT_ERR_SIZE;
+    g.e = e; g.inv = inv;
+    return launch_block_fwd<false>(g, n_head, batch, n_pts, stream);
+}
+
+extern "C" int pit_block_sep_supported(int nx, int ny, int n_head, int dim, int batch) {
+    if (nx < 16 || nx % 16 != 0 || nx > SEP_MAX || ny < 2 || ny > SEP_MAX) return 0;
+    if (!pit_block_supported(nx * ny, n_head, dim, batch)) return 0;
+    return sep_fwd_floats(n_head, nx, ny) <= n_head * PARK_FLOATS && sep_table_floats(n_head, nx, ny, nx, ny, true) <= n_head * PARK_FLOATS &&
+           (size_t)(sep_bwd_floats(n_head, nx, ny) + 2 * 16 * (BD + 4)) * sizeof(float) <= 98304;
+}
+
+extern "C" int pit_block_sep_fwd(const float* xs, const float* ys, int nx, int ny, int metric, float period, const float* head,
+                                 int head_is_scale, int n_head, int dim, int batch, float* xcat,
+                                 const float* w1, const float* b1, const float* w2, const float* b2, int out_gelu,
+                                 float* z1, float* h, float* z2, float* y, long ldy, float* scale_out, float* tables,
+                                 int math_mode, void* stream) {
+    BlockFwdArgs g;
+    if (int rc = fill_fwd_args(g, nx * ny, n_head, dim, batch, xcat, w1, b1, w2, b2, out_gelu, z1, h, z2, y, ldy, math_mode)) return rc;
+    if (int rc = fill_sep_grid(g.sg, xs, ys, nx, ny, metric, period, head, head_is_scale, n_head, dim, batch)) return rc;
+    g.sg.scale_out = scale_out;
+    g.sg.tab = tables;
+    g.sg.tab_wg = tables ? slab_grid(batch, nx * ny / 16) : -1;
+    return launch_block_fwd<true>(g, n_head, batch, nx * ny, stream);
 }
 
 #ifdef PIT_WGREC
@@ -543,14 +979,16 @@
 }
 #endif
 
-extern "C" int pit_block_bwd(const float* e, const float* inv, const float* qw, int n_pts, int n_head, int dim, int batch,
-                             const float* d_xcat, const float* xcat, double* dscale,
-                             const float* w1, const float* w2, const float* z1, const float* z2, int out_gelu, int n0_prev,
-                             float* d_xprev, long ld_dxprev, float* scratch_prev,
-                             float* d_values, long ld_dvalues,
-                             const pit_mlp_params_job* rider, const pit_mlp_params_job* rider2, int math_mode, void* stream) {
-    if (!e || !inv || !d_xcat) return PIT_ERR_NULL;
-    if (dscale && (!qw || !xcat)) return PIT_ERR_NULL;
+namespace {
+template <bool SEP>
+int block_bwd_run(const SepGrid& sg, const float* e, const float* inv, const float* qw, int n_pts, int n_head, int dim, int batch,
+                  const float* d_xcat, const float* xcat, double* dscale,
+                  const float* w1, const float* w2, const float* z1, const float* z2, int out_gelu, int n0_prev,
+                  float* d_xprev, long ld_dxprev, float* scratch_prev,
+                  float* d_values, long ld_dvalues,
+                  const pit_mlp_params_job* rider, const pit_mlp_params_job* rider2, int math_mode, void* stream) {
+    if ((!SEP && (!e || !inv)) || !d_xcat) return PIT_ERR_NULL;
+    if (dscale && ((!SEP && !qw) || !xcat)) return PIT_ERR_NULL;
     if (math_mode != PIT_MATH_FP32 || !pit_block_supported(n_pts, n_head, dim, batch)) return PIT_ERR_UNSUPPORTED;
     const bool has_mlp = w1 != nullptr;
     if (has_mlp) {
@@ -559,7 +997,7 @@
     } else if (!d_values || ld_dvalues < dim || ld_dvalues % 4 != 0 || !aligned16(d_values)) {
         return d_values ? PIT_ERR_SIZE : PIT_ERR_NULL;
     }
-    if (!aligned16(e) || !aligned16(d_xcat) || (qw && !aligned16(qw)) || (xcat && !aligned16(xcat)) ||
+    if ((!SEP && !aligned16(e)) || !aligned16(d_xcat) || (qw && !aligned16(qw)) || (xcat && !aligned16(xcat)) ||
         (has_mlp && (!aligned16(scratch_prev) || (z2 && !aligned16(z2))))) return PIT_ERR_SIZE;
     hipStream_t s = (hipStream_t)stream;
     const long rows = (long)batch * n_pts;
@@ -569,6 +1007,7 @@
     g.d_xprev = d_xprev; g.ld_dxprev = ld_dxprev;
     g.dz1 = scratch_prev; g.dz2 = has_mlp ? scratch_prev + rows * dim : nullptr;
     g.d_values = d_values; g.ld_dvalues = ld_dvalues;
+    g.sg = sg;
     g.n_chain = slab_grid(batch, n_pts / 16);
     g.n_ds = dscale ? g.n_chain : 0;
     pit_detail::DwPair dw = pit_detail::DwPair(), dw2 = pit_detail::DwPair();
@@ -580,15 +1019,17 @@
         if (jobs[r] && pit_detail::plan_dw_pair(*jobs[r], BW, plans[ndw], 768, true)) { carried[r] = true; ++ndw; }
     const int n_dw = (ndw >= 1 ? dw.n1 + dw.n2 : 0) + (ndw >= 2 ? dw2.n1 + dw2.n2 : 0);
     const bool any_rr = (ndw >= 1 && (dw.rr1 || dw.rr2)) || (ndw >= 2 && (dw2.rr1 || dw2.rr2));
-    const size_t sm = std::max(std::max(bwd_smem(n_head, dscale != nullptr), ndw ? (size_t)BW * 16 * 64 * sizeof(float) : (size_t)0),
+    const size_t chain_sm = SEP ? (size_t)(sep_bwd_floats(n_head, sg.nx, sg.ny) + 2 * 16 * (BD + 4)) * sizeof(float)
+                                : bwd_smem(n_head, dscale != nullptr);
+    const size_t sm = std::max(std::max(chain_sm, ndw ? (size_t)BW * 16 * 64 * sizeof(float) : (size_t)0),
                                any_rr ? (size_t)4 * pit_detail::RR_BK * 64 * sizeof(float) : (size_t)0);
     const dim3 grid((unsigned)(g.n_chain + g.n_ds + n_dw)), block(64 * BW);
 #define PIT_BLOCK_BWD(H_, DW_)                                                                                             \
     do {                                                                                                                   \
-        static bool once = ((void)hipFuncSetAttribute((const void*)block_bwd_kernel<H_, DW_>,                             \
+        static bool once = ((void)hipFuncSetAttribute((const void*)block_bwd_kernel<H_, DW_, SEP>,                        \
                                                 hipFuncAttributeMaxDynamicSharedMemorySize, 98304), true);                 \
         (void)once;                                                                                                        \
-        hipLaunchKernelGGL((block_bwd_kernel<H_, DW_>), grid, block, sm, s, g, dw, dw2);                                   \
+        hipLaunchKernelGGL((block_bwd_kernel<H_, DW_, SEP>), grid, block, sm, s, g, dw, dw2);                              \
     } while (0)
 #define PIT_BLOCK_BWD_H(H_) do { if (ndw == 2) PIT_BLOCK_BWD(H_, 2); else if (ndw == 1) PIT_BLOCK_BWD(H_, 1); else PIT_BLOCK_BWD(H_, 0); } while (0)
     if (n_head == 1) PIT_BLOCK_BWD_H(1); else PIT_BLOCK_BWD_H(2);
@@ -604,3 +1045,29 @@
         }
     return 0;
 }
+}
+
+extern "C" int pit_block_bwd(const float* e, const float* inv, const float* qw, int n_pts, int n_head, int dim, int batch,
+                             const float* d_xcat, const float* xcat, double* dscale,
+                             const float* w1, const float* w2, const float* z1, const float* z2, int out_gelu, int n0_prev,
+                             float* d_xprev, long ld_dxprev, float* scratch_prev,
+                             float* d_values, long ld_dvalues,
+                             const pit_mlp_params_job* rider, const pit_mlp_params_job* rider2, int math_mode, void* stream) {
+    return block_bwd_run<false>(SepGrid(), e, inv, qw, n_pts, n_head, dim, batch, d_xcat, xcat, dscale, w1, w2, z1, z2, out_gelu,
+                                n0_prev, d_xprev, ld_dxprev, scratch_prev, d_values, ld_dvalues, rider, rider2, math_mode, stream);
+}
+
+extern "C" int pit_block_sep_bwd(const float* tables, int nx, int ny, int n_head, int dim, int batch,
+                                 const float* d_xcat, const float* xcat, double* dscale,
+                                 const float* w1, const float* w2, const float* z1, const float* z2, int out_gelu, int n0_prev,
+                                 float* d_xprev, long ld_dxprev, float* scratch_prev,
+                                 float* d_values, long ld_dvalues,
+                                 const pit_mlp_params_job* rider, const pit_mlp_params_job* rider2, int math_mode, void* stream) {
+    if (!tables) return PIT_ERR_NULL;
+    if (!pit_block_sep_supported(nx, ny, n_head, dim, batch)) return PIT_ERR_UNSUPPORTED;
+    SepGrid sg = SepGrid();
+    sg.nx = nx; sg.ny = ny; sg.tab = const_cast<float*>(tables); sg.tab_wg = -1;
+    return block_bwd_run<true>(sg, nullptr, nullptr, nullptr, nx * ny, n_head, dim, batch, d_xcat, xcat, dscale, w1, w2, z1, z2,
+                               out_gelu, n0_prev, d_xprev, ld_dxprev, scratch_prev, d_values, ld_dvalues, rider, rider2, math_mode,
+                               stream);
+}
diff --git a/position_induced_transformer_amd/ops.py b/position_induced_transformer_amd/ops.py
--- a/position_induced_transformer_amd/ops.py
+++ b/position_induced_transformer_amd/ops.py
@@ -301,6 +301,27 @@
     return 0.0
 
 
+SEPARABLE_METRICS = ("euclid", "periodic2d")
+SEP_MAX = 32
+
+
+def tensor_grid(mesh: torch.Tensor):
+    if mesh.dim() != 2 or mesh.shape[1] != 2 or mesh.dtype != torch.float32:
+        return None
+    L = mesh.shape[0]
+    bits = mesh.contiguous().view(torch.int32)
+    other = (bits[:, 1] != bits[0, 1]).nonzero()
+    nx = int(other[0, 0]) if other.numel() else L
+    if nx < 16 or nx % 16 != 0 or L % nx != 0 or L // nx < 2:
+        return None
+    ny = L // nx
+    grid = bits.reshape(ny, nx, 2)
+    xb, yb = grid[0, :, 0], grid[:, 0, 1]
+    if not (torch.equal(grid[:, :, 0], xb.expand(ny, nx)) and torch.equal(grid[:, :, 1], yb[:, None].expand(ny, nx))):
+        return None
+    return nx, ny, xb.view(torch.float32).clone(), yb.view(torch.float32).clone()
+
+
 SLAB_UNION_MAX = 64
 FOLD_SLAB_ROWS = (256, 128, 64)
 PLAN_FLAGS = 0
@@ -314,7 +335,7 @@
 
     __slots__ = ("mesh_out", "mesh_in", "mesh_batch", "n_out", "n_in", "sdim", "metric", "metric_id", "period",
                  "rank_k", "rank_w", "masked", "self_attn", "stats", "nbr_idx", "nbr_cnt", "nbr_cap", "rev_ptr",
-                 "rev_row", "_complete", "_union", "_slab", "_fold")
+                 "rev_row", "_complete", "_union", "_slab", "_fold", "grid")
 
     def __init__(self, metric: str, mesh_out: torch.Tensor, mesh_in: torch.Tensor, locality: float,
                  self_attn: bool, period: Optional[float] = None):
@@ -349,6 +370,13 @@
         self._union = None
         self._slab = None
         self._fold = None
+        self.grid = None
+        if (self.self_attn and not self.masked and not batched and self.sdim == 2 and metric in SEPARABLE_METRICS
+                and self.n_in % 16 == 0):
+            g = tensor_grid(self.mesh_in.cpu())
+            if g is not None and g[0] <= SEP_MAX and g[1] <= SEP_MAX:
+                nx, ny, xs, ys = g
+                self.grid = (nx, ny, xs.to(mesh_in.device), ys.to(mesh_in.device))
         cap = 0
         if self.masked and SPARSE_MASKED:
             want = self.rank_k + 2
@@ -1118,6 +1146,15 @@
     return BLOCK_FUSION and bool(_lib.lib().pit_block_supported(int(n_pts), int(n_head), int(dim), int(batch)))
 
 
+BLOCK_SEPARABLE = os.environ.get("PIT_BLOCK_SEPARABLE", "1") != "0"
+
+
+def block_separable(plan: "MeshPlan", n_head: int, dim: int, batch: int) -> bool:
+    g = plan.grid
+    return (BLOCK_SEPARABLE and g is not None
+            and bool(_lib.lib().pit_block_sep_supported(g[0], g[1], int(n_head), int(dim), int(batch))))
+
+
 PRE_WEIGHTS = os.environ.get("PIT_PRE_WEIGHTS", "1") != "0"
 
 
@@ -1269,7 +1306,7 @@
 
 
 def early_block_weights(plan: MeshPlan, lmdas, n_head: int, need_q: bool):
-    if EARLY_WEIGHTS != "rider" or not plan.mesh_in.is_cuda:
+    if EARLY_WEIGHTS != "rider" or not plan.mesh_in.is_cuda or (BLOCK_SEPARABLE and plan.grid is not None):
         return None
     scales = [host_head_scale(p) for p in lmdas] if get_head_scale_route() == "host" else None
     heads = [t.detach().reshape(-1).contiguous() for t in lmdas]
@@ -1288,6 +1325,11 @@
     return ew
 
 
+def _sep_grid_args(plan: MeshPlan, head: torch.Tensor, is_scale: bool):
+    nx, ny, xs, ys = plan.grid
+    return (xs.data_ptr(), ys.data_ptr(), nx, ny, plan.metric_id, plan.period, head.data_ptr(), 1 if is_scale else 0)
+
+
 class _Processor(torch.autograd.Function):
 
     @staticmethod
@@ -1303,7 +1345,15 @@
         heads = [t.detach().reshape(-1).contiguous() for t in lmdas]
         kheads = list(scales) if scales is not None else heads
         need_q = any(ctx.needs_input_grad)
-        if early is not None and early.key == _weights_key(plan, params[0], scales, H) and (early.Q is not None or not need_q):
+        sep = block_separable(plan, H, D, b)
+        tabs = None
+        if sep:
+            E = Q = inv = None
+            scale = torch.empty((n, H), device=dev, dtype=torch.float32)
+            if need_q:
+                nx, ny = plan.grid[:2]
+                tabs = torch.empty((n, H * 2 * (nx * nx + ny * ny)), device=dev, dtype=torch.float32)
+        elif early is not None and early.key == _weights_key(plan, params[0], scales, H) and (early.Q is not None or not need_q):
             E, Q, inv, rowstat, scale = early.E, early.Q, early.inv, early.rowstat, early.scale
         else:
             E, Q, inv, rowstat, scale = _launch_block_weights(plan, kheads, scales is not None, H, need_q, _lib.stream_ptr())
@@ -1327,11 +1377,18 @@
         for i in range(n):
             y, ldy = (bufs[i + 1], W) if i + 1 < n else (out, D)
             w1, b1, w2, b2 = wts[i]
-            rc = L_.pit_block_fwd(E[i].data_ptr(), inv[i].data_ptr(), L, H, D, b, bufs[i].data_ptr(), w1.data_ptr(),
-                                  b1.data_ptr(), w2.data_ptr(), b2.data_ptr(), 1, z1[i].data_ptr(), hh[i].data_ptr(),
-                                  z2[i].data_ptr(), y.data_ptr(), ldy, ctx.math, _lib.stream_ptr())
-            _lib.check(rc, "pit_block_fwd")
+            mlp_args = (bufs[i].data_ptr(), w1.data_ptr(), b1.data_ptr(), w2.data_ptr(), b2.data_ptr(), 1, z1[i].data_ptr(),
+                        hh[i].data_ptr(), z2[i].data_ptr(), y.data_ptr(), ldy)
+            if sep:
+                rc = L_.pit_block_sep_fwd(*_sep_grid_args(plan, kheads[i], scales is not None), H, D, b, *mlp_args,
+                                          scale[i].data_ptr(), tabs[i].data_ptr() if tabs is not None else None, ctx.math,
+                                          _lib.stream_ptr())
+                _lib.check(rc, "pit_block_sep_fwd")
+            else:
+                rc = L_.pit_block_fwd(E[i].data_ptr(), inv[i].data_ptr(), L, H, D, b, *mlp_args, ctx.math, _lib.stream_ptr())
+                _lib.check(rc, "pit_block_fwd")
         ctx.n, ctx.H, ctx.dims, ctx.plan = n, H, (b, L, D), plan
+        ctx.sep = tabs
         ctx.params = params
         ctx.hook = _processor_hook()
         ctx.keep = (bufs, wts, heads, E, Q, inv, scale, z1, hh, z2)
@@ -1396,11 +1453,19 @@
                 prev = (None, None, None, None, 0, 0, None, 0, None, dx.data_ptr(), D)
             k = n - 1 - i
             job2 = ctypes.cast(ctypes.pointer(slices[k]), ctypes.c_void_p) if k < len(slices) else None
-            rc = L_.pit_block_bwd(E[i].data_ptr(), inv[i].data_ptr(), Q[i].data_ptr(), L, H, D, b, dxc[i].data_ptr(),
-                                  bufs[i].data_ptr(), work[i].data_ptr(), *prev,
-                                  ctypes.cast(ctypes.pointer(job), ctypes.c_void_p), job2, ctx.math,
-                                  _lib.stream_ptr())
-            _lib.check(rc, "pit_block_bwd")
+            if ctx.sep is not None:
+                nx, ny = ctx.plan.grid[:2]
+                rc = L_.pit_block_sep_bwd(ctx.sep[i].data_ptr(), nx, ny, H, D, b, dxc[i].data_ptr(),
+                                          bufs[i].data_ptr(), work[i].data_ptr(), *prev,
+                                          ctypes.cast(ctypes.pointer(job), ctypes.c_void_p), job2, ctx.math,
+                                          _lib.stream_ptr())
+                _lib.check(rc, "pit_block_sep_bwd")
+            else:
+                rc = L_.pit_block_bwd(E[i].data_ptr(), inv[i].data_ptr(), Q[i].data_ptr(), L, H, D, b, dxc[i].data_ptr(),
+                                      bufs[i].data_ptr(), work[i].data_ptr(), *prev,
+                                      ctypes.cast(ctypes.pointer(job), ctypes.c_void_p), job2, ctx.math,
+                                      _lib.stream_ptr())
+                _lib.check(rc, "pit_block_bwd")
             if ctx.hook is not None:
                 ctx.hook[0](i)
         d_heads = [None] * n
```

Measured after the change: 55680 samples/s, median of 6. About the same (+1.0%).
